# L0SG/grouped-ssd-pytorch

Hardware: AMD Instinct MI355X
Metric: 512x512 4-phase CT img/s (fwd+loss) (higher is better)
Workload: dtype f32; 1 GPU; gssdpp (BASELINE configs[2], GSSD++: self-attention + SA-base + 1 DCN layer x 4 deformable groups, dcn_cat_sab) fwd + MultiBoxLoss, train-mode BN, batch 32, [B,12,300,300] slices; batch_per_gpu=32, global_batch=32

## Files before the change

grouped-ssd-pytorch_amd/gssd/_lib.py:

```python
import ctypes as C
import os

import torch

_HERE = os.path.dirname(os.path.abspath(__file__))
LIB_PATH = os.environ.get('GSSD_LIB_PATH') or os.path.join(_HERE, 'lib', 'libgssd_hip.so')

c_fp = C.c_void_p
c_i = C.c_int
c_f = C.c_float
c_d = C.c_double
c_i64 = C.c_int64


class ConvDesc(C.Structure):
    _fields_ = [
        ('in_', c_fp), ('wgt', c_fp), ('bias', c_fp), ('out', c_fp), ('out_b', c_fp), ('alpha', c_fp),
        ('gate', c_fp), ('resid', c_fp), ('out2', c_fp), ('in_scale', c_fp), ('in_shift', c_fp), ('in_pad', c_fp),
        ('stats', c_fp), ('wgt_wino', c_fp), ('pool_sign', c_fp), ('wgt_x6', c_fp), ('wgt_patch', c_fp),
        ('B', c_i), ('H', c_i), ('W', c_i), ('in_stride', c_i), ('in_ch_off', c_i), ('Ho', c_i), ('Wo', c_i),
        ('Cout', c_i), ('groups', c_i), ('cin_g', c_i), ('KH', c_i), ('KW', c_i), ('stride', c_i), ('pad', c_i),
        ('dil', c_i), ('K', c_i), ('wgt_row_stride', c_i), ('out_stride', c_i), ('out_ch_off', c_i),
        ('out_mode', c_i), ('relu', c_i), ('m_per_image', c_i), ('split_n', c_i), ('split_k', c_i),
        ('out_b_stride', c_i), ('flags', c_i), ('stats_rep', c_i),
        ('in_batch_stride', c_i64), ('wgt_batch_stride', c_i64), ('out_batch_stride', c_i64),
        ('outb_batch_stride', c_i64), ('out_off', c_i64), ('outb_off', c_i64),
    ]


class DcnGeom(C.Structure):
    _fields_ = [(n, C.c_int32) for n in ('B', 'H', 'W', 'C', 'x_stride', 'Ho', 'Wo', 'kh', 'kw', 'sh', 'sw', 'ph', 'pw', 'dh', 'dw', 'dg',
                                         'off_stride', 'mask_stride', 'mask_logit')]


class PlanOp(C.Structure):
    _fields_ = [('kind', c_i), ('fn', c_i), ('stream', c_i), ('nargs', c_i), ('args', C.c_uint64 * 24)]


PLAN_LAUNCH, PLAN_WAIT = 0, 1


class SnItem(C.Structure):
    _fields_ = [('w', c_fp), ('u', c_fp), ('v', c_fp), ('inv_sigma', c_fp), ('rows', c_i), ('cols', c_i)]


OUT_NHWC, OUT_TRANSPOSED, OUT_HEADS, OUT_SPLIT_T = 0, 1, 2, 3
CONV_OUT_F32, CONV_OUTB_BF16_PERM32, CONV_HEADS_SLICES, CONV_POOL2, CONV_RESID_F32, CONV_F16_OK = 1, 2, 4, 8, 16, 32
CONV_IN_NCHW3, CONV_OUT_GROUPCAT, CONV_OUT_X6PLANES, CONV_RESID_XF = 64, 128, 256, 512

SIGNATURES = {
    'gssd_abi_version': (c_i, []),
    'gssd_event_create': (c_i, [C.POINTER(C.c_void_p)]),
    'gssd_event_destroy': (c_i, [c_fp]),
    'gssd_event_record_node': (c_i, [c_fp, c_fp]),
    'gssd_event_elapsed_ms': (c_i, [c_fp, c_fp, C.POINTER(C.c_float)]),
    'gssd_conv_desc_size': (c_i, []),
    'gssd_last_error': (C.c_char_p, []),
    'gssd_build_arch': (C.c_char_p, []),
    'gssd_pack_input_nhwc': (c_i, [c_fp, c_fp, c_i, c_i, c_i, c_i, c_i, c_i, c_fp]),
    'gssd_unpack_nhwc_to_nchw': (c_i, [c_fp, c_fp, c_i, c_i, c_i, c_i, c_i, c_fp]),
    'gssd_pack_conv_weight': (c_i, [c_fp, c_fp, c_i, c_i, c_i, c_i, c_i, c_i, c_fp]),
    'gssd_conv2d_nhwc_f32': (c_i, [C.POINTER(ConvDesc), c_fp]),
    'gssd_conv2d_nhwc_bf16': (c_i, [C.POINTER(ConvDesc), c_fp]),
    'gssd_conv_x6_tile': (c_i, [c_i, c_i, c_i64]),
    'gssd_conv_x6_weight_elems': (c_i64, [c_i, c_i, c_i, c_i, c_i]),
    'gssd_conv_x6_pack_weight': (c_i, [c_fp, c_fp, c_i, c_i, c_i, c_i, c_i, c_i, c_fp]),
    'gssd_conv_x6_takes': (c_i, [C.POINTER(ConvDesc)]),
    'gssd_conv_wino_x6_takes': (c_i, [C.POINTER(ConvDesc)]),
    'gssd_conv_thin_x6_takes': (c_i, [C.POINTER(ConvDesc)]),
    'gssd_conv_thin_nchw3_takes': (c_i, [C.POINTER(ConvDesc)]),
    'gssd_plan_fn_count': (c_i, []),
    'gssd_plan_fn_name': (C.c_char_p, [c_i]),
    'gssd_plan_fn_index': (c_i, [C.c_char_p]),
    'gssd_plan_fn_nargs': (c_i, [c_i]),
    'gssd_plan_op_size': (c_i, []),
    'gssd_plan_run': (c_i, [C.POINTER(PlanOp), c_i, C.POINTER(c_fp), c_i, C.POINTER(c_i)]),
    'gssd_pack_conv_weight_bf16': (c_i, [c_fp, c_fp, c_i, c_i, c_i, c_i, c_i, c_i, c_fp]),
    'gssd_cast_f32_bf16': (c_i, [c_fp, c_fp, c_i64, c_fp]),
    'gssd_cast_rows_f32_bf16': (c_i, [c_fp, c_fp, c_i64, c_i, c_i, c_i, c_fp]),
    'gssd_transpose_cast_f32_bf16': (c_i, [c_fp, c_fp, c_i64, c_i, c_i64, c_i64, c_fp]),
    'gssd_cast_bf16_f32': (c_i, [c_fp, c_fp, c_i64, c_fp]),
    'gssd_pack_input_nhwc_bf16': (c_i, [c_fp, c_fp, c_i, c_i, c_i, c_i, c_i, c_fp]),
    'gssd_bn_relu_pool_bf16': (c_i, [c_fp, c_fp, c_i, c_i, c_i, c_i, c_i, c_i, c_i, c_i, c_i, c_fp, c_d, c_fp, c_fp,
                                     c_fp, c_fp, c_f, c_f, c_i, c_i, c_i, c_fp]),
    'gssd_bn_finalize_bf16': (c_i, [c_fp, c_d, c_fp, c_fp, c_fp, c_fp, c_f, c_f, c_i, c_i, c_fp, c_fp, c_fp, c_i, c_fp]),
    'gssd_l2norm_bf16': (c_i, [c_fp, c_fp, c_fp, c_i64, c_i, c_f, c_fp]),
    'gssd_dcn_packed_weight_elems_bf16': (C.c_longlong, [c_i, c_i]),
    'gssd_dcn_pack_weight_bf16': (c_i, [c_fp, c_fp, c_i, c_i, c_i, c_fp]),
    'gssd_dcn_forward_bf16': (c_i, [c_fp, c_fp, c_fp, c_fp, c_fp, c_i, c_i, c_i, c_i, c_i, c_i, c_i, c_fp]),
    'gssd_winograd_weight_elems': (C.c_longlong, [c_i, c_i, c_i]),
    'gssd_winograd_weight_f32': (c_i, [c_fp, c_fp, c_i, c_i, c_i, c_i, c_fp]),
    'gssd_conv2d_wgrad_f32': (c_i, [C.POINTER(ConvDesc), c_fp, c_fp, c_fp]),
    'gssd_conv2d_wgrad_bf16': (c_i, [C.POINTER(ConvDesc), c_fp, c_fp, c_fp]),
    'gssd_conv2d_wgrad_bf16_supported': (c_i, [C.POINTER(ConvDesc)]),
    'gssd_unpack_conv_weight_grad': (c_i, [c_fp, c_fp, c_i, c_i, c_i, c_i, c_i, c_i, c_i, c_fp]),
    'gssd_pack_conv_weight_dgrad': (c_i, [c_fp, c_fp, c_i, c_i, c_i, c_i, c_i, c_fp]),
    'gssd_bn_relu_pool_f32': (c_i, [c_fp, c_fp, c_i, c_i, c_i, c_i, c_i, c_i, c_i, c_i, c_i, c_fp, c_d, c_fp, c_fp,
                                    c_fp, c_fp, c_f, c_f, c_i, c_i, c_i, c_fp]),
    'gssd_bn_finalize_f32': (c_i, [c_fp, c_d, c_fp, c_fp, c_fp, c_fp, c_f, c_f, c_i, c_i, c_fp, c_fp, c_fp, c_i, c_fp]),
    'gssd_bn_bwd_reduce_f32': (c_i, [c_fp, c_fp, c_fp, c_fp, c_fp, c_fp, c_i, c_i, c_i, c_i, c_i, c_i, c_i, c_i, c_i, c_i, c_fp]),
    'gssd_bn_bwd_finalize_f32': (c_i, [c_fp, c_d, c_fp, c_fp, c_f, c_i, c_fp, c_fp, c_fp, c_fp, c_fp, c_i, c_fp]),
    'gssd_bn_bwd_apply_f32': (c_i, [c_fp, c_fp, c_fp, c_fp, c_fp, c_i64, c_i, c_fp, c_fp]),
    'gssd_bn_bwd_reduce_mixed': (c_i, [c_fp, c_i, c_fp, c_fp, c_fp, c_fp, c_fp, c_fp, c_i, c_i, c_i, c_i, c_i, c_i, c_i, c_i, c_i, c_i, c_fp]),
    'gssd_bn_bwd_apply_mixed': (c_i, [c_fp, c_i, c_fp, c_fp, c_fp, c_fp, c_fp, c_i, c_fp, c_fp, c_fp, c_i64, c_i, c_fp, c_i, c_fp]),
    'gssd_bn_bwd_apply_masked_f32': (c_i, [c_fp, c_fp, c_fp, c_fp, c_i, c_fp, c_fp, c_fp, c_fp, c_i64, c_i, c_fp, c_fp]),
    'gssd_colsum_f32': (c_i, [c_fp, c_i64, c_i, c_i, c_fp, c_fp]),
    'gssd_cast_f64_f32': (c_i, [c_fp, c_fp, c_i, c_i, c_fp]),
    'gssd_l2norm_bwd_f32': (c_i, [c_fp, c_fp, c_fp, c_fp, c_fp, c_fp, c_i64, c_i, c_f, c_fp]),
    'gssd_heads_gather_f32': (c_i, [c_fp, c_fp, c_fp, c_i, c_i, c_i, c_i, c_i, c_i, c_fp]),
    'gssd_upsample_insert_f32': (c_i, [c_fp, c_fp, c_i, c_i, c_i, c_i, c_i, c_i, c_i, c_fp]),
    'gssd_l2norm_f32': (c_i, [c_fp, c_fp, c_fp, c_i64, c_i, c_f, c_fp]),
    'gssd_self_attn_core_f32': (c_i, [c_fp, c_fp, c_fp, c_i, c_i, c_i, c_i, c_i, c_i, c_fp]),
    'gssd_self_attn_core_kv_f32': (c_i, [c_fp, c_fp, c_fp, c_fp, c_i, c_i, c_i, c_i, c_i, c_i, c_i, c_i, c_fp, c_fp]),
    'gssd_sa_pool_kv_f32': (c_i, [c_fp, c_fp, c_fp, c_fp, c_i, c_i, c_i, c_i, c_i, c_i, c_i, c_fp]),
    'gssd_sa_unpool_f32': (c_i, [c_fp, c_fp, c_i, c_i, c_i, c_i, c_i, c_fp]),
    'gssd_pack_conv_weights_batched': (c_i, [c_fp, c_i, c_fp]),
    'gssd_gemm_slot_takes': (c_i, [c_fp]),
    'gssd_conv_flat_bf16_takes': (c_i, [c_fp]),
    'gssd_conv_flat_bf16_tile': (c_i, [c_i]),
    'gssd_heads_reduce_f32': (c_i, [c_fp, c_fp, c_fp, c_i, c_i, c_i, c_fp]),
    'gssd_interp_add_f32': (c_i, [c_fp, c_fp, c_fp, c_fp, c_i, c_i, c_i, c_i, c_i, c_i, c_fp]),
    'gssd_pixellink_final_f32': (c_i, [c_fp, c_fp, c_fp, c_fp, c_i, c_fp, c_fp, c_fp, c_fp, c_fp, c_fp, c_i, c_i, c_fp]),
    'gssd_pixellink_loss_f32': (c_i, [c_fp, c_fp, c_fp, c_fp, c_fp, c_fp, c_fp, c_fp, c_i, c_i, c_i, c_i, c_fp]),
    'gssd_interp_add_bwd_f32': (c_i, [c_fp, c_fp, c_fp, c_fp, c_i, c_i, c_i, c_i, c_i, c_i, c_i, c_fp]),
    'gssd_pixellink_final_bwd_f32': (c_i, [c_fp] * 6 + [c_i, c_fp, c_fp, c_fp, c_fp, c_fp, c_fp, c_i, c_fp, c_fp, c_i, c_i, c_i, c_fp]),
    'gssd_pixellink_loss_bwd_f32': (c_i, [c_fp] * 10 + [c_i, c_i, c_i, c_fp]),
    'gssd_pixellink_decode_f32': (c_i, [c_fp, c_fp, c_fp, c_fp, c_fp, c_i, c_i, c_i, C.c_float, C.c_float, c_i, c_fp]),
    'gssd_self_attn_flash_bwd_bf16': (c_i, [c_fp, c_fp, c_fp, c_fp, c_fp, c_fp, c_fp, c_fp, c_i, c_i, c_i, c_i, c_fp]),
    'gssd_cast_split_f32_bf16': (c_i, [c_fp, c_fp, c_fp, c_i64, c_fp]),
    'gssd_self_attn_flash_bwd_supported': (c_i, [c_i, c_i]),
    'gssd_self_attn_core_x6_supported': (c_i, [c_i, c_i]),
    'gssd_self_attn_core_x6_ws_bytes': (C.c_longlong, [c_i, c_i, c_i, c_i]),
    'gssd_self_attn_core_x6_f32': (c_i, [c_fp, c_fp, c_fp, c_i, c_i, c_i, c_i, c_i, c_fp, c_fp, c_fp]),
    'gssd_self_attn_core_x6_planes_f32': (c_i, [c_fp, c_fp, c_i, c_i, c_i, c_i, c_fp, c_fp]),
    'gssd_self_attn_core_bf16v': (c_i, [c_fp, c_fp, c_fp, c_i, c_i, c_i, c_i, c_i, c_fp, c_fp]),
    'gssd_softmax_rows_f32': (c_i, [c_fp, c_i64, c_i, c_i, c_fp]),
    'gssd_slice_and_cat_f32': (c_i, [c_fp, c_fp, c_fp, c_i64, c_i, c_i, c_i, c_fp]),
    'gssd_spectral_norm_f32': (c_i, [c_fp, c_i, c_i, c_f, c_fp]),
    'gssd_dcn_im2col_f32': (c_i, [c_fp, c_fp, c_fp, c_i, c_i, c_i, c_i, c_i, c_i, c_fp]),
    'gssd_dcn_im2col_bf16': (c_i, [c_fp, c_fp, c_fp, c_i, c_i, c_i, c_i, c_i, c_i, c_fp]),
    'gssd_dcn_packed_weight_elems_x6': (C.c_longlong, [c_i, c_i]),
    'gssd_dcn_pack_weight_x6': (c_i, [c_fp, c_fp, c_i, c_i, c_i, c_fp]),
    'gssd_dcn_forward_x6': (c_i, [c_fp, c_fp, c_fp, c_fp, c_fp, c_i, c_i, c_i, c_i, c_i, c_i, c_i, c_fp]),
    'gssd_conv_patch_x6_weight_elems': (C.c_longlong, [c_i, c_i]),
    'gssd_conv_patch_x6_pack_weight': (c_i, [c_fp, c_fp, c_i, c_i, c_i, c_fp]),
    'gssd_conv_patch_x6_takes': (c_i, [C.POINTER(ConvDesc)]),
    'gssd_dcn_forward_x6_ex': (c_i, [c_fp, c_fp, c_fp, c_fp, c_fp, c_i, c_i, c_i, c_i, c_i, c_i, c_i, c_i, c_fp]),
    'gssd_dcn_packed_weight_elems': (C.c_longlong, [c_i, c_i]),
    'gssd_dcn_pack_weight_f32': (c_i, [c_fp, c_fp, c_i, c_i, c_i, c_fp]),
    'gssd_dcn_streamk': (c_i, [c_i]),
    'gssd_dcn_streamk_status': (c_i, [c_fp]),
    'gssd_dcn_streamk_reset': (c_i, [c_fp]),
    'gssd_dcn_streamk_release': (c_i, [c_fp]),
    'gssd_dcn_forward_f32': (c_i, [c_fp, c_fp, c_fp, c_fp, c_fp, c_i, c_i, c_i, c_i, c_i, c_i, c_i, c_fp]),
    'gssd_resample_ksize': (c_i, [c_i, c_i, c_i]),
    'gssd_resample_coeffs': (c_i, [c_i, c_i, c_i, c_fp, c_fp]),
    'gssd_resize_u8_horizontal': (c_i, [c_fp, c_fp, c_fp, c_fp, c_i, c_i, c_i, c_i, c_i, c_i, c_fp]),
    'gssd_resize_u8_vertical': (c_i, [c_fp, c_fp, c_fp, c_fp, c_i, c_i, c_i, c_i, c_i, c_i, c_i, c_fp, c_fp]),
    'gssd_input_finish_f32': (c_i, [c_fp, c_fp, c_f, c_f, c_f, c_fp, c_i, c_i, c_i, c_i, c_i, c_fp]),
    'gssd_aug_desc_size': (c_i, []),
    'gssd_augment_minmax': (c_i, [c_fp, c_i, c_i, c_i, c_fp, c_fp]),
    'gssd_augment_horizontal': (c_i, [c_fp, c_fp, c_fp, c_f, c_f, c_f, c_fp, c_i, c_i, c_i, c_i, c_i, c_fp]),
    'gssd_augment_vertical': (c_i, [c_fp, c_fp, c_fp, c_fp, c_i, c_i, c_i, c_fp]),
    'gssd_pixellink_targets': (c_i, [c_fp, c_fp, c_i, c_i, c_i, c_fp, c_fp, c_fp, c_fp, c_fp]),
    'gssd_pixellink_final5_f32': (c_i, [c_fp] * 5 + [c_i] + [c_fp] * 6 + [c_i, c_i, c_fp]),
    'gssd_pixellink_final5_bwd_f32': (c_i, [c_fp] * 7 + [c_i] + [c_fp] * 7 + [c_i, c_fp, c_fp, c_i, c_i, c_i, c_fp]),
    'gssd_self_attn_flash_bwd_f32_supported': (c_i, [c_i, c_i]),
    'gssd_self_attn_flash_bwd_f32': (c_i, [c_fp, c_i, c_fp, c_i, c_fp, c_i, c_fp, c_fp, c_fp, c_fp, c_i, c_fp, c_fp, c_i, c_i, c_i, c_i, c_i,
                                           c_i, c_fp]),
    'gssd_eval_match': (c_i, [c_fp, C.c_longlong, c_i, c_i, c_fp, c_fp, c_fp, c_i, c_d, c_fp, c_i, c_i, c_fp, c_fp, c_fp]),
    'gssd_eval_workspace_bytes': (C.c_longlong, [c_i]),
    'gssd_eval_ap': (c_i, [c_fp, c_fp, c_i, c_i, c_d, c_i, c_fp, C.c_longlong, c_fp, c_fp]),
    'gssd_bgemm_f32': (c_i, [c_fp, c_fp, c_fp, c_i, c_i, c_i, c_i, c_i, c_i, c_i, c_i, C.c_longlong, C.c_longlong, C.c_longlong, c_i, c_f,
                             c_i, c_fp]),
    'gssd_softmax_bwd_rows_f32': (c_i, [c_fp, c_fp, c_i64, c_i, c_i, c_fp]),
    'gssd_sn_weight_grad_f32': (c_i, [c_fp, c_i, c_fp, c_fp, c_fp, c_fp, c_fp, c_fp, c_fp, c_i, c_i, c_fp]),
    'gssd_scaled_transpose_f32': (c_i, [c_fp, c_fp, c_fp, c_i, c_i, c_fp]),
    'gssd_dot_f32': (c_i, [c_fp, c_fp, c_i64, c_fp, c_fp]),
    'gssd_rowdot_f32': (c_i, [c_fp, c_fp, c_fp, c_i64, c_i, c_fp]),
    'gssd_bgemm_ex_f32': (c_i, [c_fp, c_fp, c_fp, c_i, c_i, c_i, c_i, c_i, c_i, c_i, c_i, C.c_longlong, C.c_longlong, C.c_longlong, c_i, c_f,
                                c_i, c_fp, c_fp, c_fp]),
    'gssd_axpby_f32': (c_i, [c_fp, c_fp, c_fp, c_i64, c_f, c_f, c_fp]),
    'gssd_scale_cast_f64_f32': (c_i, [c_fp, c_fp, c_fp, c_i, c_fp]),
    'gssd_sa_sigma_grad_f32': (c_i, [c_fp, c_fp, c_fp, c_i, c_fp, c_fp]),
    'gssd_dcn_col2im_f32': (c_i, [c_fp, c_fp, c_fp, c_fp, c_fp, c_i, c_i, c_i, c_i, c_i, c_i, c_fp]),
    'gssd_dcn_geo_im2col_f32': (c_i, [c_fp, c_fp, c_fp, c_fp, C.POINTER(DcnGeom), c_i, c_i, c_fp]),
    'gssd_dcn_geo_col2im_f32': (c_i, [c_fp] * 7 + [C.POINTER(DcnGeom), c_i, c_i, c_fp]),
    'gssd_match_batch': (c_i, [c_fp, c_fp, c_fp, c_i, c_i, c_f, c_f, c_f, c_fp, c_fp, c_fp]),
    'gssd_reduce_max_f32': (c_i, [c_fp, c_i64, c_fp, c_i, c_fp]),
    'gssd_hnm_loss': (c_i, [c_fp, c_fp, c_fp, c_fp, c_fp, c_i, c_i, c_i, c_i, c_i, c_fp, c_fp, c_fp, c_fp]),
    'gssd_loss_finalize': (c_i, [c_fp, c_i, c_fp, c_fp, c_fp]),
    'gssd_loss_finalize_global': (c_i, [c_fp, c_i, c_fp, c_i, c_fp, c_fp, c_fp]),
    'gssd_loss_backward': (c_i, [c_fp, c_fp, c_fp, c_fp, c_fp, c_fp, c_fp, c_fp, c_i, c_i, c_i, c_fp, c_fp, c_fp]),
    'gssd_detect': (c_i, [c_fp, c_fp, c_fp, c_i, c_i, c_i, c_i, c_f, c_f, c_f, c_f, c_i, c_i, c_fp, c_fp, c_fp, c_fp]),
    'gssd_softmax_lastdim_f32': (c_i, [c_fp, c_fp, c_i64, c_i, c_fp]),
}


class GssdError(RuntimeError):
    pass


def _load():
    if not os.path.exists(LIB_PATH):
        raise GssdError(
            f'{LIB_PATH} is missing: the HIP kernels are not built.  Run `make -C '
            f'{os.path.join(_HERE, "csrc")}` (needs hipcc, --offload-arch=gfx950) or '
            f'`python -c "import __graft_entry__ as g; g.build()"`.  There is no CPU fallback.')
    lib = C.CDLL(LIB_PATH)
    for name, (res, args) in SIGNATURES.items():
        try:
            fn = getattr(lib, name)
        except AttributeError as e:
            raise GssdError(f'{LIB_PATH} does not export {name}; rebuild it') from e
        fn.restype = res
        fn.argtypes = args
    if lib.gssd_plan_op_size() != C.sizeof(PlanOp):
        raise GssdError(f'{LIB_PATH}: struct gssd_plan_op is {lib.gssd_plan_op_size()} bytes in the library, {C.sizeof(PlanOp)} in this '
                        f'binding; rebuild the library')
    if lib.gssd_conv_desc_size() != C.sizeof(ConvDesc):
        raise GssdError(f'{LIB_PATH}: struct gssd_conv_desc is {lib.gssd_conv_desc_size()} bytes in the library, '
                        f'{C.sizeof(ConvDesc)} in this binding; rebuild the library')
    return lib


lib = _load()


def check(rc):
    if rc != 0:
        raise GssdError(f'libgssd_hip: error {rc}: {lib.gssd_last_error().decode()}')
```

grouped-ssd-pytorch_amd/gssd/csrc/elementwise.hip:

```cpp
#include "common.h"
#include "kernel_util.h"

namespace {

constexpr int EW_THREADS = 256;
inline int ew_blocks(long long work_items, int per_block = EW_THREADS, int cap = 8192) {
    long long b = (work_items + per_block - 1) / per_block;
    if (b < 1) b = 1;
    if (b > cap) b = cap;
    return (int)b;
}

__global__ void pack_input_kernel(const float* __restrict__ x, float* __restrict__ y, int B, int C, int HW,
                                  int groups, int cpg_in, int cpg_out) {
    const long long total = (long long)B * HW * groups;
    for (long long i = blockIdx.x * (long long)blockDim.x + threadIdx.x; i < total;
         i += (long long)gridDim.x * blockDim.x) {
        const int g = (int)(i % groups);
        const long long bp = i / groups;
        const int pix = (int)(bp % HW);
        const int b = (int)(bp / HW);
        float* o = y + (bp * groups + g) * cpg_out;
        for (int c = 0; c < cpg_out; ++c)
            o[c] = (c < cpg_in) ? x[((long long)b * C + g * cpg_in + c) * HW + pix] : 0.f;
    }
}

__global__ void unpack_nhwc_kernel(const float* __restrict__ x, float* __restrict__ y, int B, int C, int HW,
                                   int x_stride) {
    const long long total = (long long)B * C * HW;
    for (long long i = blockIdx.x * (long long)blockDim.x + threadIdx.x; i < total;
         i += (long long)gridDim.x * blockDim.x) {
        const int pix = (int)(i % HW);
        const long long bc = i / HW;
        const int c = (int)(bc % C);
        const int b = (int)(bc / C);
        y[i] = x[((long long)b * HW + pix) * x_stride + c];
    }
}

__global__ void pack_weight_kernel(const float* __restrict__ w, float* __restrict__ wp, int Cout, int cin_g, int taps,
                                   int cin_g_pad, int Kpad) {
    const long long total = (long long)Cout * Kpad;
    for (long long i = blockIdx.x * (long long)blockDim.x + threadIdx.x; i < total;
         i += (long long)gridDim.x * blockDim.x) {
        const int k = (int)(i % Kpad);
        const int o = (int)(i / Kpad);
        const int tap = k / cin_g_pad, c = k - tap * cin_g_pad;
        float v = 0.f;
        if (tap < taps && c < cin_g) v = w[((long long)o * cin_g + c) * taps + tap];
        wp[i] = v;
    }
}

__global__ void pack_weight_batched_kernel(const gssd_pack_item* __restrict__ items) {
    const gssd_pack_item it = items[blockIdx.y];
    const long long total = (long long)it.Cout * it.Kpad;
    for (long long i = blockIdx.x * (long long)blockDim.x + threadIdx.x; i < total; i += (long long)gridDim.x * blockDim.x) {
        const int k = (int)(i % it.Kpad);
        const int o = (int)(i / it.Kpad);
        const int tap = k / it.cin_g_pad, c = k - tap * it.cin_g_pad;
        float v = 0.f;
        if (tap < it.taps && c < it.cin_g) v = it.w[((long long)o * it.cin_g + c) * it.taps + tap];
        it.wp[i] = v;
    }
}

__global__ __launch_bounds__(256) void bn_relu_pool_kernel(
    const float* __restrict__ raw, float* __restrict__ out, int B, int H, int W, int C, int Ho, int Wo, int pk, int ps,
    int pp, const double* __restrict__ stats, double count, const float* __restrict__ gamma,
    const float* __restrict__ beta, float* running_mean, float* running_var, float momentum, float eps, int training,
    int relu, int srep) {
    extern __shared__ __attribute__((aligned(16))) float sm[];
    float* s_scale = sm;
    float* s_shift = sm + C;
    for (int c = threadIdx.x; c < C; c += blockDim.x) {
        if (gamma == nullptr) {
            s_scale[c] = 1.f;
            s_shift[c] = 0.f;
            continue;
        }
        double mean, var;
        if (training) {
            mean = gssd_stats_sum(stats, c, 2 * C, srep) / count;
            var = gssd_stats_sum(stats, C + c, 2 * C, srep) / count - mean * mean;
            if (var < 0.0) var = 0.0;
            if (blockIdx.x == 0) {
                const double unb = count > 1.0 ? var * count / (count - 1.0) : var;
                running_mean[c] = (float)((1.0 - (double)momentum) * (double)running_mean[c] + (double)momentum * mean);
                running_var[c] = (float)((1.0 - (double)momentum) * (double)running_var[c] + (double)momentum * unb);
            }
        } else {
            mean = (double)running_mean[c];
            var = (double)running_var[c];
        }
        const double inv = 1.0 / sqrt(var + (double)eps);
        const double sc = (double)gamma[c] * inv;
        s_scale[c] = (float)sc;
        s_shift[c] = (float)((double)beta[c] - mean * sc);
    }
    __syncthreads();
    const int C4 = C >> 2;
    const long long total = (long long)B * Ho * Wo * C4;
    for (long long i = blockIdx.x * (long long)blockDim.x + threadIdx.x; i < total;
         i += (long long)gridDim.x * blockDim.x) {
        const int c4 = (int)(i % C4);
        long long t = i / C4;
        const int xo = (int)(t % Wo);
        t /= Wo;
        const int yo = (int)(t % Ho);
        const int b = (int)(t / Ho);
        const f32x4 sc = *reinterpret_cast<const f32x4*>(s_scale + 4 * c4);
        const f32x4 sh = *reinterpret_cast<const f32x4*>(s_shift + 4 * c4);
        f32x4 r;
        if (pk == 0) {
            const f32x4 v = *reinterpret_cast<const f32x4*>(raw + (((long long)b * H + yo) * W + xo) * C + 4 * c4);
            r = v * sc + sh;
        } else {
            r = {-INFINITY, -INFINITY, -INFINITY, -INFINITY};
            const int y0 = yo * ps - pp, x0 = xo * ps - pp;
            for (int dy = 0; dy < pk; ++dy) {
                const int yy = y0 + dy;
                if ((unsigned)yy >= (unsigned)H) continue;
                for (int dx = 0; dx < pk; ++dx) {
                    const int xx = x0 + dx;
                    if ((unsigned)xx >= (unsigned)W) continue;
                    const f32x4 v =
                        *reinterpret_cast<const f32x4*>(raw + (((long long)b * H + yy) * W + xx) * C + 4 * c4);
                    const f32x4 a = v * sc + sh;
#pragma unroll
                    for (int e = 0; e < 4; ++e) r[e] = fmaxf(r[e], a[e]);
                }
            }
        }
        if (relu) {
#pragma unroll
            for (int e = 0; e < 4; ++e) r[e] = fmaxf(r[e], 0.f);
        }
        *reinterpret_cast<f32x4*>(out + i * 4) = r;
    }
}

__global__ void bn_finalize_kernel(const double* __restrict__ stats, double count, const float* __restrict__ gamma,
                                   const float* __restrict__ beta, float* running_mean, float* running_var,
                                   float momentum, float eps, int training, int C, float* __restrict__ scale,
                                   float* __restrict__ shift, float* __restrict__ pad, int srep) {
    const int c = blockIdx.x * blockDim.x + threadIdx.x;
    if (c >= C) return;
    double mean, var;
    if (training) {
        mean = gssd_stats_sum(stats, c, 2 * C, srep) / count;
        var = gssd_stats_sum(stats, C + c, 2 * C, srep) / count - mean * mean;
        if (var < 0.0) var = 0.0;
        if (training == 1) {
            const double unb = count > 1.0 ? var * count / (count - 1.0) : var;
            running_mean[c] = (float)((1.0 - (double)momentum) * (double)running_mean[c] + (double)momentum * mean);
            running_var[c] = (float)((1.0 - (double)momentum) * (double)running_var[c] + (double)momentum * unb);
        }
    } else {
        mean = (double)running_mean[c];
        var = (double)running_var[c];
    }
    double sc = (double)gamma[c] * (1.0 / sqrt(var + (double)eps));
    const float sh = (float)((double)beta[c] - mean * sc);
    float scf = (float)sc;
    if (scf == 0.f) scf = 1e-30f;
    scale[c] = scf;
    shift[c] = sh;
    pad[c] = scf > 0.f ? -3.0e38f : 3.0e38f;
}

__global__ __launch_bounds__(256) void l2norm_kernel(const float* __restrict__ x, const float* __restrict__ w,
                                                     float* __restrict__ out, long long pixels, int C, float eps) {
    const int lane = threadIdx.x & 63;
    const long long wave0 = (blockIdx.x * (long long)blockDim.x + threadIdx.x) >> 6;
    const long long nwaves = ((long long)gridDim.x * blockDim.x) >> 6;
    const int C4 = C >> 2;
    for (long long p = wave0; p < pixels; p += nwaves) {
        const f32x4* xp = reinterpret_cast<const f32x4*>(x + p * C);
        float ss = 0.f;
        for (int c = lane; c < C4; c += 64) {
            const f32x4 v = xp[c];
            ss += v[0] * v[0] + v[1] * v[1] + v[2] * v[2] + v[3] * v[3];
        }
        ss = wave_sum(ss);
        const float inv = 1.f / (sqrtf(ss) + eps);
        f32x4* op = reinterpret_cast<f32x4*>(out + p * C);
        for (int c = lane; c < C4; c += 64) {
            const f32x4 v = xp[c];
            const f32x4 ww = reinterpret_cast<const f32x4*>(w)[c];
            op[c] = ww * (v * inv);
        }
    }
}

__global__ __launch_bounds__(256) void softmax_rows_kernel(float* __restrict__ x, long long rows, int n, int stride) {
    const int lane = threadIdx.x & 63;
    const long long wave0 = (blockIdx.x * (long long)blockDim.x + threadIdx.x) >> 6;
    const long long nwaves = ((long long)gridDim.x * blockDim.x) >> 6;
    for (long long rI = wave0; rI < rows; rI += nwaves) {
        float* row = x + rI * stride;
        float m = -INFINITY;
        for (int c = lane; c < n; c += 64) m = fmaxf(m, row[c]);
        m = wave_max(m);
        float s = 0.f;
        for (int c = lane; c < n; c += 64) {
            const float e = expf(row[c] - m);
            row[c] = e;
            s += e;
        }
        s = wave_sum(s);
        const float inv = 1.f / s;
        for (int c = lane; c < stride; c += 64) row[c] = (c < n) ? row[c] * inv : 0.f;
    }
}

__global__ void slice_and_cat_kernel(const float* __restrict__ a, const float* __restrict__ b, float* __restrict__ out,
                                     long long pixels, int Ca, int Cb, int groups) {
    const int Co = Ca + Cb, Co4 = Co >> 2;
    const int ga = Ca / groups, gb = Cb / groups;
    const long long total = pixels * Co4;
    for (long long i = blockIdx.x * (long long)blockDim.x + threadIdx.x; i < total;
         i += (long long)gridDim.x * blockDim.x) {
        const int c = (int)(i % Co4) * 4;
        const long long p = i / Co4;
        const int g = c / (ga + gb), cc = c - g * (ga + gb);
        f32x4 v;
        if (cc < ga) v = *reinterpret_cast<const f32x4*>(a + p * Ca + g * ga + cc);
        else v = *reinterpret_cast<const f32x4*>(b + p * Cb + g * gb + (cc - ga));
        *reinterpret_cast<f32x4*>(out + i * 4) = v;
    }
}

__device__ float block_sum(float v, float* red) {
    v = wave_sum(v);
    const int lane = threadIdx.x & 63, wave = threadIdx.x >> 6;
    __syncthreads();
    if (lane == 0) red[wave] = v;
    __syncthreads();
    float t = 0.f;
    for (int i = 0; i < (int)(blockDim.x >> 6); ++i) t += red[i];
    return t;
}

__global__ __launch_bounds__(1024) void spectral_norm_kernel(const gssd_sn_item* __restrict__ items, int do_iter,
                                                            float eps) {
    extern __shared__ __attribute__((aligned(16))) float sm[];
    const gssd_sn_item it = items[blockIdx.x];
    const int R = it.rows, Cc = it.cols;
    float* su = sm;
    float* sv = sm + R;
    float* red = sv + Cc;
    const int tid = threadIdx.x, lane = tid & 63, wave = tid >> 6, nw = blockDim.x >> 6;
    for (int i = tid; i < R; i += blockDim.x) su[i] = it.u[i];
    for (int i = tid; i < Cc; i += blockDim.x) sv[i] = it.v[i];
    __syncthreads();
    const bool vec = ((Cc | R) & 3) == 0 && (Cc >> 2) <= (int)blockDim.x && (((uintptr_t)it.w) & 15) == 0;
    if (do_iter) {
        float nrm = 0.f;
        if (vec) {
            float* part = red + 16;
            const int nq = Cc >> 2, S = (int)blockDim.x / nq;
            const int cq = tid % nq, rs = tid / nq;
            if (rs < S) {
                f32x4 a8[8];
#pragma unroll
                for (int q = 0; q < 8; ++q) a8[q] = f32x4{0.f, 0.f, 0.f, 0.f};
                const float* wc = it.w + 4 * cq;
                int rr = rs;
                for (; rr + 7 * S < R; rr += 8 * S) {
#pragma unroll
                    for (int q = 0; q < 8; ++q) a8[q] += *reinterpret_cast<const f32x4*>(wc + (size_t)(rr + q * S) * Cc) * su[rr + q * S];
                }
                for (; rr < R; rr += S) a8[0] += *reinterpret_cast<const f32x4*>(wc + (size_t)rr * Cc) * su[rr];
                *reinterpret_cast<f32x4*>(part + rs * Cc + 4 * cq) = ((a8[0] + a8[1]) + (a8[2] + a8[3])) + ((a8[4] + a8[5]) + (a8[6] + a8[7]));
            }
            __syncthreads();
            for (int c = tid; c < Cc; c += blockDim.x) {
                float acc = part[c];
                for (int sl = 1; sl < S; ++sl) acc += part[sl * Cc + c];
                sv[c] = acc;
                nrm += acc * acc;
            }
        } else {
            for (int c = tid; c < Cc; c += blockDim.x) {
                float a8[8] = {0.f, 0.f, 0.f, 0.f, 0.f, 0.f, 0.f, 0.f};
                int rr = 0;
                for (; rr + 8 <= R; rr += 8) {
#pragma unroll
                    for (int q = 0; q < 8; ++q) a8[q] += it.w[(size_t)(rr + q) * Cc + c] * su[rr + q];
                }
                for (; rr < R; ++rr) a8[0] += it.w[(size_t)rr * Cc + c] * su[rr];
                const float acc = ((a8[0] + a8[1]) + (a8[2] + a8[3])) + ((a8[4] + a8[5]) + (a8[6] + a8[7]));
                sv[c] = acc;
                nrm += acc * acc;
            }
        }
        nrm = block_sum(nrm, red);
        const float inv = 1.f / fmaxf(sqrtf(nrm), eps);
        for (int c = tid; c < Cc; c += blockDim.x) sv[c] *= inv;
        __syncthreads();
    }
    float sig = 0.f, nrm2 = 0.f;
    auto row_done = [&](int rr, float acc) {
        if (do_iter) {
            su[rr] = acc;
            nrm2 += acc * acc;
        } else {
            sig += su[rr] * acc;
        }
    };
    if (vec) {
        for (int r0 = wave * 4; r0 < R; r0 += nw * 4) {
            float acc[4] = {0.f, 0.f, 0.f, 0.f};
            for (int c = lane * 4; c < Cc; c += 256) {
                const f32x4 v4 = *reinterpret_cast<const f32x4*>(sv + c);
#pragma unroll
                for (int q = 0; q < 4; ++q) {
                    if (r0 + q < R) {
                        const f32x4 w4 = *reinterpret_cast<const f32x4*>(it.w + (size_t)(r0 + q) * Cc + c);
                        acc[q] += (w4[0] * v4[0] + w4[1] * v4[1]) + (w4[2] * v4[2] + w4[3] * v4[3]);
                    }
                }
            }
#pragma unroll
            for (int q = 0; q < 4; ++q) {
                const float t = wave_sum(acc[q]);
                if (lane == 0 && r0 + q < R) row_done(r0 + q, t);
            }
        }
    } else {
        for (int rr = wave; rr < R; rr += nw) {
            float acc = 0.f;
            for (int c = lane; c < Cc; c += 64) acc += it.w[(size_t)rr * Cc + c] * sv[c];
            acc = wave_sum(acc);
            if (lane == 0) row_done(rr, acc);
        }
    }
    if (do_iter) {
        nrm2 = block_sum(nrm2, red);
        const float nn = fmaxf(sqrtf(nrm2), eps);
        __syncthreads();
        for (int i = tid; i < R; i += blockDim.x) it.u[i] = su[i] / nn;
        for (int i = tid; i < Cc; i += blockDim.x) it.v[i] = sv[i];
        const float is = nn / nrm2;
        for (int i = tid; i < R; i += blockDim.x) it.inv_sigma[i] = is;
    } else {
        sig = block_sum(sig, red);
        const float is = 1.f / sig;
        for (int i = tid; i < R; i += blockDim.x) it.inv_sigma[i] = is;
    }
}

__global__ void softmax_lastdim_kernel(const float* __restrict__ x, float* __restrict__ y, long long rows, int C) {
    for (long long i = blockIdx.x * (long long)blockDim.x + threadIdx.x; i < rows;
         i += (long long)gridDim.x * blockDim.x) {
        const float* xr = x + i * C;
        float m = xr[0];
        for (int c = 1; c < C; ++c) m = fmaxf(m, xr[c]);
        float s = 0.f;
        for (int c = 0; c < C; ++c) s += (float)exp((double)(xr[c] - m));
        for (int c = 0; c < C; ++c) y[i * C + c] = (float)exp((double)(xr[c] - m)) / s;
    }
}

__global__ __launch_bounds__(256) void reduce_max_kernel(const float* __restrict__ x, long long n, float* out) {
    __shared__ float red[4];
    float m = -INFINITY;
    const long long n4 = n >> 2;
    for (long long i = blockIdx.x * (long long)blockDim.x + threadIdx.x; i < n4; i += (long long)gridDim.x * blockDim.x) {
        const f32x4 v = reinterpret_cast<const f32x4*>(x)[i];
        m = fmaxf(fmaxf(m, fmaxf(v[0], v[1])), fmaxf(v[2], v[3]));
    }
    if (blockIdx.x == 0)
        for (long long i = (n4 << 2) + threadIdx.x; i < n; i += blockDim.x) m = fmaxf(m, x[i]);
    m = wave_max(m);
    if ((threadIdx.x & 63) == 0) red[threadIdx.x >> 6] = m;
    __syncthreads();
    if (threadIdx.x == 0) out[blockIdx.x] = fmaxf(fmaxf(red[0], red[1]), fmaxf(red[2], red[3]));
}

__global__ __launch_bounds__(256) void heads_reduce_kernel(const float* __restrict__ ws, const signed char* __restrict__ splits,
                                                          float* __restrict__ out, long long total, int P, int C) {
    for (long long i = blockIdx.x * (long long)blockDim.x + threadIdx.x; i < total; i += (long long)gridDim.x * blockDim.x) {
        const int p = (int)((i / C) % P);
        const int n = splits[p];
        float a = ws[i];
        for (int k = 1; k < n; ++k) a += ws[(size_t)k * total + i];
        out[i] = a;
    }
}

}

extern "C" int gssd_pack_input_nhwc(const float* x, float* y, int B, int C, int H, int W, int groups, int cpg_out,
                                    gssd_stream_t stream) {
    GSSD_CHECK_ARG(x && y && B > 0 && C > 0 && H > 0 && W > 0 && groups > 0 && C % groups == 0);
    GSSD_CHECK_ARG(cpg_out >= C / groups);
    const long long total = (long long)B * H * W * groups;
    hipLaunchKernelGGL(pack_input_kernel, dim3(ew_blocks(total)), dim3(EW_THREADS), 0, as_stream(stream), x, y, B, C,
                       H * W, groups, C / groups, cpg_out);
    GSSD_CHECK_LAUNCH();
    return GSSD_OK;
}

extern "C" int gssd_unpack_nhwc_to_nchw(const float* x, float* y, int B, int C, int H, int W, int x_stride,
                                        gssd_stream_t stream) {
    GSSD_CHECK_ARG(x && y && B > 0 && C > 0 && H > 0 && W > 0 && x_stride >= C);
    hipLaunchKernelGGL(unpack_nhwc_kernel, dim3(ew_blocks((long long)B * C * H * W)), dim3(EW_THREADS), 0,
                       as_stream(stream), x, y, B, C, H * W, x_stride);
    GSSD_CHECK_LAUNCH();
    return GSSD_OK;
}

extern "C" int gssd_pack_conv_weight(const float* w, float* wp, int Cout, int cin_g, int KH, int KW, int cin_g_pad,
                                     int Kpad, gssd_stream_t stream) {
    GSSD_CHECK_ARG(w && wp && Cout > 0 && cin_g > 0 && KH > 0 && KW > 0);
    GSSD_CHECK_ARG(cin_g_pad >= cin_g && cin_g_pad % 4 == 0 && Kpad >= KH * KW * cin_g_pad && Kpad % 4 == 0);
    hipLaunchKernelGGL(pack_weight_kernel, dim3(ew_blocks((long long)Cout * Kpad)), dim3(EW_THREADS), 0,
                       as_stream(stream), w, wp, Cout, cin_g, KH * KW, cin_g_pad, Kpad);
    GSSD_CHECK_LAUNCH();
    return GSSD_OK;
}

extern "C" int gssd_pack_conv_weights_batched(const gssd_pack_item* items_dev, int n_items, gssd_stream_t stream) {
    GSSD_CHECK_ARG(items_dev && n_items > 0 && n_items < 65536);
    hipLaunchKernelGGL(pack_weight_batched_kernel, dim3(48, n_items), dim3(EW_THREADS), 0, as_stream(stream), items_dev);
    GSSD_CHECK_LAUNCH();
    return GSSD_OK;
}

extern "C" int gssd_bn_relu_pool_f32(const float* raw, float* out, int B, int H, int W, int C, int Ho, int Wo,
                                     int pool_k, int pool_s, int pool_p, const double* stats, double count,
                                     const float* gamma, const float* beta, float* running_mean, float* running_var,
                                     float momentum, float eps, int training, int relu, int stats_rep, gssd_stream_t stream) {
    GSSD_CHECK_ARG(raw && out && stats_rep >= 0);
    GSSD_CHECK_ARG(gamma == nullptr || (beta && running_mean && running_var));
    GSSD_CHECK_ARG(B > 0 && H > 0 && W > 0 && C > 0 && C % 4 == 0 && Ho > 0 && Wo > 0);
    GSSD_CHECK_ARG(!training || gamma == nullptr || (stats != nullptr && count > 0));
    if (pool_k == 0) GSSD_CHECK_ARG(Ho == H && Wo == W);
    else GSSD_CHECK_ARG(pool_s > 0 && pool_p >= 0 && (Ho - 1) * pool_s - pool_p < H && (Wo - 1) * pool_s - pool_p < W);
    const long long total = (long long)B * Ho * Wo * (C / 4);
    const int blocks = ew_blocks(total, EW_THREADS * 4, 2048);
    hipLaunchKernelGGL(bn_relu_pool_kernel, dim3(blocks), dim3(EW_THREADS), 2 * C * sizeof(float), as_stream(stream),
                       raw, out, B, H, W, C, Ho, Wo, pool_k, pool_s, pool_p, stats, count, gamma, beta, running_mean,
                       running_var, momentum, eps, training, relu, stats_rep);
    GSSD_CHECK_LAUNCH();
    return GSSD_OK;
}

extern "C" int gssd_bn_finalize_f32(const double* stats, double count, const float* gamma, const float* beta,
                                    float* running_mean, float* running_var, float momentum, float eps, int training,
                                    int C, float* scale, float* shift, float* pad, int stats_rep, gssd_stream_t stream) {
    GSSD_CHECK_ARG(gamma && beta && running_mean && running_var && scale && shift && pad && C > 0 && stats_rep >= 0);
    GSSD_CHECK_ARG(!training || (stats != nullptr && count > 0));
    hipLaunchKernelGGL(bn_finalize_kernel, dim3((C + 255) / 256), dim3(256), 0, as_stream(stream), stats, count, gamma,
                       beta, running_mean, running_var, momentum, eps, training, C, scale, shift, pad, stats_rep);
    GSSD_CHECK_LAUNCH();
    return GSSD_OK;
}

extern "C" int gssd_l2norm_f32(const float* x, const float* weight, float* out, int64_t pixels, int C, float eps,
                               gssd_stream_t stream) {
    GSSD_CHECK_ARG(x && weight && out && pixels > 0 && C > 0 && C % 4 == 0);
    hipLaunchKernelGGL(l2norm_kernel, dim3(ew_blocks(pixels, 4, 4096)), dim3(256), 0, as_stream(stream), x, weight, out,
                       (long long)pixels, C, eps);
    GSSD_CHECK_LAUNCH();
    return GSSD_OK;
}

extern "C" int gssd_softmax_rows_f32(float* x, int64_t rows, int n, int row_stride, gssd_stream_t stream) {
    GSSD_CHECK_ARG(x && rows > 0 && n > 0 && row_stride >= n);
    hipLaunchKernelGGL(softmax_rows_kernel, dim3(ew_blocks(rows, 4, 16384)), dim3(256), 0, as_stream(stream), x,
                       (long long)rows, n, row_stride);
    GSSD_CHECK_LAUNCH();
    return GSSD_OK;
}

extern "C" int gssd_slice_and_cat_f32(const float* a, const float* b, float* out, int64_t pixels, int Ca, int Cb,
                                      int groups, gssd_stream_t stream) {
    GSSD_CHECK_ARG(a && b && out && pixels > 0 && groups > 0 && Ca % (4 * groups) == 0 && Cb % (4 * groups) == 0);
    hipLaunchKernelGGL(slice_and_cat_kernel, dim3(ew_blocks(pixels * ((Ca + Cb) / 4))), dim3(EW_THREADS), 0,
                       as_stream(stream), a, b, out, (long long)pixels, Ca, Cb, groups);
    GSSD_CHECK_LAUNCH();
    return GSSD_OK;
}

extern "C" int gssd_spectral_norm_f32(const gssd_sn_item* items_dev, int n, int do_power_iteration, float eps,
                                      gssd_stream_t stream) {
    GSSD_CHECK_ARG(items_dev && n > 0);
    const size_t smem = (4096 + 16 + 4096) * sizeof(float);
    hipLaunchKernelGGL(spectral_norm_kernel, dim3(n), dim3(1024), smem, as_stream(stream), items_dev,
                       do_power_iteration, eps);
    GSSD_CHECK_LAUNCH();
    return GSSD_OK;
}

extern "C" int gssd_softmax_lastdim_f32(const float* x, float* y, int64_t rows, int C, gssd_stream_t stream) {
    GSSD_CHECK_ARG(x && y && rows > 0 && C > 0);
    hipLaunchKernelGGL(softmax_lastdim_kernel, dim3(ew_blocks(rows)), dim3(EW_THREADS), 0, as_stream(stream), x, y,
                       (long long)rows, C);
    GSSD_CHECK_LAUNCH();
    return GSSD_OK;
}

extern "C" int gssd_reduce_max_f32(const float* x, int64_t n, float* out, int out_n, gssd_stream_t stream) {
    GSSD_CHECK_ARG(x && out && n > 0 && out_n > 0 && out_n <= 1024 && ((uintptr_t)x % 16) == 0);
    hipLaunchKernelGGL(reduce_max_kernel, dim3(out_n), dim3(256), 0, as_stream(stream), x, (long long)n, out);
    GSSD_CHECK_LAUNCH();
    return GSSD_OK;
}

extern "C" int gssd_heads_reduce_f32(const float* ws, const signed char* splits, float* out, int B, int P, int C, gssd_stream_t stream) {
    GSSD_CHECK_ARG(ws && splits && out && B > 0 && P > 0 && C > 0);
    const long long total = (long long)B * P * C;
    int blocks = (int)((total + 255) / 256);
    if (blocks > 4096) blocks = 4096;
    hipLaunchKernelGGL(heads_reduce_kernel, dim3(blocks), dim3(256), 0, as_stream(stream), ws, splits, out, total, P, C);
    GSSD_CHECK_LAUNCH();
    return GSSD_OK;
}
```

grouped-ssd-pytorch_amd/gssd/csrc/loss.hip:

```cpp
#include "common.h"

namespace {

constexpr int MAX_GT = 64;
constexpr int LT = 1024;

__device__ __forceinline__ float iou_pf(float ax1, float ay1, float ax2, float ay2, float area_a, float bx1, float by1,
                                        float bx2, float by2) {
    const float w = fmaxf(fminf(ax2, bx2) - fmaxf(ax1, bx1), 0.f);
    const float h = fmaxf(fminf(ay2, by2) - fmaxf(ay1, by1), 0.f);
    const float inter = w * h;
    const float area_b = (bx2 - bx1) * (by2 - by1);
    const float uni = (area_a + area_b) - inter;
    return __fdiv_rn(inter, uni);
}

__global__ __launch_bounds__(LT) void match_kernel(const float* __restrict__ targets, const int* __restrict__ gt_off,
                                                   const float* __restrict__ priors, int P, float thr,
                                                   float var0, float var1, float* __restrict__ loc_t,
                                                   int64_t* __restrict__ conf_t) {
    extern __shared__ __attribute__((aligned(16))) unsigned char smraw[];
    __shared__ float gt[MAX_GT][5];
    __shared__ float gt_area[MAX_GT];
    __shared__ int best_prior[MAX_GT];
    __shared__ float red_v[LT / 64];
    __shared__ int red_i[LT / 64];
    short* forced = reinterpret_cast<short*>(smraw);

    const int b = blockIdx.x, tid = threadIdx.x;
    const int g0 = gt_off[b];
    int n = gt_off[b + 1] - g0;
    if (n > MAX_GT) n = MAX_GT;
    if (tid < 5) gt[0][tid] = 0.f;
    __syncthreads();
    for (int i = tid; i < n * 5; i += LT) gt[i / 5][i % 5] = targets[(size_t)g0 * 5 + i];
    for (int p = tid; p < P; p += LT) forced[p] = -1;
    __syncthreads();
    if (tid < n) gt_area[tid] = (gt[tid][2] - gt[tid][0]) * (gt[tid][3] - gt[tid][1]);
    __syncthreads();

    for (int j = 0; j < n; ++j) {
        float bv = -INFINITY;
        int bi = 0x7fffffff;
        bool any_nan = false;
        for (int p = tid; p < P; p += LT) {
            const float4 pr = reinterpret_cast<const float4*>(priors)[p];
            const float hx = pr.z / 2.f, hy = pr.w / 2.f;
            const float v = iou_pf(gt[j][0], gt[j][1], gt[j][2], gt[j][3], gt_area[j], pr.x - hx, pr.y - hy, pr.x + hx,
                                   pr.y + hy);
            if (v > bv) {
                bv = v;
                bi = p;
            }
        }
        (void)any_nan;
        for (int o = 32; o > 0; o >>= 1) {
            const float ov = __shfl_xor(bv, o, 64);
            const int oi = __shfl_xor(bi, o, 64);
            if (ov > bv || (ov == bv && oi < bi)) {
                bv = ov;
                bi = oi;
            }
        }
        if ((tid & 63) == 0) {
            red_v[tid >> 6] = bv;
            red_i[tid >> 6] = bi;
        }
        __syncthreads();
        if (tid == 0) {
            for (int w = 1; w < LT / 64; ++w)
                if (red_v[w] > bv || (red_v[w] == bv && red_i[w] < bi)) {
                    bv = red_v[w];
                    bi = red_i[w];
                }
            best_prior[j] = (bi == 0x7fffffff) ? 0 : bi;
        }
        __syncthreads();
    }
    if (tid == 0)
        for (int j = 0; j < n; ++j) forced[best_prior[j]] = (short)j;
    __syncthreads();

    for (int p = tid; p < P; p += LT) {
        const float4 pr = reinterpret_cast<const float4*>(priors)[p];
        const float hx = pr.z / 2.f, hy = pr.w / 2.f;
        const float px1 = pr.x - hx, py1 = pr.y - hy, px2 = pr.x + hx, py2 = pr.y + hy;
        float bv = -INFINITY;
        int bj = 0;
        for (int j = 0; j < n; ++j) {
            const float v = iou_pf(gt[j][0], gt[j][1], gt[j][2], gt[j][3], gt_area[j], px1, py1, px2, py2);
            if (v > bv) {
                bv = v;
                bj = j;
            }
        }
        const int f = forced[p];
        if (f >= 0) {
            bv = 2.f;
            bj = f;
        }
        int64_t conf = (int64_t)(gt[bj][4] + 1.f);
        if (bv < thr) conf = 0;
        conf_t[(size_t)b * P + p] = conf;
        const float gx1 = gt[bj][0], gy1 = gt[bj][1], gx2 = gt[bj][2], gy2 = gt[bj][3];
        float4 o;
        o.x = __fdiv_rn(((gx1 + gx2) / 2.f) - pr.x, var0 * pr.z);
        o.y = __fdiv_rn(((gy1 + gy2) / 2.f) - pr.y, var0 * pr.w);
        o.z = __fdiv_rn((float)log((double)__fdiv_rn(gx2 - gx1, pr.z)), var1);
        o.w = __fdiv_rn((float)log((double)__fdiv_rn(gy2 - gy1, pr.w)), var1);
        reinterpret_cast<float4*>(loc_t)[(size_t)b * P + p] = o;
    }
}

__device__ unsigned radix_select_desc(const float* vals, int n, int k, unsigned* hist , int* bcast ,
                                      int* n_greater) {
    unsigned prefix = 0, mask = 0;
    int greater = 0;
    for (int shift = 24; shift >= 0; shift -= 8) {
        for (int i = threadIdx.x; i < 256; i += blockDim.x) hist[i] = 0;
        __syncthreads();
        for (int i = threadIdx.x; i < n; i += blockDim.x) {
            const unsigned u = __float_as_uint(vals[i]);
            if ((u & mask) == prefix) atomicAdd(&hist[(u >> shift) & 255u], 1u);
        }
        __syncthreads();
        if (threadIdx.x == 0) {
            int acc = greater, bin = 255;
            for (; bin > 0; --bin) {
                if (acc + (int)hist[bin] >= k) break;
                acc += (int)hist[bin];
            }
            bcast[0] = bin;
            bcast[1] = acc;
        }
        __syncthreads();
        prefix |= ((unsigned)bcast[0]) << shift;
        mask |= 255u << shift;
        greater = bcast[1];
        __syncthreads();
    }
    *n_greater = greater;
    return prefix;
}

__global__ __launch_bounds__(LT) void hnm_loss_kernel(const float* __restrict__ loc, const float* __restrict__ conf,
                                                      const float* __restrict__ loc_t,
                                                      const int64_t* __restrict__ conf_t,
                                                      const float* __restrict__ xmax_p, int xmax_n, int P, int C, int negpos_ratio,
                                                      uint8_t* __restrict__ sel, double* __restrict__ partial,
                                                      float* __restrict__ lca_out) {
    extern __shared__ __attribute__((aligned(16))) unsigned char smraw[];
    float* lca = reinterpret_cast<float*>(smraw);
    __shared__ unsigned hist[256];
    __shared__ int bcast[2];
    __shared__ int s_cnt[LT / 64];
    __shared__ double s_red[LT / 64][2];
    __shared__ int s_tie_base;

    const int b = blockIdx.x, tid = threadIdx.x, lane = tid & 63, wave = tid >> 6;
    float xmax = xmax_p[0];
    for (int i = 1; i < xmax_n; ++i) xmax = fmaxf(xmax, xmax_p[i]);
    const float* cb = conf + (size_t)b * P * C;
    const int64_t* tb = conf_t + (size_t)b * P;

    int npos = 0;
    for (int p = tid; p < P; p += LT) {
        const int t = (int)tb[p];
        float s = 0.f;
        for (int c = 0; c < C; ++c) s += (float)exp((double)(cb[(size_t)p * C + c] - xmax));
        float v = ((float)log((double)s) + xmax) - cb[(size_t)p * C + t];
        if (t > 0) {
            v = 0.f;
            ++npos;
        }
        if (!(v > 0.f)) v = 0.f;
        lca[p] = v;
    }
    npos = wave_sum(npos);
    if (lane == 0) s_cnt[wave] = npos;
    __syncthreads();
    npos = 0;
    for (int w = 0; w < LT / 64; ++w) npos += s_cnt[w];
    int num_neg = negpos_ratio * npos;
    if (num_neg > P - 1) num_neg = P - 1;
    if (lca_out)
        for (int p = tid; p < P; p += LT) lca_out[(size_t)b * P + p] = lca[p];

    unsigned kth_bits = 0xffffffffu;
    int n_greater = 0;
    if (num_neg > 0) kth_bits = radix_select_desc(lca, P, num_neg, hist, bcast, &n_greater);
    const int ties_needed = num_neg - n_greater;

    double sum_l = 0.0, sum_c = 0.0;
    if (tid == 0) s_tie_base = 0;
    __syncthreads();
    for (int p0 = 0; p0 < P; p0 += LT) {
        const int p = p0 + tid;
        bool is_tie = false, take = false, pos = false;
        if (p < P) {
            const unsigned u = __float_as_uint(lca[p]);
            pos = tb[p] > 0;
            if (num_neg > 0) {
                if (u > kth_bits) take = true;
                else if (u == kth_bits) is_tie = true;
            }
        }
        const unsigned long long bal = __ballot(is_tie);
        const int before = __popcll(bal & ((1ull << lane) - 1ull));
        if (lane == 0) s_cnt[wave] = __popcll(bal);
        __syncthreads();
        int base = s_tie_base;
        for (int w = 0; w < wave; ++w) base += s_cnt[w];
        if (is_tie && base + before < ties_needed) take = true;
        __syncthreads();
        if (tid == 0) {
            int t = 0;
            for (int w = 0; w < LT / 64; ++w) t += s_cnt[w];
            s_tie_base += t;
        }
        if (p < P) {
            const uint8_t code = pos ? 1 : (take ? 2 : 0);
            const bool neg_flag = take;
            sel[(size_t)b * P + p] = pos ? (uint8_t)(neg_flag ? 3 : 1) : code;
            if (pos) {
                const float4 a = reinterpret_cast<const float4*>(loc)[(size_t)b * P + p];
                const float4 t4 = reinterpret_cast<const float4*>(loc_t)[(size_t)b * P + p];
                const float d[4] = {a.x - t4.x, a.y - t4.y, a.z - t4.z, a.w - t4.w};
#pragma unroll
                for (int e = 0; e < 4; ++e) {
                    const float ad = fabsf(d[e]);
                    sum_l += (double)(ad < 1.f ? 0.5f * d[e] * d[e] : ad - 0.5f);
                }
            }
            if (pos || take) {
                const int t = (int)tb[p];
                float m = cb[(size_t)p * C];
                for (int c = 1; c < C; ++c) m = fmaxf(m, cb[(size_t)p * C + c]);
                double s = 0.0;
                for (int c = 0; c < C; ++c) s += exp((double)(cb[(size_t)p * C + c] - m));
                sum_c += (log(s) + (double)m) - (double)cb[(size_t)p * C + t];
            }
        }
        __syncthreads();
    }
    sum_l = wave_sum(sum_l);
    sum_c = wave_sum(sum_c);
    if (lane == 0) {
        s_red[wave][0] = sum_l;
        s_red[wave][1] = sum_c;
    }
    __syncthreads();
    if (tid == 0) {
        double l = 0.0, c = 0.0;
        for (int w = 0; w < LT / 64; ++w) {
            l += s_red[w][0];
            c += s_red[w][1];
        }
        partial[(size_t)b * 4 + 0] = l;
        partial[(size_t)b * 4 + 1] = c;
        partial[(size_t)b * 4 + 2] = (double)npos;
        partial[(size_t)b * 4 + 3] = (double)num_neg;
    }
}

__global__ void loss_finalize_kernel(const double* __restrict__ partial, int B, float* __restrict__ losses,
                                     double* __restrict__ n_total) {
    if (threadIdx.x == 0 && blockIdx.x == 0) {
        double l = 0.0, c = 0.0, n = 0.0;
        for (int b = 0; b < B; ++b) {
            l += partial[b * 4 + 0];
            c += partial[b * 4 + 1];
            n += partial[b * 4 + 2];
        }
        losses[0] = (float)(l / n);
        losses[1] = (float)(c / n);
        if (n_total) *n_total = n;
    }
}

__global__ void loss_finalize_global_kernel(const double* __restrict__ partial, int B, const double* __restrict__ n_global, int world,
                                            float* __restrict__ losses, double* __restrict__ n_total) {
    if (threadIdx.x == 0 && blockIdx.x == 0) {
        double l = 0.0, c = 0.0;
        for (int b = 0; b < B; ++b) {
            l += partial[b * 4 + 0];
            c += partial[b * 4 + 1];
        }
        const double n = *n_global / (double)world;
        losses[0] = (float)(l / n);
        losses[1] = (float)(c / n);
        *n_total = n;
    }
}

__global__ void loss_backward_kernel(const float* __restrict__ loc, const float* __restrict__ conf,
                                     const float* __restrict__ loc_t, const int64_t* __restrict__ conf_t,
                                     const uint8_t* __restrict__ sel, const double* __restrict__ n_total,
                                     const float* __restrict__ gl_p, const float* __restrict__ gc_p, long long BP, int C,
                                     float* __restrict__ dloc, float* __restrict__ dconf) {
    const float invN = (float)(1.0 / *n_total);
    const float gl = (gl_p ? *gl_p : 1.f) * invN, gc = (gc_p ? *gc_p : 1.f) * invN;
    for (long long i = blockIdx.x * (long long)blockDim.x + threadIdx.x; i < BP;
         i += (long long)gridDim.x * blockDim.x) {
        const uint8_t s = sel[i];
        float4 g = {0.f, 0.f, 0.f, 0.f};
        if (s & 1) {
            const float4 a = reinterpret_cast<const float4*>(loc)[i];
            const float4 t = reinterpret_cast<const float4*>(loc_t)[i];
            const float d[4] = {a.x - t.x, a.y - t.y, a.z - t.z, a.w - t.w};
            float o[4];
#pragma unroll
            for (int e = 0; e < 4; ++e) o[e] = (fabsf(d[e]) < 1.f ? d[e] : (d[e] > 0.f ? 1.f : -1.f)) * gl;
            g = {o[0], o[1], o[2], o[3]};
        }
        reinterpret_cast<float4*>(dloc)[i] = g;
        if (s) {
            const int t = (int)conf_t[i];
            float m = conf[i * C];
            for (int c = 1; c < C; ++c) m = fmaxf(m, conf[i * C + c]);
            float z = 0.f;
            for (int c = 0; c < C; ++c) z += __expf(conf[i * C + c] - m);
            for (int c = 0; c < C; ++c) dconf[i * C + c] = (__expf(conf[i * C + c] - m) / z - (c == t ? 1.f : 0.f)) * gc;
        } else {
            for (int c = 0; c < C; ++c) dconf[i * C + c] = 0.f;
        }
    }
}

}

extern "C" int gssd_match_batch(const float* targets, const int* gt_off, const float* priors, int B, int P,
                                float threshold, float var0, float var1, float* loc_t, int64_t* conf_t,
                                gssd_stream_t stream) {
    GSSD_CHECK_ARG(targets && gt_off && priors && loc_t && conf_t);
    GSSD_CHECK_ARG(B > 0 && P > 0 && P < 32768);
    GSSD_CHECK_ARG(((uintptr_t)priors % 16) == 0 && ((uintptr_t)loc_t % 16) == 0);
    hipLaunchKernelGGL(match_kernel, dim3(B), dim3(LT), (size_t)P * sizeof(short), as_stream(stream), targets, gt_off,
                       priors, P, threshold, var0, var1, loc_t, conf_t);
    GSSD_CHECK_LAUNCH();
    return GSSD_OK;
}

extern "C" int gssd_hnm_loss(const float* loc, const float* conf, const float* loc_t, const int64_t* conf_t,
                             const float* xmax, int xmax_n, int B, int P, int C, int negpos_ratio, uint8_t* sel,
                             double* partial, float* loss_c_all, gssd_stream_t stream) {
    GSSD_CHECK_ARG(loc && conf && loc_t && conf_t && xmax && xmax_n > 0 && sel && partial);
    GSSD_CHECK_ARG(B > 0 && P > 0 && P <= 36000 && C >= 2 && negpos_ratio >= 0);
    GSSD_CHECK_ARG(((uintptr_t)loc % 16) == 0 && ((uintptr_t)loc_t % 16) == 0);
    static unsigned attr_mask = 0;
    const size_t smem = (size_t)P * sizeof(float);
    if (smem > 48 * 1024)
        if (const int rc = gssd_max_dynamic_lds(&attr_mask, hnm_loss_kernel, 150 * 1024)) return rc;
    hipLaunchKernelGGL(hnm_loss_kernel, dim3(B), dim3(LT), smem, as_stream(stream), loc, conf, loc_t, conf_t, xmax, xmax_n, P,
                       C, negpos_ratio, sel, partial, loss_c_all);
    GSSD_CHECK_LAUNCH();
    return GSSD_OK;
}

extern "C" int gssd_loss_finalize(const double* partial, int B, float* losses, double* n_total, gssd_stream_t stream) {
    GSSD_CHECK_ARG(partial && losses && B > 0);
    hipLaunchKernelGGL(loss_finalize_kernel, dim3(1), dim3(64), 0, as_stream(stream), partial, B, losses, n_total);
    GSSD_CHECK_LAUNCH();
    return GSSD_OK;
}

extern "C" int gssd_loss_finalize_global(const double* partial, int B, const double* n_global, int world, float* losses, double* n_total,
                                         gssd_stream_t stream) {
    GSSD_CHECK_ARG(partial && losses && n_global && n_total && B > 0 && world > 0);
    hipLaunchKernelGGL(loss_finalize_global_kernel, dim3(1), dim3(64), 0, as_stream(stream), partial, B, n_global, world, losses, n_total);
    GSSD_CHECK_LAUNCH();
    return GSSD_OK;
}

extern "C" int gssd_loss_backward(const float* loc, const float* conf, const float* loc_t, const int64_t* conf_t,
                                  const uint8_t* sel, const double* n_total, const float* grad_l, const float* grad_c,
                                  int B, int P, int C, float* dloc, float* dconf, gssd_stream_t stream) {
    GSSD_CHECK_ARG(loc && conf && loc_t && conf_t && sel && n_total && dloc && dconf && B > 0 && P > 0 && C >= 2);
    const long long BP = (long long)B * P;
    int blocks = (int)((BP + 255) / 256);
    if (blocks > 4096) blocks = 4096;
    hipLaunchKernelGGL(loss_backward_kernel, dim3(blocks), dim3(256), 0, as_stream(stream), loc, conf, loc_t, conf_t, sel,
                       n_total, grad_l, grad_c, BP, C, dloc, dconf);
    GSSD_CHECK_LAUNCH();
    return GSSD_OK;
}
```

grouped-ssd-pytorch_amd/gssd/csrc/plan_run.hip:

```cpp
#include <hip/hip_runtime.h>
#include <cstdint>
#include <cstring>
#include <mutex>
#include <tuple>
#include <type_traits>
#include <utility>
#include "common.h"

namespace {

template <class T>
inline T plan_arg(uint64_t w) {
    if constexpr (std::is_pointer_v<T>) {
        return reinterpret_cast<T>(static_cast<uintptr_t>(w));
    } else if constexpr (std::is_same_v<T, float>) {
        const uint32_t b = static_cast<uint32_t>(w);
        float f;
        memcpy(&f, &b, 4);
        return f;
    } else if constexpr (std::is_same_v<T, double>) {
        double d;
        memcpy(&d, &w, 8);
        return d;
    } else {
        static_assert(std::is_integral_v<T>, "plan argument types: pointers, integers, float, double");
        return static_cast<T>(static_cast<int64_t>(w));
    }
}

template <class... P, size_t... I>
inline int plan_call(int (*f)(P...), const uint64_t* a, gssd_stream_t s, std::index_sequence<I...>) {
    using T = std::tuple<P...>;
    static_assert(sizeof...(P) - 1 <= GSSD_PLAN_MAX_ARGS, "GSSD_PLAN_MAX_ARGS");
    static_assert(std::is_same_v<std::tuple_element_t<sizeof...(P) - 1, T>, gssd_stream_t>, "the last parameter is the stream");
    return f(plan_arg<std::tuple_element_t<I, T>>(a[I])..., s);
}

template <class... P>
constexpr int plan_nargs(int (*)(P...)) { return (int)sizeof...(P) - 1; }

struct PlanFn {
    const char* name;
    int nargs;
    int (*thunk)(const uint64_t*, gssd_stream_t);
};

template <auto F>
int plan_thunk(const uint64_t* a, gssd_stream_t s) {
    return plan_call(F, a, s, std::make_index_sequence<plan_nargs(F)>{});
}

#define GSSD_PLAN_FN(f) PlanFn{#f, plan_nargs(&f), &plan_thunk<&f>}
const PlanFn g_plan_fns[] = {
    GSSD_PLAN_FN(gssd_event_record_node),
    GSSD_PLAN_FN(gssd_pack_input_nhwc),
    GSSD_PLAN_FN(gssd_unpack_nhwc_to_nchw),
    GSSD_PLAN_FN(gssd_pack_conv_weight),
    GSSD_PLAN_FN(gssd_pack_conv_weights_batched),
    GSSD_PLAN_FN(gssd_conv2d_nhwc_f32),
    GSSD_PLAN_FN(gssd_conv_x6_pack_weight),
    GSSD_PLAN_FN(gssd_conv_patch_x6_pack_weight),
    GSSD_PLAN_FN(gssd_conv2d_nhwc_bf16),
    GSSD_PLAN_FN(gssd_pack_conv_weight_bf16),
    GSSD_PLAN_FN(gssd_cast_f32_bf16),
    GSSD_PLAN_FN(gssd_cast_bf16_f32),
    GSSD_PLAN_FN(gssd_pack_input_nhwc_bf16),
    GSSD_PLAN_FN(gssd_bn_relu_pool_bf16),
    GSSD_PLAN_FN(gssd_bn_finalize_bf16),
    GSSD_PLAN_FN(gssd_l2norm_bf16),
    GSSD_PLAN_FN(gssd_winograd_weight_f32),
    GSSD_PLAN_FN(gssd_conv2d_wgrad_f32),
    GSSD_PLAN_FN(gssd_conv2d_wgrad_bf16),
    GSSD_PLAN_FN(gssd_unpack_conv_weight_grad),
    GSSD_PLAN_FN(gssd_pack_conv_weight_dgrad),
    GSSD_PLAN_FN(gssd_bn_relu_pool_f32),
    GSSD_PLAN_FN(gssd_bn_finalize_f32),
    GSSD_PLAN_FN(gssd_bn_bwd_reduce_f32),
    GSSD_PLAN_FN(gssd_bn_bwd_finalize_f32),
    GSSD_PLAN_FN(gssd_bn_bwd_apply_f32),
    GSSD_PLAN_FN(gssd_bn_bwd_reduce_mixed),
    GSSD_PLAN_FN(gssd_bn_bwd_apply_mixed),
    GSSD_PLAN_FN(gssd_bn_bwd_apply_masked_f32),
    GSSD_PLAN_FN(gssd_colsum_f32),
    GSSD_PLAN_FN(gssd_cast_f64_f32),
    GSSD_PLAN_FN(gssd_l2norm_bwd_f32),
    GSSD_PLAN_FN(gssd_heads_gather_f32),
    GSSD_PLAN_FN(gssd_upsample_insert_f32),
    GSSD_PLAN_FN(gssd_l2norm_f32),
    GSSD_PLAN_FN(gssd_self_attn_core_f32),
    GSSD_PLAN_FN(gssd_self_attn_core_kv_f32),
    GSSD_PLAN_FN(gssd_sa_pool_kv_f32),
    GSSD_PLAN_FN(gssd_sa_unpool_f32),
    GSSD_PLAN_FN(gssd_self_attn_core_bf16v),
    GSSD_PLAN_FN(gssd_self_attn_core_x6_f32),
    GSSD_PLAN_FN(gssd_self_attn_core_x6_planes_f32),
    GSSD_PLAN_FN(gssd_self_attn_flash_bwd_bf16),
    GSSD_PLAN_FN(gssd_softmax_rows_f32),
    GSSD_PLAN_FN(gssd_slice_and_cat_f32),
    GSSD_PLAN_FN(gssd_spectral_norm_f32),
    GSSD_PLAN_FN(gssd_dcn_im2col_f32),
    GSSD_PLAN_FN(gssd_dcn_im2col_bf16),
    GSSD_PLAN_FN(gssd_dcn_geo_im2col_f32),
    GSSD_PLAN_FN(gssd_dcn_geo_col2im_f32),
    GSSD_PLAN_FN(gssd_dcn_pack_weight_f32),
    GSSD_PLAN_FN(gssd_dcn_forward_f32),
    GSSD_PLAN_FN(gssd_dcn_streamk_reset),
    GSSD_PLAN_FN(gssd_dcn_pack_weight_x6),
    GSSD_PLAN_FN(gssd_dcn_forward_x6),
    GSSD_PLAN_FN(gssd_dcn_forward_x6_ex),
    GSSD_PLAN_FN(gssd_dcn_pack_weight_bf16),
    GSSD_PLAN_FN(gssd_dcn_forward_bf16),
    GSSD_PLAN_FN(gssd_dcn_col2im_f32),
    GSSD_PLAN_FN(gssd_resize_u8_horizontal),
    GSSD_PLAN_FN(gssd_resize_u8_vertical),
    GSSD_PLAN_FN(gssd_input_finish_f32),
    GSSD_PLAN_FN(gssd_augment_minmax),
    GSSD_PLAN_FN(gssd_augment_horizontal),
    GSSD_PLAN_FN(gssd_augment_vertical),
    GSSD_PLAN_FN(gssd_pixellink_targets),
    GSSD_PLAN_FN(gssd_bgemm_f32),
    GSSD_PLAN_FN(gssd_bgemm_ex_f32),
    GSSD_PLAN_FN(gssd_rowdot_f32),
    GSSD_PLAN_FN(gssd_softmax_bwd_rows_f32),
    GSSD_PLAN_FN(gssd_sn_weight_grad_f32),
    GSSD_PLAN_FN(gssd_scaled_transpose_f32),
    GSSD_PLAN_FN(gssd_cast_split_f32_bf16),
    GSSD_PLAN_FN(gssd_cast_rows_f32_bf16),
    GSSD_PLAN_FN(gssd_transpose_cast_f32_bf16),
    GSSD_PLAN_FN(gssd_dot_f32),
    GSSD_PLAN_FN(gssd_axpby_f32),
    GSSD_PLAN_FN(gssd_scale_cast_f64_f32),
    GSSD_PLAN_FN(gssd_sa_sigma_grad_f32),
    GSSD_PLAN_FN(gssd_match_batch),
    GSSD_PLAN_FN(gssd_reduce_max_f32),
    GSSD_PLAN_FN(gssd_hnm_loss),
    GSSD_PLAN_FN(gssd_loss_finalize),
    GSSD_PLAN_FN(gssd_loss_finalize_global),
    GSSD_PLAN_FN(gssd_loss_backward),
    GSSD_PLAN_FN(gssd_detect),
    GSSD_PLAN_FN(gssd_softmax_lastdim_f32),
    GSSD_PLAN_FN(gssd_eval_match),
    GSSD_PLAN_FN(gssd_eval_ap),
    GSSD_PLAN_FN(gssd_heads_reduce_f32),
    GSSD_PLAN_FN(gssd_interp_add_f32),
    GSSD_PLAN_FN(gssd_pixellink_final_f32),
    GSSD_PLAN_FN(gssd_pixellink_loss_f32),
    GSSD_PLAN_FN(gssd_interp_add_bwd_f32),
    GSSD_PLAN_FN(gssd_pixellink_final_bwd_f32),
    GSSD_PLAN_FN(gssd_pixellink_loss_bwd_f32),
    GSSD_PLAN_FN(gssd_pixellink_decode_f32),
    GSSD_PLAN_FN(gssd_pixellink_final5_f32),
    GSSD_PLAN_FN(gssd_pixellink_final5_bwd_f32),
    GSSD_PLAN_FN(gssd_self_attn_flash_bwd_f32),
};
#undef GSSD_PLAN_FN
constexpr int N_PLAN_FNS = (int)(sizeof(g_plan_fns) / sizeof(g_plan_fns[0]));

constexpr int N_EVENTS = 64;
struct EventRing {
    hipEvent_t ev[N_EVENTS];
    int next = 0;
    bool ready = false;
    std::mutex mu;
};
EventRing g_rings[32];

int record_and_wait(hipStream_t src, hipStream_t dst) {
    int cur = 0, dev = -1;
    (void)hipGetDevice(&cur);
    hipDevice_t sdev;
    if (src && hipStreamGetDevice(src, &sdev) == hipSuccess) dev = (int)sdev;
    if (dev < 0) dev = cur;
    if (dev < 0 || dev >= 32) return 1;
    EventRing& r = g_rings[dev];
    std::lock_guard<std::mutex> lock(r.mu);
    if (!r.ready) {
        if (dev != cur && hipSetDevice(dev) != hipSuccess) return 1;
        bool ok = true;
        for (int i = 0; i < N_EVENTS && ok; ++i) ok = hipEventCreateWithFlags(&r.ev[i], hipEventDisableTiming) == hipSuccess;
        if (dev != cur) (void)hipSetDevice(cur);
        if (!ok) return 1;
        r.ready = true;
    }
    hipEvent_t e = r.ev[r.next];
    r.next = (r.next + 1) % N_EVENTS;
    return (hipEventRecord(e, src) != hipSuccess || hipStreamWaitEvent(dst, e, 0) != hipSuccess) ? 1 : 0;
}

}

extern "C" int gssd_plan_fn_count(void) { return N_PLAN_FNS; }

extern "C" const char* gssd_plan_fn_name(int index) { return index >= 0 && index < N_PLAN_FNS ? g_plan_fns[index].name : nullptr; }

extern "C" int gssd_plan_fn_index(const char* name) {
    if (!name) return -1;
    for (int i = 0; i < N_PLAN_FNS; ++i)
        if (!strcmp(g_plan_fns[i].name, name)) return i;
    return -1;
}

extern "C" int gssd_plan_fn_nargs(int index) { return index >= 0 && index < N_PLAN_FNS ? g_plan_fns[index].nargs : -1; }

extern "C" int gssd_plan_op_size(void) { return (int)sizeof(gssd_plan_op); }

extern "C" int gssd_plan_run(const gssd_plan_op* ops, int n_ops, const gssd_stream_t* streams, int n_streams, int* failed_at) {
    GSSD_CHECK_ARG(ops && n_ops >= 0 && streams && n_streams > 0);
    if (failed_at) *failed_at = -1;
    for (int i = 0; i < n_ops; ++i) {
        const gssd_plan_op& op = ops[i];
        int rc = GSSD_OK;
        if (op.stream < 0 || op.stream >= n_streams) {
            gssd_set_error("gssd_plan_run: stream index out of range");
            rc = GSSD_EINVAL;
        } else if (op.kind == GSSD_PLAN_LAUNCH) {
            if (op.fn < 0 || op.fn >= N_PLAN_FNS) {
                gssd_set_error("gssd_plan_run: function index out of range");
                rc = GSSD_EINVAL;
            } else if (op.nargs != g_plan_fns[op.fn].nargs) {
                gssd_set_error("gssd_plan_run: argument count does not match the function's parameters");
                rc = GSSD_EINVAL;
            } else {
                rc = g_plan_fns[op.fn].thunk(op.args, streams[op.stream]);
            }
        } else if (op.kind == GSSD_PLAN_WAIT) {
            if (op.fn < 0 || op.fn >= n_streams) {
                gssd_set_error("gssd_plan_run: awaited stream index out of range");
                rc = GSSD_EINVAL;
            } else if (op.fn != op.stream) {
                if (record_and_wait(as_stream(streams[op.fn]), as_stream(streams[op.stream]))) {
                    gssd_set_error("gssd_plan_run: event record / stream wait failed");
                    rc = GSSD_ELAUNCH;
                }
            }
        } else {
            gssd_set_error("gssd_plan_run: unknown op kind");
            rc = GSSD_EINVAL;
        }
        if (rc != GSSD_OK) {
            if (failed_at) *failed_at = i;
            return rc;
        }
    }
    return GSSD_OK;
}
```

grouped-ssd-pytorch_amd/gssd/ops.py:

```python
import ctypes as C

import os
import torch

from . import _lib
from ._lib import ConvDesc, SnItem, check, lib

BK = 32


def _stream():
    return torch.cuda.current_stream().cuda_stream


def _p(t):
    return 0 if t is None else t.data_ptr()


def _need_cuda(*ts):
    for t in ts:
        if t is not None and not t.is_cuda:
            raise _lib.GssdError('the GSSD HIP path needs tensors on the MI355X (got a CPU tensor); '
                                 'there is no CPU fallback')


def round_up(x, m):
    return (x + m - 1) // m * m


def pack_input(x_nchw, groups, cpg_out):
    _need_cuda(x_nchw)
    x = x_nchw.contiguous().float()
    B, Cc, H, W = x.shape
    y = torch.empty(B, H, W, groups * cpg_out, device=x.device, dtype=torch.float32)
    check(lib.gssd_pack_input_nhwc(_p(x), _p(y), B, Cc, H, W, groups, cpg_out, _stream()))
    return y


def unpack_nhwc(x_nhwc, C_=None):
    _need_cuda(x_nhwc)
    B, H, W, S = x_nhwc.shape
    C_ = C_ or S
    y = torch.empty(B, C_, H, W, device=x_nhwc.device, dtype=torch.float32)
    check(lib.gssd_unpack_nhwc_to_nchw(_p(x_nhwc), _p(y), B, C_, H, W, S, _stream()))
    return y


def packed_k(cin_g, kh, kw):
    cin_pad = round_up(cin_g, 4)
    return cin_pad, kh * kw * cin_pad


class PackRecorder:

    class Unstable(Exception):
        """a source that is not the parameter's own fp32 storage (its pointer would not survive to the next refresh)"""

    def __init__(self):
        self.items, self.keep = [], []

    def add(self, src, dst, Cout, cin_g, taps, cin_pad, K):
        self.items.append((src.data_ptr(), dst.data_ptr(), Cout, cin_g, taps, cin_pad, K))
        self.keep += [src, dst]


recorder = None


def _stable_f32(t):
    d = t.detach()
    if not isinstance(t, torch.nn.Parameter) or d.dtype != torch.float32 or not d.is_contiguous():
        raise PackRecorder.Unstable()
    return d


def pack_weight(w_oihw, out=None, row_offset=0):
    _need_cuda(w_oihw)
    w = _stable_f32(w_oihw) if recorder is not None else w_oihw.detach().contiguous().float()
    Cout, cin_g, KH, KW = w.shape
    cin_pad, K = packed_k(cin_g, KH, KW)
    if out is None:
        out = torch.empty(Cout, K, device=w.device, dtype=torch.float32)
    assert out.shape[1] == K
    dst = out[row_offset:row_offset + Cout]
    if recorder is not None:
        recorder.add(w, dst, Cout, cin_g, KH * KW, cin_pad, K)
        return out
    check(lib.gssd_pack_conv_weight(_p(w), _p(dst), Cout, cin_g, KH, KW, cin_pad, K, _stream()))
    return out


def copy_into(dst, src):
    if recorder is not None and dst.dtype == torch.float32 and dst.is_contiguous() and dst.numel() == src.numel():
        s = _stable_f32(src)
        n = s.numel()
        recorder.add(s, dst, 1, n, 1, n, n)
        return dst
    if recorder is not None:
        raise PackRecorder.Unstable()
    return dst.copy_(src.detach().reshape(dst.shape) if src.numel() == dst.numel() else src.detach())


def pack_table(rec, device):
    import numpy as np
    dt = np.dtype([('w', np.uint64), ('wp', np.uint64), ('Cout', np.int32), ('cin_g', np.int32), ('taps', np.int32),
                   ('cin_pad', np.int32), ('K', np.int32), ('reserved', np.int32)])
    arr = np.zeros(len(rec.items), dt)
    for i, it in enumerate(rec.items):
        arr[i] = it + (0,)
    return torch.from_numpy(arr.view(np.uint8).copy()).to(device)


def run_pack_table(table, n):
    check(lib.gssd_pack_conv_weights_batched(_p(table), n, _stream()))


def pack_weight_bf16(w_oihw, out=None, row_offset=0, cin_pad=None):
    _need_cuda(w_oihw)
    w = w_oihw.detach().contiguous().float()
    Cout, cin_g, KH, KW = w.shape
    cin_pad = cin_pad or round_up(cin_g, 8)
    K = KH * KW * cin_pad
    if out is None:
        out = torch.empty(Cout, K, device=w.device, dtype=torch.bfloat16)
    assert out.shape[1] == K and out.dtype == torch.bfloat16
    dst = out[row_offset:row_offset + Cout]
    check(lib.gssd_pack_conv_weight_bf16(_p(w), _p(dst), Cout, cin_g, KH, KW, cin_pad, K, _stream()))
    return out


def cast_bf16(x, out=None):
    _need_cuda(x)
    x = x.detach().contiguous().float()
    if out is None:
        out = torch.empty(x.shape, device=x.device, dtype=torch.bfloat16)
    check(lib.gssd_cast_f32_bf16(_p(x), _p(out), x.numel(), _stream()))
    return out


def make_conv_desc(inp, wgt, out, *, B, H, W, in_stride, cin_g, Cout, groups=1, k=1, stride=1, pad=0, dil=1,
                   bias=None, in_ch_off=0, out_stride=None, out_ch_off=0, out_mode=_lib.OUT_NHWC, relu=False,
                   stats=None, alpha=None, gate=None, resid=None, out2=None, out_b=None, split_n=0,
                   m_per_image=False, in_batch_stride=0, wgt_batch_stride=0, out_batch_stride=0,
                   outb_batch_stride=0, out_off=0, outb_off=0, wgt_row_stride=None, split_k=1, in_scale=None,
                   in_shift=None, in_pad=None, wgt_wino=None, out_b_stride=0, flags=0, pool_sign=None, stats_rep=0, wgt_x6=None, wgt_patch=None):
    Ho = (H + 2 * pad - dil * (k - 1) - 1) // stride + 1
    Wo = (W + 2 * pad - dil * (k - 1) - 1) // stride + 1
    K = k * k * cin_g
    d = ConvDesc()
    d.in_, d.wgt, d.bias, d.out, d.out_b = _p(inp), _p(wgt), _p(bias), _p(out), _p(out_b)
    d.alpha, d.gate, d.resid, d.out2, d.stats = _p(alpha), _p(gate), _p(resid), _p(out2), _p(stats)
    d.B, d.H, d.W, d.in_stride, d.in_ch_off, d.Ho, d.Wo = B, H, W, in_stride, in_ch_off, Ho, Wo
    d.Cout, d.groups, d.cin_g, d.KH, d.KW, d.stride, d.pad, d.dil = Cout, groups, cin_g, k, k, stride, pad, dil
    d.K = K
    d.wgt_row_stride = wgt_row_stride if wgt_row_stride is not None else K
    d.out_stride = out_stride if out_stride is not None else Cout
    d.out_ch_off, d.out_mode, d.relu, d.m_per_image, d.split_n = out_ch_off, out_mode, int(relu), int(m_per_image), split_n
    d.split_k = split_k
    d.in_scale, d.in_shift, d.in_pad = _p(in_scale), _p(in_shift), _p(in_pad)
    d.wgt_wino = _p(wgt_wino)
    d.wgt_x6 = _p(wgt_x6)
    d.wgt_patch = _p(wgt_patch)
    d.stats_rep = int(stats_rep)
    d.pool_sign = _p(pool_sign)
    d.out_b_stride = out_b_stride
    d.flags = flags
    d.in_batch_stride, d.wgt_batch_stride = in_batch_stride, wgt_batch_stride
    d.out_batch_stride, d.outb_batch_stride, d.out_off, d.outb_off = out_batch_stride, outb_batch_stride, out_off, outb_off
    return d, Ho, Wo


def auto_split_k(M, Cout, groups, K, target_blocks=1024, max_split=48):
    cout_g = Cout // groups
    bn = 128 if cout_g > 64 else 64 if cout_g > 32 else 32 if cout_g > 16 else 16
    blocks = -(-M // 128) * groups * (-(-cout_g // bn))
    chunks = -(-K // BK)
    return int(max(1, min(max_split, chunks // 4, target_blocks // blocks)))


def run_conv(desc):
    check(lib.gssd_conv2d_nhwc_f32(C.byref(desc), _stream()))


def winograd_eligible(k, stride, pad, dil, cin_g, cout_g, groups=4):
    if not (k == 3 and stride == 1 and pad == 1 and dil == 1 and cin_g % 16 == 0):
        return False
    return cout_g % 32 == 0 or (groups == 1 and cout_g >= 24) or (groups == 4 and cin_g == 16 and cout_g == 16)


def x6_tile(cout_g, groups, M):
    return int(lib.gssd_conv_x6_tile(cout_g, groups, M))


X6_F16 = os.environ.get('GSSD_X6_F16', '1') != '0'


def x6_wanted(k, cin_g, cout_g, groups, M, winograd=False, forward=False):
    ok = cin_g % 32 == 0 and cout_g >= 128 and cout_g % 8 == 0 and k * k * cin_g >= 256 and M >= 4096
    if winograd:
        return ok and forward and X6_F16 and M < 16384
    return ok


def x6_weight(w_packed, groups, cin_g, taps, bn, out=None):
    Cout = w_packed.shape[0]
    if out is None:
        n = int(lib.gssd_conv_x6_weight_elems(Cout, groups, cin_g, taps, bn))
        if n <= 0:
            raise _lib.GssdError(f'not a conv_x6 shape: Cout {Cout}, groups {groups}, cin_g {cin_g}, tile {bn}')
        out = torch.empty(n, device=w_packed.device, dtype=torch.int16)
    check(lib.gssd_conv_x6_pack_weight(_p(w_packed), _p(out), Cout, groups, cin_g, taps, w_packed.stride(0), bn, _stream()))
    return out


def patch_x6_weight(w_packed, cin, out=None):
    Cout = w_packed.shape[0]
    if out is None:
        n = int(lib.gssd_conv_patch_x6_weight_elems(Cout, cin))
        if n <= 0:
            raise _lib.GssdError(f'not a conv_patch_x6 shape: Cout {Cout}, cin {cin}')
        out = torch.empty(n, device=w_packed.device, dtype=torch.int16)
    check(lib.gssd_conv_patch_x6_pack_weight(_p(w_packed), _p(out), Cout, cin, w_packed.stride(0), _stream()))
    return out


def winograd_weight(w_packed, groups, cin_g, out=None):
    Cout = w_packed.shape[0]
    if out is None:
        n = int(lib.gssd_winograd_weight_elems(Cout, groups, cin_g))
        if n <= 0:
            raise _lib.GssdError(f'not a Winograd shape: Cout {Cout}, groups {groups}, cin_g {cin_g}')
        out = torch.empty(n, device=w_packed.device, dtype=torch.float32)
    check(lib.gssd_winograd_weight_f32(_p(w_packed), _p(out), Cout, groups, cin_g, w_packed.stride(0), _stream()))
    return out


def conv2d_nhwc(x, w_oihw, bias=None, stride=1, pad=0, dil=1, groups=1, relu=False, stats=None, winograd=False, x6=False, patch=False, _keep=None, **kw):
    _need_cuda(x, w_oihw)
    B, H, W, Cin = x.shape
    Cout, cin_g, k, _ = w_oihw.shape
    assert cin_g % 4 == 0 and Cin == cin_g * groups
    wp = pack_weight(w_oihw)
    Ho = (H + 2 * pad - dil * (k - 1) - 1) // stride + 1
    Wo = (W + 2 * pad - dil * (k - 1) - 1) // stride + 1
    out = torch.empty(B, Ho, Wo, Cout, device=x.device, dtype=torch.float32)
    U = winograd_weight(wp, groups, cin_g) if winograd else None
    X6 = x6_weight(wp, groups, cin_g, k * k, x6_tile(Cout // groups, groups, B * Ho * Wo)) if x6 else None
    if patch:
        kw['wgt_patch'] = patch_x6_weight(wp, cin_g)
        kw['flags'] = kw.get('flags', 0) | _lib.CONV_F16_OK | _lib.CONV_OUT_F32
    d, _, _ = make_conv_desc(x, wp, out, B=B, H=H, W=W, in_stride=Cin, cin_g=cin_g, Cout=Cout, groups=groups, k=k,
                             stride=stride, pad=pad, dil=dil, bias=bias, relu=relu, stats=stats, wgt_wino=U, wgt_x6=X6, **kw)
    if patch and lib.gssd_conv_patch_x6_takes(C.byref(d)) != 1:
        raise _lib.GssdError('conv2d_nhwc(patch=True): csrc/conv_patch_x6.hip does not take this descriptor')
    if x6 and lib.gssd_conv_x6_takes(C.byref(d)) != 1:
        raise _lib.GssdError('conv2d_nhwc(x6=True): csrc/conv_x6.hip does not take this descriptor')
    if _keep is not None:
        _keep.extend([d, wp, U, X6, kw.get('wgt_patch'), out])
        return d
    run_conv(d)
    return out


def conv_wgrad(desc, dy, Cout, cin_g_real, k, cin_g_pad=None, out=None, accumulate=False):
    cin_g_pad = cin_g_pad or desc.cin_g
    K = k * k * cin_g_pad
    dwp = torch.zeros(Cout, K, device=dy.device, dtype=torch.float32)
    check(lib.gssd_conv2d_wgrad_f32(C.byref(desc), _p(dy), _p(dwp), _stream()))
    if out is None:
        out = torch.empty(Cout, cin_g_real, k, k, device=dy.device, dtype=torch.float32)
    check(lib.gssd_unpack_conv_weight_grad(_p(dwp), _p(out), Cout, cin_g_real, k, k, cin_g_pad, K, int(accumulate), _stream()))
    return out


def pack_weight_dgrad(w_oihw, groups, out=None):
    w = w_oihw.detach().contiguous().float()
    Cout, cin_g, KH, KW = w.shape
    Kd = KH * KW * (Cout // groups)
    if out is None:
        out = torch.empty(groups * cin_g, Kd, device=w.device, dtype=torch.float32)
    check(lib.gssd_pack_conv_weight_dgrad(_p(w), _p(out), Cout, groups, cin_g, KH, KW, _stream()))
    return out


def bn_relu_pool(raw, out, stats, count, gamma, beta, rmean, rvar, training, relu=True, pool=None, momentum=0.1,
                 eps=1e-5, stats_rep=0):
    B, H, W, Cc = raw.shape
    _, Ho, Wo, _ = out.shape
    pk, ps, pp = pool if pool else (0, 1, 0)
    check(lib.gssd_bn_relu_pool_f32(_p(raw), _p(out), B, H, W, Cc, Ho, Wo, pk, ps, pp, _p(stats), float(count),
                                    _p(gamma), _p(beta), _p(rmean), _p(rvar), momentum, eps, int(training), int(relu),
                                    int(stats_rep), _stream()))
    return out


def bn_finalize(stats, count, gamma, beta, rmean, rvar, training, scale, shift, pad, momentum=0.1, eps=1e-5, stats_rep=0):
    check(lib.gssd_bn_finalize_f32(_p(stats), float(count), _p(gamma), _p(beta), _p(rmean), _p(rvar), momentum, eps,
                                   int(training), gamma.numel(), _p(scale), _p(shift), _p(pad), int(stats_rep), _stream()))


def pool_out_size(n, k, s, p, ceil):
    if ceil:
        o = -(-(n + 2 * p - k) // s) + 1
        if (o - 1) * s >= n + p:
            o -= 1
        return o
    return (n + 2 * p - k) // s + 1


def l2norm(x, weight, eps=1e-10, out=None):
    _need_cuda(x, weight)
    Cc = x.shape[-1]
    out = torch.empty_like(x) if out is None else out
    check(lib.gssd_l2norm_f32(_p(x), _p(weight), _p(out), x.numel() // Cc, Cc, eps, _stream()))
    return out


def softmax_rows_(x, n):
    rows = x.numel() // x.shape[-1]
    check(lib.gssd_softmax_rows_f32(_p(x), rows, n, x.shape[-1], _stream()))
    return x


def slice_and_cat(a, b, groups, out=None):
    _need_cuda(a, b)
    Ca, Cb = a.shape[-1], b.shape[-1]
    out = torch.empty(*a.shape[:-1], Ca + Cb, device=a.device, dtype=torch.float32) if out is None else out
    check(lib.gssd_slice_and_cat_f32(_p(a), _p(b), _p(out), a.numel() // Ca, Ca, Cb, groups, _stream()))
    return out


def sn_items_tensor(items, device):
    arr = (SnItem * len(items))()
    for i, (w, u, v, s) in enumerate(items):
        rows = w.shape[0]
        cols = w.numel() // rows
        if rows + cols > 4096:
            raise _lib.GssdError(f'spectral norm: rows + cols = {rows + cols} exceeds the kernel\'s 4096-float LDS vectors')
        arr[i].w, arr[i].u, arr[i].v, arr[i].inv_sigma, arr[i].rows, arr[i].cols = _p(w), _p(u), _p(v), _p(s), rows, cols
    raw = bytes(arr)
    return torch.frombuffer(bytearray(raw), dtype=torch.uint8).to(device)


def spectral_norm(items_dev, n, do_power_iteration, eps=1e-12):
    check(lib.gssd_spectral_norm_f32(_p(items_dev), n, int(do_power_iteration), eps, _stream()))


def dcn_im2col(x, om, cols, dg):
    B, H, W, Cc = x.shape
    check(lib.gssd_dcn_im2col_f32(_p(x), _p(om), _p(cols), B, H, W, Cc, dg, om.shape[-1], _stream()))
    return cols


def dcn_pack_weight(w_oihw, dg, out=None):
    _need_cuda(w_oihw)
    w = w_oihw.detach().contiguous().float()
    Cout, Cc = w.shape[0], w.shape[1]
    if out is None:
        n = int(lib.gssd_dcn_packed_weight_elems(Cout, Cc))
        if n <= 0:
            raise _lib.GssdError(f'deformable conv: unsupported shape C {Cc}, Cout {Cout}')
        out = torch.empty(n, device=w.device, dtype=torch.float32)
    check(lib.gssd_dcn_pack_weight_f32(_p(w), _p(out), Cout, Cc, dg, _stream()))
    return out


def dcn_forward(x, om, w_oihw, bias, dg, w_packed=None):
    _need_cuda(x, om, w_oihw)
    B, H, W, Cc = x.shape
    Cout = w_oihw.shape[0]
    wp = w_packed if w_packed is not None else dcn_pack_weight(w_oihw, dg)
    out = torch.empty(B, H, W, Cout, device=x.device, dtype=torch.float32)
    check(lib.gssd_dcn_forward_f32(_p(x), _p(om), _p(wp), _p(bias), _p(out), B, H, W, Cc, dg, om.shape[-1], Cout, _stream()))
    return out


def dcn_forward_x6(x, om, w_oihw, bias, dg, f16ok=False):
    _need_cuda(x, om, w_oihw)
    B, H, W, Cc = x.shape
    w = w_oihw.detach().contiguous().float()
    Cout = w.shape[0]
    n = int(lib.gssd_dcn_packed_weight_elems_x6(Cout, Cc))
    if n <= 0:
        raise _lib.GssdError(f'deformable conv (x6): unsupported shape C {Cc}, Cout {Cout}')
    wp = torch.empty(n, device=w.device, dtype=torch.bfloat16)
    check(lib.gssd_dcn_pack_weight_x6(_p(w), _p(wp), Cout, Cc, dg, _stream()))
    out = torch.empty(B, H, W, Cout, device=x.device, dtype=torch.float32)
    check(lib.gssd_dcn_forward_x6_ex(_p(x), _p(om), _p(wp), _p(bias), _p(out), B, H, W, Cc, dg, om.shape[-1], Cout,
                                     _lib.CONV_F16_OK if f16ok else 0, _stream()))
    return out


def dcn_col2im(x, om, dcols, dx, dom, dg):
    B, H, W, Cc = x.shape
    check(lib.gssd_dcn_col2im_f32(_p(x), _p(om), _p(dcols), _p(dx), _p(dom), B, H, W, Cc, dg, om.shape[-1], _stream()))
    return dx, dom


def softmax_lastdim(x):
    _need_cuda(x)
    x = x.contiguous().float()
    y = torch.empty_like(x)
    check(lib.gssd_softmax_lastdim_f32(_p(x), _p(y), x.numel() // x.shape[-1], x.shape[-1], _stream()))
    return y


def pack_targets(targets, device):
    ns = [int(t.shape[0]) for t in targets]
    if max(ns) > 64:
        raise _lib.GssdError('more than 64 ground-truth boxes in one image')
    off = [0]
    for n in ns:
        off.append(off[-1] + n)
    if all(t.is_cuda for t in targets):
        flat = torch.cat([t.detach().reshape(-1, 5) for t in targets], 0).to(device=device, dtype=torch.float32)
    else:
        flat = torch.cat([t.detach().to('cpu', torch.float32).reshape(-1, 5) for t in targets], 0).to(device)
    if flat.shape[0] == 0:
        flat = torch.zeros(1, 5, device=device)
    return flat.contiguous(), torch.tensor(off, dtype=torch.int32).to(device, non_blocking=True)


def match_batch(tg, gt_off, priors, threshold=0.5, variance=(0.1, 0.2)):
    _need_cuda(tg, gt_off, priors)
    B = gt_off.shape[0] - 1
    P = priors.shape[0]
    loc_t = torch.empty(B, P, 4, device=tg.device, dtype=torch.float32)
    conf_t = torch.empty(B, P, device=tg.device, dtype=torch.int64)
    check(lib.gssd_match_batch(_p(tg), _p(gt_off), _p(priors), B, P, threshold, variance[0], variance[1], _p(loc_t),
                               _p(conf_t), _stream()))
    return loc_t, conf_t


def multibox_loss_forward(loc, conf, priors, tg, n_gt, threshold=0.5, negpos_ratio=3, variance=(0.1, 0.2),
                          want_scores=False, global_n=False):
    _need_cuda(loc, conf, priors)
    loc = loc.contiguous()
    conf = conf.contiguous()
    B, P, _ = loc.shape
    Cc = conf.shape[-1]
    priors = priors[:P].contiguous()
    loc_t, conf_t = match_batch(tg, n_gt, priors, threshold, variance)
    dev = loc.device
    NX = 128
    xmax = torch.empty(NX, device=dev, dtype=torch.float32)
    check(lib.gssd_reduce_max_f32(_p(conf), conf.numel(), _p(xmax), NX, _stream()))
    sel = torch.empty(B, P, device=dev, dtype=torch.uint8)
    partial = torch.empty(B, 4, device=dev, dtype=torch.float64)
    lca = torch.empty(B, P, device=dev, dtype=torch.float32) if want_scores else None
    check(lib.gssd_hnm_loss(_p(loc), _p(conf), _p(loc_t), _p(conf_t), _p(xmax), NX, B, P, Cc, int(negpos_ratio), _p(sel),
                            _p(partial), _p(lca), _stream()))
    losses = torch.empty(2, device=dev, dtype=torch.float32)
    n_total = torch.empty(1, device=dev, dtype=torch.float64)
    check(lib.gssd_loss_finalize(_p(partial), B, _p(losses), _p(n_total), _stream()))
    if global_n:
        import torch.distributed as dist
        if dist.is_initialized() and dist.get_world_size() > 1:
            n_glob = n_total.clone()
            dist.all_reduce(n_glob, op=dist.ReduceOp.SUM)
            check(lib.gssd_loss_finalize_global(_p(partial), B, _p(n_glob), dist.get_world_size(), _p(losses), _p(n_total), _stream()))
    return dict(losses=losses, loc_t=loc_t, conf_t=conf_t, sel=sel, n_total=n_total, loss_c_all=lca, partial=partial,
                loc=loc, conf=conf)


def multibox_loss_backward(ctx, grad_l, grad_c):
    loc, conf = ctx['loc'], ctx['conf']
    B, P, _ = loc.shape
    Cc = conf.shape[-1]
    dloc = torch.empty_like(loc)
    dconf = torch.empty_like(conf)
    gl = grad_l.reshape(1).float().contiguous() if grad_l is not None else None
    gc = grad_c.reshape(1).float().contiguous() if grad_c is not None else None
    check(lib.gssd_loss_backward(_p(loc), _p(conf), _p(ctx['loc_t']), _p(ctx['conf_t']), _p(ctx['sel']),
                                 _p(ctx['n_total']), _p(gl), _p(gc), B, P, Cc, _p(dloc), _p(dconf), _stream()))
    if grad_l is None:
        dloc.zero_()
    if grad_c is None:
        dconf.zero_()
    return dloc, dconf


def detect(loc, conf, priors, num_classes, top_k=200, conf_thresh=0.01, nms_thresh=0.45, variance=(0.1, 0.2),
           conf_is_logits=False, want_keep=False, loc_is_boxes=False):
    _need_cuda(loc, conf, priors)
    if nms_thresh <= 0:
        raise ValueError('nms_threshold must be non negative.')
    loc = loc.contiguous().float()
    conf = conf.contiguous().float()
    priors = priors.contiguous().float()
    B, P, _ = loc.shape
    out = torch.empty(B, num_classes, top_k, 5, device=loc.device, dtype=torch.float32)
    keep = torch.empty(B, num_classes, top_k, device=loc.device, dtype=torch.int32) if want_keep else None
    cnt = torch.empty(B, num_classes, device=loc.device, dtype=torch.int32) if want_keep else None
    check(lib.gssd_detect(_p(loc), _p(conf), _p(priors), B, P, num_classes, top_k, conf_thresh, nms_thresh,
                          variance[0], variance[1], int(conf_is_logits), int(loc_is_boxes), _p(out), _p(keep), _p(cnt),
                          _stream()))
    return (out, keep, cnt) if want_keep else out


def detect_boxes(boxes, scores, overlap, top_k):
    _need_cuda(boxes, scores)
    n = boxes.shape[0]
    conf = torch.stack([torch.zeros_like(scores), scores], 1).unsqueeze(0).contiguous()
    out, keep, cnt = detect(boxes.unsqueeze(0), conf, boxes, 2, top_k=top_k, conf_thresh=0.0, nms_thresh=overlap,
                            want_keep=True, loc_is_boxes=True)
    return out[0, 1], keep[0, 1], cnt[0, 1]


def bn_backward(dout, raw, fwd_stats, count, gamma, scale, shift, pool=None, relu=True, eps=1e-5, want_colsum=False, stats_rep=0):
    B, H, W, Cc = raw.shape
    _, Ho, Wo, _ = dout.shape
    pk, ps, pp = pool if pool else (0, 1, 0)
    dev = raw.device
    dz = torch.zeros_like(raw) if (pool and ps < pk) else torch.empty_like(raw)
    sums = torch.zeros(2 * Cc, device=dev, dtype=torch.float64)
    check(lib.gssd_bn_bwd_reduce_f32(_p(dout), _p(raw), _p(scale), _p(shift), _p(dz), _p(sums), B, H, W, Cc, Ho, Wo, pk, ps, pp,
                                     int(relu), _stream()))
    ca, cb, cc, dg, db = (torch.empty(Cc, device=dev) for _ in range(5))
    check(lib.gssd_bn_bwd_finalize_f32(_p(fwd_stats), float(count), _p(sums), _p(gamma), eps, Cc, _p(ca), _p(cb), _p(cc), _p(dg),
                                       _p(db), int(stats_rep), _stream()))
    cs = torch.zeros(Cc, device=dev, dtype=torch.float64) if want_colsum else None
    check(lib.gssd_bn_bwd_apply_f32(_p(dz), _p(raw), _p(ca), _p(cb), _p(cc), B * H * W, Cc, _p(cs), _stream()))
    return dz, dg, db, cs


def l2norm_backward(x, weight, dy, dx_add=None, eps=1e-10):
    Cc = x.shape[-1]
    dx = torch.empty_like(x)
    dw = torch.zeros(Cc, device=x.device, dtype=torch.float64)
    check(lib.gssd_l2norm_bwd_f32(_p(x), _p(weight), _p(dy), _p(dx), _p(dx_add), _p(dw), x.numel() // Cc, Cc, eps, _stream()))
    return dx, dw
```

grouped-ssd-pytorch_amd/gssd/plan_common.py:

```python
import ctypes as C
import os
import torch
from . import _lib, ops
from ._lib import lib

VGG_CFG = [64, 64, 'M', 128, 128, 'M', 256, 256, 256, 'C', 512, 512, 512, 'M', 512, 512, 512]
EXTRAS_CFG = [256, 'S', 512, 128, 'S', 256, 128, 256, 128, 256]
MBOX = [4, 6, 6, 6, 4, 4]
SRC_HW = [38, 19, 10, 5, 3, 1]
HEAD_OFF = [sum(h * h * a for h, a in zip(SRC_HW[:i], MBOX[:i])) for i in range(6)]
FUSE_NAMES = ['11', '21', '31', '41', '51', '61']


USE_HEADS_WINO = os.environ.get('GSSD_HEADS_WINO', '1') != '0'
USE_PATCH_X6 = os.environ.get('GSSD_PATCH_X6', '1') != '0'
USE_CONV_X6 = os.environ.get('GSSD_CONV_X6', '1') != '0'
USE_WINOGRAD = os.environ.get('GSSD_NO_WINOGRAD', '0') != '1'
DCN_X6 = os.environ.get('GSSD_DCN_X6', '1') != '0'
USE_GRAPH = os.environ.get('GSSD_NO_GRAPH', '0') != '1'
USE_FLASH_X6 = os.environ.get('GSSD_FLASH_X6', '1') != '0'
USE_BRANCH_STREAMS = os.environ.get('GSSD_NO_BRANCH_STREAMS', '0') != '1'
FUSE_PACK = os.environ.get('GSSD_FUSE_PACK', '1') != '0'
FUSE_CAT = os.environ.get('GSSD_FUSE_CAT', '1') != '0'
FUSE_SPLIT = os.environ.get('GSSD_FUSE_SPLIT', '1') != '0'
FUSE_SA_BN = os.environ.get('GSSD_FUSE_SA_BN', '1') != '0'
FUSE_HEAD_BN = os.environ.get('GSSD_FUSE_HEAD_BN', '1') != '0'
SN_STREAM = 9
ALL_STREAMS = -1

class Tag(tuple):
    layer = None


class _Step:
    __slots__ = ('fn', 'args', 'keep', 'tag', 'sid', 'wait')

    def __init__(self, fn, args, keep=None, tag=None, sid=0, wait=None):
        self.fn, self.args, self.keep, self.tag, self.sid, self.wait = fn, args, keep, tag, sid, wait


def conv_tag(d, real_cin_g=None, bf16=False):
    cout_g = d.Cout // d.groups
    inst = '128x128' if cout_g > 64 else '128x64' if cout_g > 32 else '128x32' if cout_g > 16 else '128x16'
    if cout_g > 64:
        mt = -(-(d.Ho * d.Wo * (1 if d.m_per_image else d.B)) // 128)
        z = d.B if d.m_per_image else d.split_k
        b128 = mt * d.groups * (-(-cout_g // 128)) * z
        b64 = mt * d.groups * (-(-cout_g // 64)) * z
        e128 = b128 / (-(-b128 // 512) * 512)
        e64 = 0.94 * b64 / (-(-b64 // 768) * 768)
        if e64 > e128 or d.K <= 256:
            inst = '128x64'
    Ms, Mtot = d.Ho * d.Wo * (1 if d.m_per_image else d.B), d.Ho * d.Wo * d.B
    if (cout_g > 32 and d.split_k == 1 and Mtot <= 4096 and os.environ.get('GSSD_NO_SMALL_TILES') is None
            and not (d.out_mode == _lib.OUT_SPLIT_T and d.split_n % 64 != 0)):
        inst = '32x64' if (Mtot <= 512 or (d.m_per_image and Ms <= 128)) else '64x64'
    if (bf16 and os.environ.get('GSSD_BF16_BIG_TILES', '0') == '1' and not d.m_per_image and d.split_k == 1 and d.B * d.Ho * d.Wo >= 8192
            and cout_g % 128 == 0 and d.K % 64 == 0 and d.K >= 256
            and (d.out_mode == _lib.OUT_NHWC or (d.out_mode == _lib.OUT_SPLIT_T and d.split_n % 128 == 0))):
        inst = '256x128'
    name = ('conv_bf16<' if bf16 else 'conv_igemm<') + inst + '>'
    if not bf16 and d.wgt_patch and lib.gssd_conv_patch_x6_takes(C.byref(d)) == 1:
        M6 = d.B * d.Ho * d.Wo
        return ('conv_patch_x6<128>', 2.0 * M6 * d.Cout * 9 * d.cin_g, 4.0 * (d.B * d.H * d.W * d.cin_g + M6 * d.Cout + d.Cout * 9 * d.cin_g))
    if not bf16 and d.wgt_x6 and lib.gssd_conv_x6_takes(C.byref(d)) == 1:
        M6 = d.B * d.Ho * d.Wo
        flops = 2.0 * M6 * d.Cout * d.KH * d.KW * d.cin_g
        return (f'conv_x6<{ops.x6_tile(cout_g, d.groups, M6)}>', flops, 4.0 * (d.B * d.H * d.W * d.cin_g * d.groups + M6 * d.Cout + d.Cout * d.KH * d.KW * d.cin_g))
    if bf16:
        if (d.groups == 4 and d.KH == 3 and d.stride == 1 and d.pad == 1 and d.dil == 1 and d.H * d.W >= 75 * 75
                and (d.cin_g, cout_g) in ((8, 16), (16, 16), (16, 32), (32, 32)) and not d.m_per_image and d.split_k == 1
                and d.flags in (0, _lib.CONV_POOL2)):
            name = f'conv_thin_bf16<{d.cin_g},{cout_g}>' + ('/pool2' if d.flags & _lib.CONV_POOL2 else '')
    elif (d.groups == 4 and d.KH == 3 and d.stride == 1 and d.pad == 1 and d.dil == 1 and d.H * d.W >= 75 * 75
            and (d.cin_g, cout_g) in ((4, 16), (16, 16), (16, 32)) and not d.m_per_image and d.split_k == 1):
        name = f'conv_thin<{d.cin_g},{cout_g}>'
        if d.wgt_wino and (d.cin_g, cout_g) == (16, 32) and os.environ.get('GSSD_CONV21_WINO', '1') != '0':
            name = 'conv_wino<32>'
        if d.wgt_wino and (d.cin_g, cout_g) == (16, 16) and not d.resid:
            name = 'conv_thin_wino<16,16>'
    elif (d.wgt_wino and ops.winograd_eligible(d.KH, d.stride, d.pad, d.dil, d.cin_g, cout_g, d.groups) and not d.m_per_image
          and d.split_k <= 1 and not d.relu):
        name = f'conv_wino<{64 if (cout_g % 64 == 0 or (cout_g % 32 != 0 and cout_g > 32)) else 32}>'
    igemm_name = ('conv_bf16<' if bf16 else 'conv_igemm<') + inst + '>'
    if name.startswith('conv_wino<') and lib.gssd_conv_wino_x6_takes(C.byref(d)) == 1:
        name = f'conv_wino_x6<{64 if cout_g > 32 else 32}>'
    elif name.startswith('conv_wino<') and d.out_mode == _lib.OUT_HEADS:
        name = igemm_name
    if not bf16 and lib.gssd_conv_thin_x6_takes(C.byref(d)) == 1:
        name = f'conv_thin_x6<{d.cin_g},{cout_g}>'
    if name.startswith(('conv_wino<', 'conv_wino_x6<', 'conv_thin_x6<')):
        name += ('' if d.in_scale else '/plain') + ('/pool2' if d.flags & _lib.CONV_POOL2 else '')
    if bf16 and name.startswith('conv_bf16'):
        bm = lib.gssd_conv_flat_bf16_takes(C.byref(d))
        if bm:
            name = f'conv_flat_bf16<{d.cin_g},{min(cout_g, 128) if cout_g % 128 == 0 else 64},{bm}>'
    if not bf16 and name.startswith('conv_igemm') and lib.gssd_gemm_slot_takes(C.byref(d)) == 1:
        name = 'gemm_slot<128x128>'
    M = d.B * d.Ho * d.Wo
    cin_g = real_cin_g if real_cin_g is not None else d.cin_g
    flops = 2.0 * M * d.Cout * d.KH * d.KW * cin_g
    esz = 2.0 if bf16 else 4.0
    out_elems = M * d.Cout // 4 if (d.flags & _lib.CONV_POOL2) else M * d.Cout
    byts = esz * (d.B * d.H * d.W * cin_g * d.groups + out_elems + d.Cout * d.KH * d.KW * cin_g)
    return (name, flops, byts)
```

grouped-ssd-pytorch_amd/gssd/plan_graph.py:

```python
import ctypes as C
import os
import torch
from . import _lib, ops, plan_common
from ._lib import lib
from .plan_common import ALL_STREAMS, FUSE_NAMES, SN_STREAM, VGG_CFG


class PlanGraphMixin:
    def _place_branch0(self):
        if (os.environ.get('GSSD_BRANCH0_LATE', '1') == '0' or getattr(self, '_mark_conv7', None) is None
                or not self.eng.net.use_self_attention):
            return
        idx = [i for i, st in enumerate(self.steps) if st.sid == 1]
        if not idx or idx[-1] - idx[0] + 1 != len(idx) or idx[-1] >= self._mark_conv7:
            return
        a, b, c = idx[0], idx[-1] + 1, self._mark_conv7
        block = self.steps[a:b]
        self.steps[a:c] = self.steps[b:c] + block

    def _place_sn_step(self):
        sn = next((i for i, st in enumerate(self.steps) if st.sid == SN_STREAM), None)
        if sn is None or sn > self._pack_step:
            return
        st = self.steps.pop(sn)
        self._pack_step -= 1
        self.steps.insert(self._pack_step + 2, st)

    def _fuse_input_pack(self):
        i = self._pack_step
        if (not plan_common.FUSE_PACK or not getattr(self, 'nograd', False) or self.bf16 or i + 1 >= len(self.steps)
                or self.steps[i].fn is not lib.gssd_pack_input_nhwc):
            return
        st, x16_ptr = self.steps[i + 1], self.steps[i].args[1]
        d = st.keep
        if (st.fn is not lib.gssd_conv2d_nhwc_f32 or not isinstance(d, _lib.ConvDesc) or d.in_ != x16_ptr or st.wait is not None
                or lib.gssd_conv_thin_nchw3_takes(C.byref(d)) != 1):
            return
        d.flags |= _lib.CONV_IN_NCHW3
        del self.steps[i]
        self._reduce_steps = tuple(k - 1 for k in self._reduce_steps)
        self._pack_step, self._in_desc = None, d

    def _set_input(self, ptr):
        d = self.__dict__.get('_in_desc')
        if d is not None:
            d.in_ = ptr
        else:
            self.steps[self._pack_step].args[0] = ptr

    def _build_bn_graph(self, x16):
        net = self.eng.net
        g = net.groups_vgg
        cur, H, Cc = x16, 300, self.cpad * g
        vi = 0
        cfg = list(VGG_CFG)
        i = 0
        x43 = None
        xf = None
        while i < len(cfg):
            v = cfg[i]
            assert v not in ('M', 'C')
            conv, bn = net.vgg[vi], net.vgg[vi + 1]
            pool = None
            nxt = cfg[i + 1] if i + 1 < len(cfg) else None
            is_conv4_3 = (vi == 30)
            last = (i == len(cfg) - 1)
            if nxt in ('M', 'C') and not is_conv4_3:
                pool = (2, 2, 0, nxt == 'C')
            if last:
                pool = (3, 1, 1, False)
            defer = (pool is None and not is_conv4_3) or (is_conv4_3 and self._sa_base_reads_raw(H, conv.out_channels))
            cur, H, Cc, xf = self._conv_bn(f'vgg.{vi}', conv, bn, cur, H, Cc, g, relu=True, pool=pool, in_xf=xf,
                                           defer_bn=defer)
            vi += 3
            if nxt in ('M', 'C'):
                vi += 1
                i += 1
            i += 1
            if is_conv4_3:
                x43 = cur
                cur, H, Cc, src0 = self._after_conv4_3(cur, H, Cc, xf)
                xf = None
        vi += 1
        xf = None
        for li in range(2):
            conv, bn = net.vgg[vi], net.vgg[vi + 1]
            cur, H, Cc, xf = self._conv_bn(f'vgg.{vi}', conv, bn, cur, H, Cc, g, relu=True, in_xf=xf, defer_bn=(li == 0))
            vi += 3
        sources = [src0]
        self._mark_conv7 = len(self.steps)
        sab_i, sa_i = 1, 1
        if net.use_self_attention_base:
            cur, _ = self._self_attn('self_attn_base_list', sab_i, cur, H, Cc, need_out2=False, want_map=self.want_maps)
            sab_i += 1
        sources.append(self._branch(cur, H, Cc, sa_i, '21'))
        sa_i += 1
        ge = net.groups_extra
        n_ex = len(net.extras)
        fi = 2
        xf = None
        for k in range(0, n_ex, 2):
            conv, bn = net.extras[k], net.extras[k + 1]
            cur, H, Cc, xf = self._conv_bn(f'extras.{k}', conv, bn, cur, H, Cc, ge, relu=True, in_xf=xf,
                                           defer_bn=((k + 1) % 4 != 3))
            if (k + 1) % 4 == 3:
                if net.use_self_attention_base:
                    cur, _ = self._self_attn('self_attn_base_list', sab_i, cur, H, Cc, need_out2=False, want_map=self.want_maps)
                    sab_i += 1
                sources.append(self._branch(cur, H, Cc, sa_i, FUSE_NAMES[fi]))
                sa_i += 1
                fi += 1
        self.sources = sources

    def _build_plain_graph(self, x16):
        net = self.eng.net
        g, ge = net.groups_vgg, net.groups_extra
        cur, H, Cc = x16, 300, self.cpad * g
        mods = list(net.vgg)
        i = 0
        src0 = None
        while i < len(mods):
            m = mods[i]
            if isinstance(m, torch.nn.Conv2d):
                cur, H, Cc = self._conv_act(f'vgg.{i}', m, cur, H, Cc, g)
                i += 2
                if i - 2 == 21:
                    cur, H, Cc, src0 = self._after_conv4_3(cur, H, Cc)
                    i += 1
            else:
                cur, H = self._pool_only(cur, H, Cc, m.kernel_size, m.stride, m.padding, m.ceil_mode)
                i += 1
        sources = [src0]
        sab_i, sa_i = 1, 1
        if net.use_self_attention_base:
            cur, _ = self._self_attn('self_attn_base_list', sab_i, cur, H, Cc, need_out2=False, want_map=self.want_maps)
            sab_i += 1
        sources.append(self._branch(cur, H, Cc, sa_i, '21'))
        sa_i += 1
        fi = 2
        for k, m in enumerate(net.extras):
            cur, H, Cc = self._conv_act(f'extras.{k}', m, cur, H, Cc, ge)
            if k % 2 == 1:
                if net.use_self_attention_base:
                    cur, _ = self._self_attn('self_attn_base_list', sab_i, cur, H, Cc, need_out2=False, want_map=self.want_maps)
                    sab_i += 1
                sources.append(self._branch(cur, H, Cc, sa_i, FUSE_NAMES[fi]))
                sa_i += 1
                fi += 1
        self.sources = sources

    def _finish_heads(self):
        B, dev = self.B, self.dev
        smax = max(d.split_k for d in self.head_descs)
        splits = torch.ones(self.P, dtype=torch.int8)
        off = 0
        for d in self.head_descs:
            A = d.split_n // 4
            n = d.Ho * d.Wo * A
            splits[off:off + n] = d.split_k
            off += n
        assert off == self.P
        self._head_splits = splits.to(dev)
        self._ws_loc = torch.empty(smax, B, self.P, 4, device=dev, dtype=torch.float32)
        self._ws_conf = torch.empty(smax, B, self.P, self.nc, device=dev, dtype=torch.float32)
        for d in self.head_descs:
            d.out, d.out_b = self._ws_loc.data_ptr(), self._ws_conf.data_ptr()
            d.flags |= _lib.CONV_HEADS_SLICES
        prev, self._sid = getattr(self, '_sid', 0), 0
        self._pending_wait = ALL_STREAMS
        self._reduce_steps = (len(self.steps), len(self.steps) + 1)
        self._add(lib.gssd_heads_reduce_f32, [self._ws_loc.data_ptr(), self._head_splits.data_ptr(), 0, B, self.P, 4])
        self._add(lib.gssd_heads_reduce_f32, [self._ws_conf.data_ptr(), self._head_splits.data_ptr(), 0, B, self.P, self.nc])
        self._sid = prev

    def _set_outputs(self, loc, conf):
        self.steps[self._reduce_steps[0]].args[2] = loc.data_ptr()
        self.steps[self._reduce_steps[1]].args[2] = conf.data_ptr()

    def _sa_base_reads_raw(self, H, Cc):
        net = self.eng.net
        return bool(plan_common.FUSE_SA_BN and getattr(self, 'nograd', False) and not self.bf16 and not self.want_maps
                    and net.use_self_attention_base and Cc <= 512 and (Cc // 4) % 64 == 0 and all(self._sa_on_x6(H, Cc)))

    def _after_conv4_3(self, x, H, Cc, xf=None):
        net, B = self.eng.net, self.B
        attn_g, cat_g = None, 0
        if net.use_self_attention_base:
            cat_g = (net.groups_vgg if (plan_common.FUSE_CAT and getattr(self, 'nograd', False) and not self.bf16 and net.use_dcn
                                        and net.dcn_cat_sab) else 0)
            x, attn_g = self._self_attn('self_attn_base_list', 0, x, H, Cc, need_out2=bool(net.dcn_cat_sab), want_map=self.want_maps,
                                        cat_groups=cat_g, in_xf=xf)
        if net.use_dcn:
            xin, Cin = x, Cc
            if net.dcn_cat_sab and cat_g and attn_g is None:
                xin, Cin = x, 2 * Cc
            elif net.dcn_cat_sab:
                xc = self._abuf(B, H, H, 2 * Cc)
                esz = 2 if self.bf16 else 1
                self._add(lib.gssd_slice_and_cat_f32, (x.data_ptr(), attn_g.data_ptr(), xc.data_ptr(), B * H * H, Cc // esz, Cc // esz,
                                                       net.groups_vgg))
                self.rec.append(('slice_cat', dict(a=x, b=attn_g, out=xc, H=H, Ca=Cc, Cb=Cc, groups=net.groups_vgg,
                                                   detach_b=bool(net.detach_sab))))
                xin, Cin = xc, 2 * Cc
            for li in range(net.num_dcn_layers):
                xin, Cin = self._dcn(li, xin, H, Cin)
            x, Cc = xin, Cin
        self.x_after_block = x
        s = self._abuf(B, H, H, Cc)
        self._sid = 1
        self._add(lib.gssd_l2norm_bf16 if self.bf16 else lib.gssd_l2norm_f32,
                  (x.data_ptr(), net.L2Norm.weight.data_ptr(), s.data_ptr(), B * H * H, Cc, float(net.L2Norm.eps)))
        self.rec.append(('l2norm', dict(x_in=x, out=s, H=H, C=Cc, mod=net.L2Norm)))
        self._sid = 0
        src0 = self._branch(s, H, Cc, 0, '11')
        self._layer = 'vgg.33'
        pooled, Hp = self._pool_only(x, H, Cc, 2, 2, 0)
        self._layer = None
        return pooled, Hp, Cc, src0

    def _branch(self, s, H, Cc, sa_i, fuse):
        net = self.eng.net
        xf = None
        prev, self._sid = getattr(self, '_sid', 0), sa_i + 1
        if net.use_self_attention:
            s, _ = self._self_attn('self_attn_list', sa_i, s, H, Cc, need_out2=False, want_map=self.want_maps)
        if net.use_fuseconv and net.batch_norm:
            conv, bn = getattr(net, f'fuse_{fuse}'), getattr(net, f'bn_fuse_{fuse}')
            defer = bool(plan_common.FUSE_HEAD_BN and getattr(self, 'nograd', False) and not self.bf16 and not self.want_maps
                         and conv.out_channels <= 512)
            s, H, Cc, xf = self._conv_bn(f'fuse_{fuse}', conv, bn, s, H, Cc, 1, relu=True, defer_bn=defer)
        elif net.use_fuseconv:
            s, H, Cc = self._conv_act(f'fuse_{fuse}', getattr(net, f'fuse_{fuse}'), s, H, Cc, 1)
        self._head(sa_i, s, H, Cc, in_xf=xf)
        self._sid = prev
        self.__dict__.setdefault('sources_xf', {})[sa_i] = xf
        return (s, H, Cc)
```

grouped-ssd-pytorch_amd/layers/modules/multibox_loss.py:

```python
import torch
import torch.nn as nn

from gssd import ops
from data.config import v2 as cfg


class _MultiBoxLossFn(torch.autograd.Function):
    @staticmethod
    def forward(ctx, loc, conf, priors, tg, n_gt, threshold, negpos_ratio, variance, global_n=False):
        st = ops.multibox_loss_forward(loc.detach(), conf.detach(), priors, tg, n_gt, threshold, negpos_ratio,
                                       variance, global_n=global_n)
        ctx.st = st
        losses = st['losses']
        return losses[0], losses[1]

    @staticmethod
    def backward(ctx, g_l, g_c):
        dloc, dconf = ops.multibox_loss_backward(ctx.st, g_l, g_c)
        return dloc, dconf, None, None, None, None, None, None, None


class MultiBoxLoss(nn.Module):
    def __init__(self, num_classes, overlap_thresh, prior_for_matching, bkg_label, neg_mining, neg_pos, neg_overlap,
                 encode_target, use_gpu=True):
        super().__init__()
        self.use_gpu = use_gpu
        self.num_classes = num_classes
        self.threshold = overlap_thresh
        self.background_label = bkg_label
        self.encode_target = encode_target
        self.use_prior_for_matching = prior_for_matching
        self.do_neg_mining = neg_mining
        self.negpos_ratio = neg_pos
        self.neg_overlap = neg_overlap
        self.variance = cfg['variance']
        self.global_normalizer = False

    def forward(self, predictions, targets):
        loc_data, conf_data, priors = predictions
        P = loc_data.size(1)
        priors = priors[:P, :]
        if priors.device != loc_data.device:
            priors = priors.to(loc_data.device)
        tg, n_gt = ops.pack_targets(targets, loc_data.device)
        return _MultiBoxLossFn.apply(loc_data, conf_data, priors.detach().contiguous(), tg, n_gt, float(self.threshold),
                                     int(self.negpos_ratio), (float(self.variance[0]), float(self.variance[1])),
                                     bool(self.global_normalizer))
```

include/gssd_hip.h:

```cpp
#ifndef GSSD_HIP_H
#define GSSD_HIP_H

#include <stdint.h>

#ifdef __cplusplus
extern "C" {
#endif

#define GSSD_OK 0
#define GSSD_EINVAL (-1)
#define GSSD_ELAUNCH (-2)

typedef void* gssd_stream_t;

int gssd_abi_version(void);
int gssd_conv_desc_size(void);
const char* gssd_last_error(void);
const char* gssd_build_arch(void);

typedef void* gssd_event_t;
int gssd_event_create(gssd_event_t* ev);
int gssd_event_destroy(gssd_event_t ev);
int gssd_event_record_node(gssd_event_t ev, gssd_stream_t stream);
int gssd_event_elapsed_ms(gssd_event_t start, gssd_event_t stop, float* ms);


int gssd_pack_input_nhwc(const float* x_nchw, float* y_nhwc, int B, int C, int H, int W, int groups,
                         int cpg_out, gssd_stream_t stream);

int gssd_unpack_nhwc_to_nchw(const float* x_nhwc, float* y_nchw, int B, int C, int H, int W, int x_stride,
                             gssd_stream_t stream);

int gssd_pack_conv_weight(const float* w_oihw, float* w_packed, int Cout, int cin_g, int KH, int KW,
                          int cin_g_pad, int Kpad, gssd_stream_t stream);

typedef struct gssd_pack_item {
    const float* w;
    float* wp;
    int32_t Cout, cin_g, taps, cin_g_pad, Kpad, reserved;
} gssd_pack_item;
int gssd_pack_conv_weights_batched(const gssd_pack_item* items_dev, int n_items, gssd_stream_t stream);

#define GSSD_OUT_NHWC 0
#define GSSD_OUT_TRANSPOSED 1
#define GSSD_OUT_HEADS 2
#define GSSD_OUT_SPLIT_T 3

typedef struct gssd_conv_desc {
    const float* in;
    const float* wgt;
    const float* bias;
    float* out;
    float* out_b;
    const float* alpha;
    const float* gate;
    const float* resid;
    float* out2;
    const float* in_scale;
    const float* in_shift;
    const float* in_pad;
    double* stats;
    const float* wgt_wino;
    const float* pool_sign;
    const void* wgt_x6;
    const void* wgt_patch;
    int B, H, W;
    int in_stride;
    int in_ch_off;
    int Ho, Wo;
    int Cout, groups;
    int cin_g;
    int KH, KW, stride, pad, dil;
    int K;
    int wgt_row_stride;
    int out_stride;
    int out_ch_off;
    int out_mode;
    int relu;
    int m_per_image;
    int split_n;
    int split_k;
    int out_b_stride;
    int flags;
    int stats_rep;
    int64_t in_batch_stride, wgt_batch_stride, out_batch_stride, outb_batch_stride;
    int64_t out_off, outb_off;
} gssd_conv_desc;

int gssd_conv2d_nhwc_f32(const gssd_conv_desc* d, gssd_stream_t stream);

int gssd_conv_x6_tile(int cout_g, int groups, long long M);
long long gssd_conv_x6_weight_elems(int Cout, int groups, int cin_g, int taps, int BN);
int gssd_conv_x6_pack_weight(const float* w_packed, void* w_x6, int Cout, int groups, int cin_g, int taps, int row_stride, int BN,
                             gssd_stream_t stream);
int gssd_conv_x6_takes(const gssd_conv_desc* d);

#define GSSD_CONV_OUT_F32 1
#define GSSD_CONV_OUTB_BF16_PERM32 2
#define GSSD_CONV_HEADS_SLICES 4
#define GSSD_CONV_POOL2 8
#define GSSD_CONV_RESID_F32 16
#define GSSD_CONV_F16_OK 32
#define GSSD_CONV_IN_NCHW3 64
#define GSSD_CONV_OUT_GROUPCAT 128
#define GSSD_CONV_OUT_X6PLANES 256
#define GSSD_CONV_RESID_XF 512
int gssd_conv2d_nhwc_bf16(const gssd_conv_desc* d, gssd_stream_t stream);
int gssd_pack_conv_weight_bf16(const float* w_oihw, void* w_packed, int Cout, int cin_g, int KH, int KW, int cin_g_pad, int Kpad,
                               gssd_stream_t stream);
int gssd_cast_f32_bf16(const float* x, void* y, int64_t n, gssd_stream_t stream);
int gssd_cast_bf16_f32(const void* x, float* y, int64_t n, gssd_stream_t stream);
int gssd_pack_input_nhwc_bf16(const float* x_nchw, void* y_nhwc, int B, int C, int H, int W, int groups, gssd_stream_t stream);
int gssd_bn_relu_pool_bf16(const void* raw, void* out, int B, int H, int W, int C, int Ho, int Wo, int pool_k, int pool_s, int pool_p,
                           const double* stats, double count, const float* gamma, const float* beta, float* running_mean,
                           float* running_var, float momentum, float eps, int training, int relu, int stats_rep,
                           gssd_stream_t stream);
int gssd_bn_finalize_bf16(const double* stats, double count, const float* gamma, const float* beta, float* running_mean,
                          float* running_var, float momentum, float eps, int training, int C, float* scale, float* shift,
                          void* pad_bf16, int stats_rep, gssd_stream_t stream);
int gssd_l2norm_bf16(const void* x, const float* weight, void* out, int64_t pixels, int C, float eps, gssd_stream_t stream);

long long gssd_winograd_weight_elems(int Cout, int groups, int cin_g);
int gssd_winograd_weight_f32(const float* w_packed, float* U, int Cout, int groups, int cin_g, int row_stride,
                             gssd_stream_t stream);

int gssd_conv2d_wgrad_f32(const gssd_conv_desc* d, const float* dy, float* dw_packed, gssd_stream_t stream);
int gssd_conv2d_wgrad_bf16(const gssd_conv_desc* d, const void* dy, float* dw_packed, gssd_stream_t stream);
int gssd_conv2d_wgrad_bf16_supported(const gssd_conv_desc* d);
int gssd_unpack_conv_weight_grad(const float* w_packed, float* w_oihw, int Cout, int cin_g, int KH, int KW,
                                 int cin_g_pad, int Kpad, int accumulate, gssd_stream_t stream);
int gssd_pack_conv_weight_dgrad(const float* w_oihw, float* w_packed, int Cout, int groups, int cin_g, int KH, int KW,
                                gssd_stream_t stream);

int gssd_bn_relu_pool_f32(const float* raw, float* out, int B, int H, int W, int C, int Ho, int Wo, int pool_k,
                          int pool_s, int pool_p, const double* stats, double count, const float* gamma,
                          const float* beta, float* running_mean, float* running_var, float momentum, float eps,
                          int training, int relu, int stats_rep, gssd_stream_t stream);

int gssd_bn_finalize_f32(const double* stats, double count, const float* gamma, const float* beta,
                         float* running_mean, float* running_var, float momentum, float eps, int training, int C,
                         float* scale, float* shift, float* pad, int stats_rep, gssd_stream_t stream);

int gssd_bn_bwd_reduce_f32(const float* dout, const float* raw, const float* scale, const float* shift, float* dz,
                           double* sums, int B, int H, int W, int C, int Ho, int Wo, int pool_k, int pool_s, int pool_p,
                           int relu, gssd_stream_t stream);
int gssd_bn_bwd_finalize_f32(const double* fwd_stats, double count, const double* bwd_sums, const float* gamma, float eps,
                             int C, float* coef_a, float* coef_b, float* coef_c, float* dgamma, float* dbeta,
                             int stats_rep, gssd_stream_t stream);
int gssd_bn_bwd_apply_f32(float* dz, const float* raw, const float* coef_a, const float* coef_b, const float* coef_c,
                          int64_t pixels, int C, double* colsum, gssd_stream_t stream);
int gssd_bn_bwd_reduce_mixed(const void* dout, int dout_bf16, const void* raw_bf16, const float* scale, const float* shift, float* dz,
                             void* dz_bf16, double* sums, int B, int H, int W, int C, int Ho, int Wo, int pool_k, int pool_s, int pool_p,
                             int relu, gssd_stream_t stream);
int gssd_bn_bwd_apply_mixed(const void* dout, int dout_bf16, float* dz, void* dz_bf16, const void* raw_bf16, const float* scale,
                            const float* shift, int relu, const float* coef_a, const float* coef_b, const float* coef_c, int64_t pixels,
                            int C, double* colsum, int store_f32, gssd_stream_t stream);
int gssd_bn_bwd_apply_masked_f32(const float* dout, const float* raw, const float* scale, const float* shift, int relu,
                                 const float* coef_a, const float* coef_b, const float* coef_c, float* draw, int64_t pixels, int C,
                                 double* colsum, gssd_stream_t stream);
int gssd_colsum_f32(const float* x, int64_t rows, int C, int row_stride, double* out, gssd_stream_t stream);
int gssd_cast_f64_f32(const double* x, float* y, int n, int accumulate, gssd_stream_t stream);
int gssd_l2norm_bwd_f32(const float* x, const float* weight, const float* dy, float* dx, const float* dx_add,
                        double* dweight, int64_t pixels, int C, float eps, gssd_stream_t stream);
int gssd_heads_gather_f32(const float* dloc, const float* dconf, float* out, int B, int HW, int A, int nc, int P,
                          int prior_off, gssd_stream_t stream);
int gssd_upsample_insert_f32(const float* dy, float* u, int B, int Ho, int Wo, int H, int W, int C, int s,
                             gssd_stream_t stream);

int gssd_l2norm_f32(const float* x, const float* weight, float* out, int64_t pixels, int C, float eps,
                    gssd_stream_t stream);

int gssd_self_attn_core_f32(const float* tp, const float* gT, void* out, int B, int N, int Np, int D, int C2, int out_bf16,
                            gssd_stream_t stream);

int gssd_self_attn_core_kv_f32(const float* tp, const float* kp, const float* gT, void* out, int B, int N, int Nk, int Nkp, int D,
                               int C2, int kstride, int out_bf16, float* lse, gssd_stream_t stream);

int gssd_sa_pool_kv_f32(const float* tp, const float* gT, float* kp, float* gTp, int B, int H, int P, int C8, int C2, int Np, int Nkp,
                        gssd_stream_t stream);

int gssd_sa_unpool_f32(const float* dkg, float* dst, int B, int H, int P, int CW, int ld, gssd_stream_t stream);

int gssd_gemm_slot_takes(const gssd_conv_desc* d);

int gssd_conv_flat_bf16_takes(const gssd_conv_desc* d);
int gssd_conv_flat_bf16_tile(int pixels_per_workgroup);

int gssd_self_attn_core_bf16v(const float* tp, const void* gT_bf16, void* out_bf16, int B, int N, int Np32, int D, int C2,
                              float* lse, gssd_stream_t stream);

int gssd_self_attn_flash_bwd_bf16(const float* tp, const void* tp_bf16, const void* tp_bf16_lo, const void* g_bf16, const void* dag_bf16,
                                  const float* lse, const float* dvec, float* dtpg, int B, int N, int D, int C2, gssd_stream_t stream);
int gssd_self_attn_flash_bwd_supported(int D, int C2);

int gssd_softmax_rows_f32(float* x, int64_t rows, int n, int row_stride, gssd_stream_t stream);

int gssd_slice_and_cat_f32(const float* a, const float* b, float* out, int64_t pixels, int Ca, int Cb,
                           int groups, gssd_stream_t stream);

typedef struct gssd_sn_item {
    const float* w;
    float* u;
    float* v;
    float* inv_sigma;
    int rows, cols;
} gssd_sn_item;
int gssd_spectral_norm_f32(const gssd_sn_item* items_dev, int n, int do_power_iteration, float eps,
                           gssd_stream_t stream);

int gssd_dcn_im2col_f32(const float* x, const float* om, float* cols, int B, int H, int W, int C, int dg,
                        int om_stride, gssd_stream_t stream);
int gssd_dcn_im2col_bf16(const void* x_bf16, const float* om, void* cols_bf16, int B, int H, int W, int C, int dg, int om_stride,
                         gssd_stream_t stream);

long long gssd_dcn_packed_weight_elems(int Cout, int C);
int gssd_dcn_pack_weight_f32(const float* w_oihw, float* w_packed, int Cout, int C, int dg, gssd_stream_t stream);
int gssd_dcn_forward_f32(const float* x, const float* om, const float* w_packed, const float* bias, float* out, int B, int H,
                         int W, int C, int dg, int om_stride, int Cout, gssd_stream_t stream);
int gssd_dcn_streamk(int mode);
#define GSSD_DCN_SK_UNSUPPORTED 1
#define GSSD_DCN_SK_MAPPING 2
#define GSSD_DCN_SK_TIMEOUT 4
int gssd_dcn_streamk_status(unsigned* xcc_map);
int gssd_dcn_streamk_reset(gssd_stream_t stream);
int gssd_dcn_streamk_release(const void* out);

long long gssd_dcn_packed_weight_elems_x6(int Cout, int C);
int gssd_dcn_pack_weight_x6(const float* w_oihw, void* w_packed, int Cout, int C, int dg, gssd_stream_t stream);
int gssd_dcn_forward_x6(const float* x, const float* om, const void* w_packed, const float* bias, float* out, int B, int H, int W, int C,
                        int dg, int om_stride, int Cout, gssd_stream_t stream);
long long gssd_conv_patch_x6_weight_elems(int Cout, int C);
int gssd_conv_patch_x6_pack_weight(const float* w_packed, void* out, int Cout, int C, int row_stride, gssd_stream_t stream);
int gssd_conv_patch_x6_takes(const gssd_conv_desc* d);
int gssd_dcn_forward_x6_ex(const float* x, const float* om, const void* w_packed, const float* bias, float* out, int B, int H, int W, int C,
                           int dg, int om_stride, int Cout, int flags, gssd_stream_t stream);
long long gssd_dcn_packed_weight_elems_bf16(int Cout, int C);
int gssd_dcn_pack_weight_bf16(const float* w_oihw, void* w_packed, int Cout, int C, int dg, gssd_stream_t stream);
int gssd_dcn_forward_bf16(const void* x, const float* om, const void* w_packed, const float* bias, void* out, int B, int H, int W,
                          int C, int dg, int om_stride, int Cout, gssd_stream_t stream);

int gssd_dcn_col2im_f32(const float* x, const float* om, const float* dcols, float* dx, float* dom, int B, int H, int W,
                        int C, int dg, int om_stride, gssd_stream_t stream);

typedef struct gssd_dcn_geom {
    int32_t B, H, W, C, x_stride;
    int32_t Ho, Wo;
    int32_t kh, kw, sh, sw, ph, pw, dh, dw;
    int32_t dg;
    int32_t off_stride, mask_stride;
    int32_t mask_logit;
} gssd_dcn_geom;
int gssd_dcn_geo_im2col_f32(const float* x, const float* offset, const float* mask, float* cols, const gssd_dcn_geom* geom, int b0,
                            int b1, gssd_stream_t stream);
int gssd_dcn_geo_col2im_f32(const float* x, const float* offset, const float* mask, const float* dcols, float* dx, float* doffset,
                            float* dmask, const gssd_dcn_geom* geom, int b0, int b1, gssd_stream_t stream);

#define GSSD_FILTER_BILINEAR 2
#define GSSD_FILTER_BICUBIC 3

int gssd_resample_ksize(int in_size, int out_size, int filter);
int gssd_resample_coeffs(int in_size, int out_size, int filter, int32_t* bounds, int32_t* kk);

int gssd_resize_u8_horizontal(const uint8_t* in, uint8_t* out, const int32_t* bounds, const int32_t* kk, int ksize,
                              int n_img, int H, int W_in, int W_out, int C, gssd_stream_t stream);
int gssd_resize_u8_vertical(const uint8_t* in, uint8_t* out, const int32_t* bounds, const int32_t* kk, int ksize, int n_img,
                            int H_in, int H_out, int W, int C, int imgs_per_study, int32_t* minmax, gssd_stream_t stream);

int gssd_input_finish_f32(const uint8_t* img, const int32_t* minmax, float mean0, float mean1, float mean2, float* out_nchw,
                          int B, int phases, int S, int C, int normalize, gssd_stream_t stream);

typedef struct gssd_aug_desc {
    int64_t src;
    int64_t work;
    int32_t H, W;
    int32_t s_phase, s_chan, s_y, s_x;
    int32_t top, left;
    int32_t cy, cx, ch, cw;
    int32_t mirror;
    int32_t fill;
    float delta, alpha;
    int32_t hb, hk, hks;
    int32_t vb, vk, vks;
    int32_t row0, nrows;
} gssd_aug_desc;
int gssd_aug_desc_size(void);

int gssd_augment_minmax(const gssd_aug_desc* desc, int B, int max_rows, int p_only, int32_t* minmax, gssd_stream_t stream);
int gssd_augment_horizontal(const gssd_aug_desc* desc, const int32_t* minmax, const int32_t* table, float mean0, float mean1,
                            float mean2, uint8_t* work, int B, int max_rows, int max_cw, int size, int p_only, gssd_stream_t stream);
int gssd_augment_vertical(const gssd_aug_desc* desc, const int32_t* table, const uint8_t* work, float* out_nchw, int B, int size,
                          int p_only, gssd_stream_t stream);

int gssd_pixellink_targets(const float* boxes, const int32_t* offsets, int B, int size, int factor, int64_t* pixel_mask,
                           int64_t* neg_pixel_mask, float* pixel_pos_weight, int64_t* link_mask, gssd_stream_t stream);

int gssd_bgemm_f32(const float* A, const float* B, float* C, int M, int N, int K, int lda, int ldb, int ldc, int transA, int transB,
                   long long strideA, long long strideB, long long strideC, int batch, float alpha, int accumulate,
                   gssd_stream_t stream);
int gssd_bgemm_ex_f32(const float* A, const float* B, float* C, int M, int N, int K, int lda, int ldb, int ldc, int transA, int transB,
                      long long strideA, long long strideB, long long strideC, int batch, float alpha, int mode, const float* rowvec,
                      const float* aux, gssd_stream_t stream);
int gssd_rowdot_f32(const float* a, const float* b, float* out, int64_t rows, int C, gssd_stream_t stream);
int gssd_softmax_bwd_rows_f32(const float* attn, float* dattn, int64_t rows, int n, int row_stride, gssd_stream_t stream);
int gssd_sn_weight_grad_f32(const float* dw_eff, int ld_dw, const float* w_orig, const float* u, const float* v, const float* inv_sigma,
                            const float* scale, double* dot_scratch , float* dw_orig, int rows, int cols,
                            gssd_stream_t stream);
int gssd_scaled_transpose_f32(const float* w, const float* alpha, float* out, int rows, int cols, gssd_stream_t stream);
int gssd_cast_split_f32_bf16(const float* x, void* hi, void* lo, int64_t n, gssd_stream_t stream);
int gssd_cast_rows_f32_bf16(const float* x, void* y, int64_t rows, int cols, int ld_x, int ld_y, gssd_stream_t stream);
int gssd_transpose_cast_f32_bf16(const float* x, void* y, int64_t rows, int cols, int64_t ld_x, int64_t ld_y, gssd_stream_t stream);
int gssd_dot_f32(const float* a, const float* b, int64_t n, double* out, gssd_stream_t stream);
int gssd_axpby_f32(const float* x, const float* y, float* out, int64_t n, float a, float b, gssd_stream_t stream);
int gssd_scale_cast_f64_f32(const double* x, const float* scale, float* y, int n, gssd_stream_t stream);
int gssd_sa_sigma_grad_f32(const double* dot, const double* colsum, const float* bias, int C, float* dsigma, gssd_stream_t stream);


int gssd_match_batch(const float* targets, const int* gt_off, const float* priors, int B, int P,
                     float threshold, float var0, float var1, float* loc_t, int64_t* conf_t, gssd_stream_t stream);

int gssd_reduce_max_f32(const float* x, int64_t n, float* out, int out_n, gssd_stream_t stream);

int gssd_hnm_loss(const float* loc, const float* conf, const float* loc_t, const int64_t* conf_t, const float* xmax,
                  int xmax_n, int B, int P, int C, int negpos_ratio, uint8_t* sel, double* partial, float* loss_c_all,
                  gssd_stream_t stream);
int gssd_loss_finalize(const double* partial, int B, float* losses, double* n_total, gssd_stream_t stream);
int gssd_loss_finalize_global(const double* partial, int B, const double* n_global, int world, float* losses, double* n_total,
                              gssd_stream_t stream);
int gssd_loss_backward(const float* loc, const float* conf, const float* loc_t, const int64_t* conf_t,
                       const uint8_t* sel, const double* n_total, const float* grad_l, const float* grad_c, int B,
                       int P, int C, float* dloc, float* dconf, gssd_stream_t stream);

int gssd_detect(const float* loc, const float* conf, const float* priors, int B, int P, int C, int top_k,
                float conf_thresh, float nms_thresh, float var0, float var1, int conf_is_logits, int loc_is_boxes,
                float* out, int* keep_idx, int* keep_cnt, gssd_stream_t stream);

int gssd_softmax_lastdim_f32(const float* x, float* y, int64_t rows, int C, gssd_stream_t stream);


int gssd_eval_match(const float* det, long long img_stride, int N, int top_k, const float* scales, const double* gt,
                    const int* gt_off, int max_gt, double thresh, const double* thr, int n_iou, int n_iobb, float* conf_out,
                    uint8_t* flag_out, gssd_stream_t stream);

long long gssd_eval_workspace_bytes(int M);
int gssd_eval_ap(const float* conf, const uint8_t* flags, int M, int n_metrics, double npos, int use_07_metric, void* workspace,
                 long long workspace_bytes, double* ap_out, gssd_stream_t stream);

int gssd_heads_reduce_f32(const float* ws, const signed char* splits, float* out, int B, int P, int C, gssd_stream_t stream);


int gssd_interp_add_f32(const float* src, const float* addend, float* out, float* out2, int B, int Hs, int Ws, int Hd, int Wd, int C,
                        gssd_stream_t stream);

int gssd_pixellink_final_f32(const float* f0, const float* f1, const float* f2, const float* f3, int nf, const float* w1,
                             const float* b1, const float* w2, const float* b2, float* out1, float* out2, int B, int HW,
                             gssd_stream_t stream);

int gssd_pixellink_loss_f32(const float* out1, const float* out2, const long long* pixel_target, const unsigned char* neg_pixel_mask,
                            const float* pixel_pos_weight, const long long* link_target, double* per_image, float* neg_weight_out,
                            int B, int H, int W, int neg_pos_ratio, gssd_stream_t stream);

int gssd_interp_add_bwd_f32(const float* d_out, const float* d_out2, float* d_src, float* d_addend, int B, int Hs, int Ws, int Hd, int Wd,
                            int C, int ld, gssd_stream_t stream);
int gssd_pixellink_final_bwd_f32(const float* d_out1, const float* d_out2, const float* f0, const float* f1, const float* f2,
                                 const float* f3, int nf, const float* w1, const float* w2, float* g0, float* g1, float* g2, float* g3,
                                 int accumulate_mask, double* dw1, double* dw2, int B, int HW, int ld, gssd_stream_t stream);
int gssd_pixellink_loss_bwd_f32(const float* out1, const float* out2, const long long* pixel_target, const float* neg_weight,
                                const float* pixel_pos_weight, const long long* link_target, const double* per_image,
                                const float* upstream4, float* d_out1, float* d_out2, int B, int H, int W, gssd_stream_t stream);

int gssd_pixellink_decode_f32(const float* out1, const float* out2, int* labels, float* comps, int* ncomp, int B, int H, int W,
                              float pixel_thr, float link_thr, int max_comp, gssd_stream_t stream);

int gssd_pixellink_final5_f32(const float* f0, const float* f1, const float* f2, const float* f3, const float* f4, int nf, const float* w1,
                              const float* b1, const float* w2, const float* b2, float* out1, float* out2, int B, int HW, gssd_stream_t stream);
int gssd_pixellink_final5_bwd_f32(const float* d_out1, const float* d_out2, const float* f0, const float* f1, const float* f2, const float* f3,
                                  const float* f4, int nf, const float* w1, const float* w2, float* g0, float* g1, float* g2, float* g3,
                                  float* g4, int accumulate_mask, double* dw1, double* dw2, int B, int HW, int ld, gssd_stream_t stream);

int gssd_self_attn_flash_bwd_f32_supported(int D, int C2);
int gssd_self_attn_flash_bwd_f32(const float* tp, int qstride, const float* keys, int krow, const float* gT, int Nkp, const float* dag,
                                 const float* lse, const float* dvec, float* dq, int ld_q, float* dk, float* dv, int ld_kv, int B, int N, int Nk,
                                 int D, int C2, gssd_stream_t stream);

int gssd_self_attn_core_x6_supported(int D, int C2);
long long gssd_self_attn_core_x6_ws_bytes(int B, int N, int D, int C2);
int gssd_self_attn_core_x6_f32(const float* tp, const float* gT, float* out, int B, int N, int Np, int D, int C2, void* ws, float* lse,
                               gssd_stream_t stream);
int gssd_self_attn_core_x6_planes_f32(const void* ws, float* out, int B, int N, int D, int C2, float* lse, gssd_stream_t stream);

#define GSSD_PLAN_LAUNCH 0
#define GSSD_PLAN_WAIT 1
#define GSSD_PLAN_MAX_ARGS 24
typedef struct gssd_plan_op {
    int kind;
    int fn;
    int stream;
    int nargs;
    uint64_t args[GSSD_PLAN_MAX_ARGS];
} gssd_plan_op;
int gssd_plan_fn_count(void);
const char* gssd_plan_fn_name(int index);
int gssd_plan_fn_index(const char* name);
int gssd_plan_fn_nargs(int index);
int gssd_plan_op_size(void);
int gssd_plan_run(const gssd_plan_op* ops, int n_ops, const gssd_stream_t* streams, int n_streams, int* failed_at);

int gssd_conv_wino_x6_takes(const gssd_conv_desc* d);
int gssd_conv_thin_x6_takes(const gssd_conv_desc* d);
int gssd_conv_thin_nchw3_takes(const gssd_conv_desc* d);

#ifdef __cplusplus
}
#endif
#endif
```

Baseline: 4710 img/s.

## Fuse multibox loss match/HNM/finalize kernels and merge heads reduce launches

Replaces the match_batch, reduce_max, hnm_loss and loss_finalize sequence with a fused two-stage path. Prior matching is sliced across blocks and also computes per-slice conf maxima, and a per-image hard-negative-mining kernel does a radix select and finalizes the loss through a ticket. It also merges the two heads-reduce launches (loc and conf) into one kernel with vectorized loads. The aim is fewer kernel launches and fewer passes over conf/loc_t in the loss tail, at the cost of more complex kernels and new workspace handling.

Measured after the change: 4789 img/s (median of 6 runs). +1.7%, better.

```diff
diff --git a/grouped-ssd-pytorch_amd/gssd/_lib.py b/grouped-ssd-pytorch_amd/gssd/_lib.py
--- a/grouped-ssd-pytorch_amd/gssd/_lib.py
+++ b/grouped-ssd-pytorch_amd/gssd/_lib.py
@@ -119,6 +119,7 @@
     'gssd_conv_flat_bf16_takes': (c_i, [c_fp]),
     'gssd_conv_flat_bf16_tile': (c_i, [c_i]),
     'gssd_heads_reduce_f32': (c_i, [c_fp, c_fp, c_fp, c_i, c_i, c_i, c_fp]),
+    'gssd_heads_reduce2_f32': (c_i, [c_fp, c_fp, c_fp, c_fp, c_fp, c_i, c_i, c_i, c_fp]),
     'gssd_interp_add_f32': (c_i, [c_fp, c_fp, c_fp, c_fp, c_i, c_i, c_i, c_i, c_i, c_i, c_fp]),
     'gssd_pixellink_final_f32': (c_i, [c_fp, c_fp, c_fp, c_fp, c_i, c_fp, c_fp, c_fp, c_fp, c_fp, c_fp, c_i, c_i, c_fp]),
     'gssd_pixellink_loss_f32': (c_i, [c_fp, c_fp, c_fp, c_fp, c_fp, c_fp, c_fp, c_fp, c_i, c_i, c_i, c_i, c_fp]),
@@ -190,6 +191,9 @@
     'gssd_reduce_max_f32': (c_i, [c_fp, c_i64, c_fp, c_i, c_fp]),
     'gssd_hnm_loss': (c_i, [c_fp, c_fp, c_fp, c_fp, c_fp, c_i, c_i, c_i, c_i, c_i, c_fp, c_fp, c_fp, c_fp]),
     'gssd_loss_finalize': (c_i, [c_fp, c_i, c_fp, c_fp, c_fp]),
+    'gssd_multibox_loss_workspace_bytes': (C.c_longlong, [c_i]),
+    'gssd_multibox_loss_forward_f32': (c_i, [c_fp, c_fp, c_fp, c_fp, c_fp, c_i, c_i, c_i, c_f, c_f, c_f, c_i, c_fp, c_fp, c_fp, c_fp,
+                                             c_fp, c_fp, c_fp, c_fp, C.c_longlong, c_fp]),
     'gssd_loss_finalize_global': (c_i, [c_fp, c_i, c_fp, c_i, c_fp, c_fp, c_fp]),
     'gssd_loss_backward': (c_i, [c_fp, c_fp, c_fp, c_fp, c_fp, c_fp, c_fp, c_fp, c_i, c_i, c_i, c_fp, c_fp, c_fp]),
     'gssd_detect': (c_i, [c_fp, c_fp, c_fp, c_i, c_i, c_i, c_i, c_f, c_f, c_f, c_f, c_i, c_i, c_fp, c_fp, c_fp, c_fp]),
diff --git a/grouped-ssd-pytorch_amd/gssd/csrc/elementwise.hip b/grouped-ssd-pytorch_amd/gssd/csrc/elementwise.hip
--- a/grouped-ssd-pytorch_amd/gssd/csrc/elementwise.hip
+++ b/grouped-ssd-pytorch_amd/gssd/csrc/elementwise.hip
@@ -391,6 +391,47 @@
     }
 }
 
+template <int CV>
+__device__ __forceinline__ void heads_reduce_rows(const float* __restrict__ ws, const signed char* __restrict__ splits,
+                                                  float* __restrict__ out, int rows, int P, int C, int block, int nblocks) {
+    const size_t total = (size_t)rows * C;
+    for (int r = block * 256 + threadIdx.x; r < rows; r += nblocks * 256) {
+        const int n = splits[r % P];
+        if constexpr (CV == 4) {
+            float4 a = reinterpret_cast<const float4*>(ws)[r];
+            for (int k = 1; k < n; ++k) {
+                const float4 t = reinterpret_cast<const float4*>(ws + (size_t)k * total)[r];
+                a.x += t.x; a.y += t.y; a.z += t.z; a.w += t.w;
+            }
+            reinterpret_cast<float4*>(out)[r] = a;
+        } else if constexpr (CV == 2) {
+            float2 a = reinterpret_cast<const float2*>(ws)[r];
+            for (int k = 1; k < n; ++k) {
+                const float2 t = reinterpret_cast<const float2*>(ws + (size_t)k * total)[r];
+                a.x += t.x; a.y += t.y;
+            }
+            reinterpret_cast<float2*>(out)[r] = a;
+        } else {
+            for (int c = 0; c < C; ++c) {
+                const size_t i = (size_t)r * C + c;
+                float a = ws[i];
+                for (int k = 1; k < n; ++k) a += ws[(size_t)k * total + i];
+                out[i] = a;
+            }
+        }
+    }
+}
+
+template <int CV>
+__global__ __launch_bounds__(256) void heads_reduce2_kernel(const float* __restrict__ ws_loc, const float* __restrict__ ws_conf,
+                                                           const signed char* __restrict__ splits, float* __restrict__ loc,
+                                                           float* __restrict__ conf, int rows, int P, int C, int blocks_loc) {
+    if ((int)blockIdx.x < blocks_loc)
+        heads_reduce_rows<4>(ws_loc, splits, loc, rows, P, 4, blockIdx.x, blocks_loc);
+    else
+        heads_reduce_rows<CV>(ws_conf, splits, conf, rows, P, C, blockIdx.x - blocks_loc, gridDim.x - blocks_loc);
+}
+
 }
 
 extern "C" int gssd_pack_input_nhwc(const float* x, float* y, int B, int C, int H, int W, int groups, int cpg_out,
@@ -520,3 +561,23 @@
     GSSD_CHECK_LAUNCH();
     return GSSD_OK;
 }
+
+extern "C" int gssd_heads_reduce2_f32(const float* ws_loc, const float* ws_conf, const signed char* splits, float* loc, float* conf, int B,
+                                      int P, int C, gssd_stream_t stream) {
+    GSSD_CHECK_ARG(ws_loc && ws_conf && splits && loc && conf && B > 0 && P > 0 && C > 0);
+    GSSD_CHECK_ARG((long long)B * P < (1ll << 30));
+    GSSD_CHECK_ARG(((uintptr_t)ws_loc % 16) == 0 && ((uintptr_t)loc % 16) == 0);
+    const int rows = B * P;
+    int blocks = (rows + 255) / 256;
+    if (blocks > 4096) blocks = 4096;
+    const uintptr_t ca = (uintptr_t)ws_conf | (uintptr_t)conf | (uintptr_t)((size_t)rows * C * sizeof(float));
+    const dim3 grid(2 * blocks), block(256);
+    if (C == 4 && ca % 16 == 0)
+        hipLaunchKernelGGL(heads_reduce2_kernel<4>, grid, block, 0, as_stream(stream), ws_loc, ws_conf, splits, loc, conf, rows, P, C, blocks);
+    else if (C == 2 && ca % 8 == 0)
+        hipLaunchKernelGGL(heads_reduce2_kernel<2>, grid, block, 0, as_stream(stream), ws_loc, ws_conf, splits, loc, conf, rows, P, C, blocks);
+    else
+        hipLaunchKernelGGL(heads_reduce2_kernel<0>, grid, block, 0, as_stream(stream), ws_loc, ws_conf, splits, loc, conf, rows, P, C, blocks);
+    GSSD_CHECK_LAUNCH();
+    return GSSD_OK;
+}
diff --git a/grouped-ssd-pytorch_amd/gssd/csrc/loss.hip b/grouped-ssd-pytorch_amd/gssd/csrc/loss.hip
--- a/grouped-ssd-pytorch_amd/gssd/csrc/loss.hip
+++ b/grouped-ssd-pytorch_amd/gssd/csrc/loss.hip
@@ -290,6 +290,382 @@
         losses[0] = (float)(l / n);
         losses[1] = (float)(c / n);
         *n_total = n;
+    }
+}
+
+constexpr int MS = GSSD_MULTIBOX_SLICES;
+constexpr int MT = 512;
+constexpr int MK = 6;
+constexpr int MAX_CH = 36;
+
+__device__ __forceinline__ unsigned long long wave_max_u64(unsigned long long k) {
+#pragma unroll
+    for (int o = 32; o > 0; o >>= 1) {
+        const unsigned long long t = __shfl_xor(k, o, 64);
+        k = t > k ? t : k;
+    }
+    return k;
+}
+
+__device__ __forceinline__ unsigned long long match_key(float v, int p) {
+    unsigned u = (v == 0.f) ? 0u : __float_as_uint(v);
+    u = (u & 0x80000000u) ? ~u : (u | 0x80000000u);
+    return ((unsigned long long)u << 32) | (unsigned)~p;
+}
+
+__global__ __launch_bounds__(MT) void match_slice_kernel(const float* __restrict__ targets, const int* __restrict__ gt_off,
+                                                         const float* __restrict__ priors, const float* __restrict__ conf, int P, int C,
+                                                         float thr, float var0, float var1, float* __restrict__ loc_t,
+                                                         int64_t* __restrict__ conf_t, float* __restrict__ pmax) {
+    extern __shared__ __attribute__((aligned(16))) unsigned char smraw[];
+    __shared__ float gt[MAX_GT][5];
+    __shared__ float gt_area[MAX_GT];
+    __shared__ unsigned long long best_key[MAX_GT];
+    __shared__ int best_prior[MAX_GT];
+    __shared__ float red_m[MT / 64];
+
+    const int s = blockIdx.x, b = blockIdx.y, tid = threadIdx.x, lane = tid & 63;
+    const int chunk = (P + MS - 1) / MS;
+    const int p0 = min(s * chunk, P), p1 = min(p0 + chunk, P);
+    float* s_bv = reinterpret_cast<float*>(smraw);
+    int* s_bj = reinterpret_cast<int*>(s_bv + chunk);
+
+    const int g0 = gt_off[b];
+    int n = gt_off[b + 1] - g0;
+    if (n > MAX_GT) n = MAX_GT;
+    if (tid < 5) gt[0][tid] = 0.f;
+    if (tid < MAX_GT) best_key[tid] = 0ull;
+    for (int q = p0 + tid; q < p1; q += MT) {
+        s_bv[q - p0] = -INFINITY;
+        s_bj[q - p0] = 0;
+    }
+    __syncthreads();
+    for (int i = tid; i < n * 5; i += MT) gt[i / 5][i % 5] = targets[(size_t)g0 * 5 + i];
+    __syncthreads();
+    if (tid < n) gt_area[tid] = (gt[tid][2] - gt[tid][0]) * (gt[tid][3] - gt[tid][1]);
+    __syncthreads();
+
+    for (int base = 0; base < P; base += MT * MK) {
+        float px1[MK], py1[MK], px2[MK], py2[MK];
+#pragma unroll
+        for (int k = 0; k < MK; ++k) {
+            const int p = base + k * MT + tid;
+            const float4 pr = p < P ? reinterpret_cast<const float4*>(priors)[p] : make_float4(0.f, 0.f, 0.f, 0.f);
+            const float hx = pr.z / 2.f, hy = pr.w / 2.f;
+            px1[k] = pr.x - hx;
+            py1[k] = pr.y - hy;
+            px2[k] = pr.x + hx;
+            py2[k] = pr.y + hy;
+        }
+        for (int j = 0; j < n; ++j) {
+            const float gx1 = gt[j][0], gy1 = gt[j][1], gx2 = gt[j][2], gy2 = gt[j][3], ga = gt_area[j];
+            float bv = -INFINITY;
+            int bi = 0x7fffffff;
+#pragma unroll
+            for (int k = 0; k < MK; ++k) {
+                const int p = base + k * MT + tid;
+                if (p < P) {
+                    const float v = iou_pf(gx1, gy1, gx2, gy2, ga, px1[k], py1[k], px2[k], py2[k]);
+                    if (v > bv) {
+                        bv = v;
+                        bi = p;
+                    }
+                    if (p >= p0 && p < p1 && v > s_bv[p - p0]) {
+                        s_bv[p - p0] = v;
+                        s_bj[p - p0] = j;
+                    }
+                }
+            }
+            unsigned long long key = (bi == 0x7fffffff) ? 0ull : match_key(bv, bi);
+            key = wave_max_u64(key);
+            if (lane == 0 && key) atomicMax(&best_key[j], key);
+        }
+    }
+    __syncthreads();
+    if (tid < n) best_prior[tid] = best_key[tid] ? (int)~(unsigned)best_key[tid] : 0;
+    __syncthreads();
+
+    for (int p = p0 + tid; p < p1; p += MT) {
+        const float4 pr = reinterpret_cast<const float4*>(priors)[p];
+        float bv = s_bv[p - p0];
+        int bj = s_bj[p - p0];
+        int f = -1;
+        for (int j = 0; j < n; ++j)
+            if (best_prior[j] == p) f = j;
+        if (f >= 0) {
+            bv = 2.f;
+            bj = f;
+        }
+        int64_t cf = (int64_t)(gt[bj][4] + 1.f);
+        if (bv < thr) cf = 0;
+        conf_t[(size_t)b * P + p] = cf;
+        const float gx1 = gt[bj][0], gy1 = gt[bj][1], gx2 = gt[bj][2], gy2 = gt[bj][3];
+        float4 o;
+        o.x = __fdiv_rn(((gx1 + gx2) / 2.f) - pr.x, var0 * pr.z);
+        o.y = __fdiv_rn(((gy1 + gy2) / 2.f) - pr.y, var0 * pr.w);
+        o.z = __fdiv_rn((float)log((double)__fdiv_rn(gx2 - gx1, pr.z)), var1);
+        o.w = __fdiv_rn((float)log((double)__fdiv_rn(gy2 - gy1, pr.w)), var1);
+        reinterpret_cast<float4*>(loc_t)[(size_t)b * P + p] = o;
+    }
+
+    const float* cs = conf + ((size_t)b * P + p0) * C;
+    const int len = (p1 - p0) * C;
+    int head = (int)(((16u - (unsigned)((uintptr_t)cs & 15u)) & 15u) >> 2);
+    if (head > len) head = len;
+    float m = -INFINITY;
+    if (tid < head) m = cs[tid];
+    const int n4 = (len - head) >> 2;
+    for (int i = tid; i < n4; i += MT) {
+        const float4 v = reinterpret_cast<const float4*>(cs + head)[i];
+        m = fmaxf(fmaxf(m, fmaxf(v.x, v.y)), fmaxf(v.z, v.w));
+    }
+    for (int i = head + (n4 << 2) + tid; i < len; i += MT) m = fmaxf(m, cs[i]);
+    m = wave_max(m);
+    if (lane == 0) red_m[tid >> 6] = m;
+    __syncthreads();
+    if (tid == 0) {
+        for (int w = 1; w < MT / 64; ++w) m = fmaxf(m, red_m[w]);
+        pmax[b * MS + s] = m;
+    }
+}
+
+__device__ unsigned radix_select_desc_scan(const float* vals, int n, int k, unsigned (*hist)[256], int* n_greater) {
+    const int tid = threadIdx.x, lane = tid & 63;
+    unsigned prefix = 0, mask = 0;
+    int greater = 0;
+    for (int pass = 0; pass < 4; ++pass) {
+        const int shift = 24 - 8 * pass;
+        unsigned* h = hist[pass];
+        for (int base = 0; base < n; base += LT) {
+            const int i = base + tid;
+            bool act = false;
+            unsigned d = 0;
+            if (i < n) {
+                const unsigned u = __float_as_uint(vals[i]);
+                act = (u & mask) == prefix;
+                d = (u >> shift) & 255u;
+            }
+            unsigned long long peers = __ballot(act);
+            if (peers == 0ull) continue;
+#pragma unroll
+            for (int bit = 0; bit < 8; ++bit) {
+                const bool on = (d >> bit) & 1u;
+                const unsigned long long bb = __ballot(act && on);
+                peers &= on ? bb : ~bb;
+            }
+            if (act && lane == __ffsll((long long)peers) - 1) atomicAdd(&h[d], (unsigned)__popcll(peers));
+        }
+        __syncthreads();
+        const uint4 c = reinterpret_cast<const uint4*>(h)[lane];
+        const int sum4 = (int)(c.x + c.y + c.z + c.w);
+        int incl = sum4;
+#pragma unroll
+        for (int o = 1; o < 64; o <<= 1) {
+            const int t = __shfl_down(incl, o, 64);
+            if (lane + o < 64) incl += t;
+        }
+        const int above = greater + incl - sum4;
+        const int cum3 = above + (int)c.w, cum2 = cum3 + (int)c.z, cum1 = cum2 + (int)c.y, cum0 = cum1 + (int)c.x;
+        const int reach = wave_sum((int)(cum3 >= k) + (int)(cum2 >= k) + (int)(cum1 >= k) + (int)(cum0 >= k));
+        const int bin = reach > 0 ? reach - 1 : 0;
+        const int r = bin & 3;
+        const int before = r == 3 ? above : (r == 2 ? cum3 : (r == 1 ? cum2 : cum1));
+        greater = __shfl(before, bin >> 2, 64);
+        prefix |= ((unsigned)bin) << shift;
+        mask |= 255u << shift;
+    }
+    *n_greater = greater;
+    return prefix;
+}
+
+__global__ __launch_bounds__(LT) void hnm_fused_kernel(const float* __restrict__ loc, const float* __restrict__ conf,
+                                                       const float* __restrict__ loc_t, const int64_t* __restrict__ conf_t,
+                                                       const float* __restrict__ pmax, int pmax_n, int P, int C, int negpos_ratio,
+                                                       uint8_t* __restrict__ sel, double* partial, float* __restrict__ lca_out,
+                                                       unsigned* ticket, int B, float* __restrict__ losses,
+                                                       double* __restrict__ n_total) {
+    extern __shared__ __attribute__((aligned(16))) unsigned char smraw[];
+    float* lca = reinterpret_cast<float*>(smraw);
+    __shared__ __attribute__((aligned(16))) unsigned hist[4][256];
+    __shared__ int s_cnt[LT / 64];
+    __shared__ float s_max[LT / 64];
+    __shared__ double s_red[LT / 64][2];
+    __shared__ int s_tie[MAX_CH * (LT / 64)];
+    __shared__ int s_last;
+
+    const int b = blockIdx.x, tid = threadIdx.x, lane = tid & 63, wave = tid >> 6;
+    float xmax = -INFINITY;
+    for (int i = tid; i < pmax_n; i += LT) xmax = fmaxf(xmax, pmax[i]);
+    xmax = wave_max(xmax);
+    if (lane == 0) s_max[wave] = xmax;
+    reinterpret_cast<unsigned*>(hist)[tid] = 0u;
+    __syncthreads();
+    xmax = s_max[0];
+    for (int w = 1; w < LT / 64; ++w) xmax = fmaxf(xmax, s_max[w]);
+    const float* cb = conf + (size_t)b * P * C;
+    const int64_t* tb = conf_t + (size_t)b * P;
+
+    int npos = 0;
+    int t_n = 0;
+    float c_n[4] = {0.f, 0.f, 0.f, 0.f};
+    auto fetch = [&](int q) {
+        if (q < P) {
+            t_n = (int)tb[q];
+#pragma unroll
+            for (int c = 0; c < 4; ++c)
+                if (c < C) c_n[c] = cb[(size_t)q * C + c];
+        }
+    };
+    fetch(tid);
+    for (int p = tid; p < P; p += LT) {
+        const int t = t_n;
+        const float cv[4] = {c_n[0], c_n[1], c_n[2], c_n[3]};
+        fetch(p + LT);
+        float s = 0.f;
+#pragma unroll
+        for (int c = 0; c < 4; ++c)
+            if (c < C) s += (float)exp((double)(cv[c] - xmax));
+        for (int c = 4; c < C; ++c) s += (float)exp((double)(cb[(size_t)p * C + c] - xmax));
+        const float xt = t == 0 ? cv[0] : (t == 1 ? cv[1] : (t == 2 ? cv[2] : (t == 3 ? cv[3] : cb[(size_t)p * C + t])));
+        float v = ((float)log((double)s) + xmax) - xt;
+        if (t > 0) {
+            v = 0.f;
+            ++npos;
+        }
+        if (!(v > 0.f)) v = 0.f;
+        lca[p] = v;
+    }
+    npos = wave_sum(npos);
+    if (lane == 0) s_cnt[wave] = npos;
+    __syncthreads();
+    npos = 0;
+    for (int w = 0; w < LT / 64; ++w) npos += s_cnt[w];
+    int num_neg = negpos_ratio * npos;
+    if (num_neg > P - 1) num_neg = P - 1;
+    if (lca_out)
+        for (int p = tid; p < P; p += LT) lca_out[(size_t)b * P + p] = lca[p];
+
+    unsigned kth_bits = 0xffffffffu;
+    int n_greater = 0;
+    const int nch = (P + LT - 1) / LT;
+    if (num_neg > 0) {
+        kth_bits = radix_select_desc_scan(lca, P, num_neg, hist, &n_greater);
+        for (int k = 0; k < nch; ++k) {
+            const int p = k * LT + tid;
+            const unsigned long long bal = __ballot(p < P && __float_as_uint(lca[p < P ? p : 0]) == kth_bits);
+            if (lane == 0) s_tie[k * (LT / 64) + wave] = __popcll(bal);
+        }
+        __syncthreads();
+        if (wave == 0) {
+            const int ntot = nch * (LT / 64), per = (ntot + 63) / 64;
+            int sum = 0;
+            for (int e = 0; e < per; ++e) {
+                const int idx = lane * per + e;
+                if (idx < ntot) sum += s_tie[idx];
+            }
+            int incl = sum;
+#pragma unroll
+            for (int o = 1; o < 64; o <<= 1) {
+                const int t = __shfl_up(incl, o, 64);
+                if (lane >= o) incl += t;
+            }
+            int run = incl - sum;
+            for (int e = 0; e < per; ++e) {
+                const int idx = lane * per + e;
+                if (idx < ntot) {
+                    const int v = s_tie[idx];
+                    s_tie[idx] = run;
+                    run += v;
+                }
+            }
+        }
+        __syncthreads();
+    }
+    const int ties_needed = num_neg - n_greater;
+
+    double sum_l = 0.0, sum_c = 0.0;
+    for (int k = 0; k < nch; ++k) {
+        const int p = k * LT + tid;
+        bool is_tie = false, take = false, pos = false;
+        if (p < P) {
+            const unsigned u = __float_as_uint(lca[p]);
+            pos = tb[p] > 0;
+            if (num_neg > 0) {
+                if (u > kth_bits) take = true;
+                else if (u == kth_bits) is_tie = true;
+            }
+        }
+        const unsigned long long bal = __ballot(is_tie);
+        if (is_tie && s_tie[k * (LT / 64) + wave] + __popcll(bal & ((1ull << lane) - 1ull)) < ties_needed) take = true;
+        if (p < P) {
+            const uint8_t code = pos ? 1 : (take ? 2 : 0);
+            const bool neg_flag = take;
+            sel[(size_t)b * P + p] = pos ? (uint8_t)(neg_flag ? 3 : 1) : code;
+            if (pos) {
+                const float4 a = reinterpret_cast<const float4*>(loc)[(size_t)b * P + p];
+                const float4 t4 = reinterpret_cast<const float4*>(loc_t)[(size_t)b * P + p];
+                const float d[4] = {a.x - t4.x, a.y - t4.y, a.z - t4.z, a.w - t4.w};
+#pragma unroll
+                for (int e = 0; e < 4; ++e) {
+                    const float ad = fabsf(d[e]);
+                    sum_l += (double)(ad < 1.f ? 0.5f * d[e] * d[e] : ad - 0.5f);
+                }
+            }
+            if (pos || take) {
+                const int t = (int)tb[p];
+                float m = cb[(size_t)p * C];
+                for (int c = 1; c < C; ++c) m = fmaxf(m, cb[(size_t)p * C + c]);
+                double s = 0.0;
+                for (int c = 0; c < C; ++c) s += exp((double)(cb[(size_t)p * C + c] - m));
+                sum_c += (log(s) + (double)m) - (double)cb[(size_t)p * C + t];
+            }
+        }
+    }
+    sum_l = wave_sum(sum_l);
+    sum_c = wave_sum(sum_c);
+    if (lane == 0) {
+        s_red[wave][0] = sum_l;
+        s_red[wave][1] = sum_c;
+    }
+    __syncthreads();
+    unsigned long long* part = reinterpret_cast<unsigned long long*>(partial);
+    if (tid == 0) {
+        double l = 0.0, c = 0.0;
+        for (int w = 0; w < LT / 64; ++w) {
+            l += s_red[w][0];
+            c += s_red[w][1];
+        }
+        __hip_atomic_store(part + (size_t)b * 4 + 0, (unsigned long long)__double_as_longlong(l), __ATOMIC_RELAXED, __HIP_MEMORY_SCOPE_AGENT);
+        __hip_atomic_store(part + (size_t)b * 4 + 1, (unsigned long long)__double_as_longlong(c), __ATOMIC_RELAXED, __HIP_MEMORY_SCOPE_AGENT);
+        __hip_atomic_store(part + (size_t)b * 4 + 2, (unsigned long long)__double_as_longlong((double)npos), __ATOMIC_RELAXED,
+                           __HIP_MEMORY_SCOPE_AGENT);
+        __hip_atomic_store(part + (size_t)b * 4 + 3, (unsigned long long)__double_as_longlong((double)num_neg), __ATOMIC_RELAXED,
+                           __HIP_MEMORY_SCOPE_AGENT);
+        asm volatile("s_waitcnt vmcnt(0)" ::: "memory");
+        const unsigned t = __hip_atomic_fetch_add(ticket, 1u, __ATOMIC_RELAXED, __HIP_MEMORY_SCOPE_AGENT);
+        s_last = (t == (unsigned)(B - 1)) ? 1 : 0;
+    }
+    __syncthreads();
+    if (s_last && wave == 0) {
+        double l = 0.0, c = 0.0, n = 0.0;
+        for (int base = 0; base < B; base += 64) {
+            const int bb = base + lane < B ? base + lane : B - 1;
+            const double vl = __longlong_as_double((long long)__hip_atomic_load(part + (size_t)bb * 4 + 0, __ATOMIC_RELAXED, __HIP_MEMORY_SCOPE_AGENT));
+            const double vc = __longlong_as_double((long long)__hip_atomic_load(part + (size_t)bb * 4 + 1, __ATOMIC_RELAXED, __HIP_MEMORY_SCOPE_AGENT));
+            const double vn = __longlong_as_double((long long)__hip_atomic_load(part + (size_t)bb * 4 + 2, __ATOMIC_RELAXED, __HIP_MEMORY_SCOPE_AGENT));
+            const int cnt = B - base < 64 ? B - base : 64;
+            for (int i = 0; i < cnt; ++i) {
+                l += __shfl(vl, i, 64);
+                c += __shfl(vc, i, 64);
+                n += __shfl(vn, i, 64);
+            }
+        }
+        if (lane == 0) {
+            losses[0] = (float)(l / n);
+            losses[1] = (float)(c / n);
+            if (n_total) *n_total = n;
+            __hip_atomic_store(ticket, 0u, __ATOMIC_RELAXED, __HIP_MEMORY_SCOPE_AGENT);
+        }
     }
 }
 
@@ -364,6 +740,34 @@
     return GSSD_OK;
 }
 
+extern "C" long long gssd_multibox_loss_workspace_bytes(int B) { return B > 0 ? 16 + (long long)B * MS * (long long)sizeof(float) : 0; }
+
+extern "C" int gssd_multibox_loss_forward_f32(const float* loc, const float* conf, const float* priors, const float* targets,
+                                              const int* gt_off, int B, int P, int C, float threshold, float var0, float var1,
+                                              int negpos_ratio, float* loc_t, int64_t* conf_t, uint8_t* sel, double* partial,
+                                              float* losses, double* n_total, float* loss_c_all, void* workspace,
+                                              long long workspace_bytes, gssd_stream_t stream) {
+    GSSD_CHECK_ARG(loc && conf && priors && targets && gt_off && loc_t && conf_t && sel && partial && losses && workspace);
+    GSSD_CHECK_ARG(B > 0 && B <= 65535 && P > 0 && P < 32768 && C >= 2 && negpos_ratio >= 0);
+    GSSD_CHECK_ARG(workspace_bytes >= gssd_multibox_loss_workspace_bytes(B));
+    GSSD_CHECK_ARG(((uintptr_t)priors % 16) == 0 && ((uintptr_t)loc % 16) == 0 && ((uintptr_t)loc_t % 16) == 0);
+    GSSD_CHECK_ARG(((uintptr_t)workspace % 16) == 0 && ((uintptr_t)partial % 8) == 0 && ((uintptr_t)conf % 4) == 0);
+    unsigned* ticket = static_cast<unsigned*>(workspace);
+    float* pmax = reinterpret_cast<float*>(static_cast<unsigned char*>(workspace) + 16);
+    const int chunk = (P + MS - 1) / MS;
+    hipLaunchKernelGGL(match_slice_kernel, dim3(MS, B), dim3(MT), (size_t)chunk * (sizeof(float) + sizeof(int)), as_stream(stream),
+                       targets, gt_off, priors, conf, P, C, threshold, var0, var1, loc_t, conf_t, pmax);
+    GSSD_CHECK_LAUNCH();
+    static unsigned attr_mask = 0;
+    const size_t smem = (size_t)P * sizeof(float);
+    if (smem > 48 * 1024)
+        if (const int rc = gssd_max_dynamic_lds(&attr_mask, hnm_fused_kernel, 150 * 1024)) return rc;
+    hipLaunchKernelGGL(hnm_fused_kernel, dim3(B), dim3(LT), smem, as_stream(stream), loc, conf, loc_t, conf_t, pmax, B * MS, P, C,
+                       negpos_ratio, sel, partial, loss_c_all, ticket, B, losses, n_total);
+    GSSD_CHECK_LAUNCH();
+    return GSSD_OK;
+}
+
 extern "C" int gssd_loss_finalize_global(const double* partial, int B, const double* n_global, int world, float* losses, double* n_total,
                                          gssd_stream_t stream) {
     GSSD_CHECK_ARG(partial && losses && n_global && n_total && B > 0 && world > 0);
diff --git a/grouped-ssd-pytorch_amd/gssd/csrc/plan_run.hip b/grouped-ssd-pytorch_amd/gssd/csrc/plan_run.hip
--- a/grouped-ssd-pytorch_amd/gssd/csrc/plan_run.hip
+++ b/grouped-ssd-pytorch_amd/gssd/csrc/plan_run.hip
@@ -135,6 +135,7 @@
     GSSD_PLAN_FN(gssd_reduce_max_f32),
     GSSD_PLAN_FN(gssd_hnm_loss),
     GSSD_PLAN_FN(gssd_loss_finalize),
+    GSSD_PLAN_FN(gssd_multibox_loss_forward_f32),
     GSSD_PLAN_FN(gssd_loss_finalize_global),
     GSSD_PLAN_FN(gssd_loss_backward),
     GSSD_PLAN_FN(gssd_detect),
@@ -142,6 +143,7 @@
     GSSD_PLAN_FN(gssd_eval_match),
     GSSD_PLAN_FN(gssd_eval_ap),
     GSSD_PLAN_FN(gssd_heads_reduce_f32),
+    GSSD_PLAN_FN(gssd_heads_reduce2_f32),
     GSSD_PLAN_FN(gssd_interp_add_f32),
     GSSD_PLAN_FN(gssd_pixellink_final_f32),
     GSSD_PLAN_FN(gssd_pixellink_loss_f32),
diff --git a/grouped-ssd-pytorch_amd/gssd/ops.py b/grouped-ssd-pytorch_amd/gssd/ops.py
--- a/grouped-ssd-pytorch_amd/gssd/ops.py
+++ b/grouped-ssd-pytorch_amd/gssd/ops.py
@@ -432,27 +432,51 @@
     return loc_t, conf_t
 
 
+FUSE_LOSS = os.environ.get('GSSD_FUSE_LOSS', '1') != '0'
+_loss_ws = {}
+
+
+def _loss_workspace(dev, B):
+    key = (dev.index if dev.index is not None else torch.cuda.current_device(), _stream())
+    need = int(lib.gssd_multibox_loss_workspace_bytes(B))
+    if torch.cuda.is_current_stream_capturing():
+        return torch.zeros(max(need, 4096), device=dev, dtype=torch.uint8)
+    ws = _loss_ws.get(key)
+    if ws is None or ws.numel() < need:
+        ws = _loss_ws[key] = torch.zeros(max(need, 4096), device=dev, dtype=torch.uint8)
+    return ws
+
+
 def multibox_loss_forward(loc, conf, priors, tg, n_gt, threshold=0.5, negpos_ratio=3, variance=(0.1, 0.2),
-                          want_scores=False, global_n=False):
+                          want_scores=False, global_n=False, fused=None):
     _need_cuda(loc, conf, priors)
     loc = loc.contiguous()
     conf = conf.contiguous()
     B, P, _ = loc.shape
     Cc = conf.shape[-1]
     priors = priors[:P].contiguous()
-    loc_t, conf_t = match_batch(tg, n_gt, priors, threshold, variance)
     dev = loc.device
-    NX = 128
-    xmax = torch.empty(NX, device=dev, dtype=torch.float32)
-    check(lib.gssd_reduce_max_f32(_p(conf), conf.numel(), _p(xmax), NX, _stream()))
     sel = torch.empty(B, P, device=dev, dtype=torch.uint8)
     partial = torch.empty(B, 4, device=dev, dtype=torch.float64)
     lca = torch.empty(B, P, device=dev, dtype=torch.float32) if want_scores else None
-    check(lib.gssd_hnm_loss(_p(loc), _p(conf), _p(loc_t), _p(conf_t), _p(xmax), NX, B, P, Cc, int(negpos_ratio), _p(sel),
-                            _p(partial), _p(lca), _stream()))
     losses = torch.empty(2, device=dev, dtype=torch.float32)
     n_total = torch.empty(1, device=dev, dtype=torch.float64)
-    check(lib.gssd_loss_finalize(_p(partial), B, _p(losses), _p(n_total), _stream()))
+    if FUSE_LOSS if fused is None else fused:
+        _need_cuda(tg, n_gt)
+        loc_t = torch.empty(B, P, 4, device=dev, dtype=torch.float32)
+        conf_t = torch.empty(B, P, device=dev, dtype=torch.int64)
+        ws = _loss_workspace(dev, B)
+        check(lib.gssd_multibox_loss_forward_f32(_p(loc), _p(conf), _p(priors), _p(tg), _p(n_gt), B, P, Cc, threshold, variance[0],
+                                                 variance[1], int(negpos_ratio), _p(loc_t), _p(conf_t), _p(sel), _p(partial),
+                                                 _p(losses), _p(n_total), _p(lca), _p(ws), ws.numel(), _stream()))
+    else:
+        loc_t, conf_t = match_batch(tg, n_gt, priors, threshold, variance)
+        NX = 128
+        xmax = torch.empty(NX, device=dev, dtype=torch.float32)
+        check(lib.gssd_reduce_max_f32(_p(conf), conf.numel(), _p(xmax), NX, _stream()))
+        check(lib.gssd_hnm_loss(_p(loc), _p(conf), _p(loc_t), _p(conf_t), _p(xmax), NX, B, P, Cc, int(negpos_ratio), _p(sel),
+                                _p(partial), _p(lca), _stream()))
+        check(lib.gssd_loss_finalize(_p(partial), B, _p(losses), _p(n_total), _stream()))
     if global_n:
         import torch.distributed as dist
         if dist.is_initialized() and dist.get_world_size() > 1:
diff --git a/grouped-ssd-pytorch_amd/gssd/plan_common.py b/grouped-ssd-pytorch_amd/gssd/plan_common.py
--- a/grouped-ssd-pytorch_amd/gssd/plan_common.py
+++ b/grouped-ssd-pytorch_amd/gssd/plan_common.py
@@ -25,6 +25,7 @@
 FUSE_SPLIT = os.environ.get('GSSD_FUSE_SPLIT', '1') != '0'
 FUSE_SA_BN = os.environ.get('GSSD_FUSE_SA_BN', '1') != '0'
 FUSE_HEAD_BN = os.environ.get('GSSD_FUSE_HEAD_BN', '1') != '0'
+FUSE_HEADS_REDUCE = os.environ.get('GSSD_FUSE_HEADS_REDUCE', '1') != '0'
 SN_STREAM = 9
 ALL_STREAMS = -1
 
diff --git a/grouped-ssd-pytorch_amd/gssd/plan_graph.py b/grouped-ssd-pytorch_amd/gssd/plan_graph.py
--- a/grouped-ssd-pytorch_amd/gssd/plan_graph.py
+++ b/grouped-ssd-pytorch_amd/gssd/plan_graph.py
@@ -168,12 +168,20 @@
             d.flags |= _lib.CONV_HEADS_SLICES
         prev, self._sid = getattr(self, '_sid', 0), 0
         self._pending_wait = ALL_STREAMS
-        self._reduce_steps = (len(self.steps), len(self.steps) + 1)
-        self._add(lib.gssd_heads_reduce_f32, [self._ws_loc.data_ptr(), self._head_splits.data_ptr(), 0, B, self.P, 4])
-        self._add(lib.gssd_heads_reduce_f32, [self._ws_conf.data_ptr(), self._head_splits.data_ptr(), 0, B, self.P, self.nc])
+        if plan_common.FUSE_HEADS_REDUCE:
+            self._reduce_steps = (len(self.steps),)
+            self._add(lib.gssd_heads_reduce2_f32, [self._ws_loc.data_ptr(), self._ws_conf.data_ptr(), self._head_splits.data_ptr(), 0, 0,
+                                                   B, self.P, self.nc])
+        else:
+            self._reduce_steps = (len(self.steps), len(self.steps) + 1)
+            self._add(lib.gssd_heads_reduce_f32, [self._ws_loc.data_ptr(), self._head_splits.data_ptr(), 0, B, self.P, 4])
+            self._add(lib.gssd_heads_reduce_f32, [self._ws_conf.data_ptr(), self._head_splits.data_ptr(), 0, B, self.P, self.nc])
         self._sid = prev
 
     def _set_outputs(self, loc, conf):
+        if len(self._reduce_steps) == 1:
+            self.steps[self._reduce_steps[0]].args[3:5] = [loc.data_ptr(), conf.data_ptr()]
+            return
         self.steps[self._reduce_steps[0]].args[2] = loc.data_ptr()
         self.steps[self._reduce_steps[1]].args[2] = conf.data_ptr()
 
diff --git a/grouped-ssd-pytorch_amd/layers/modules/multibox_loss.py b/grouped-ssd-pytorch_amd/layers/modules/multibox_loss.py
--- a/grouped-ssd-pytorch_amd/layers/modules/multibox_loss.py
+++ b/grouped-ssd-pytorch_amd/layers/modules/multibox_loss.py
@@ -7,9 +7,9 @@
 
 class _MultiBoxLossFn(torch.autograd.Function):
     @staticmethod
-    def forward(ctx, loc, conf, priors, tg, n_gt, threshold, negpos_ratio, variance, global_n=False):
+    def forward(ctx, loc, conf, priors, tg, n_gt, threshold, negpos_ratio, variance, global_n=False, fused=None):
         st = ops.multibox_loss_forward(loc.detach(), conf.detach(), priors, tg, n_gt, threshold, negpos_ratio,
-                                       variance, global_n=global_n)
+                                       variance, global_n=global_n, fused=fused)
         ctx.st = st
         losses = st['losses']
         return losses[0], losses[1]
@@ -17,7 +17,7 @@
     @staticmethod
     def backward(ctx, g_l, g_c):
         dloc, dconf = ops.multibox_loss_backward(ctx.st, g_l, g_c)
-        return dloc, dconf, None, None, None, None, None, None, None
+        return dloc, dconf, None, None, None, None, None, None, None, None
 
 
 class MultiBoxLoss(nn.Module):
@@ -35,8 +35,9 @@
         self.neg_overlap = neg_overlap
         self.variance = cfg['variance']
         self.global_normalizer = False
+        self.fused = None
 
-    def forward(self, predictions, targets):
+    def forward(self, predictions, targets, fused=None):
         loc_data, conf_data, priors = predictions
         P = loc_data.size(1)
         priors = priors[:P, :]
@@ -45,4 +46,4 @@
         tg, n_gt = ops.pack_targets(targets, loc_data.device)
         return _MultiBoxLossFn.apply(loc_data, conf_data, priors.detach().contiguous(), tg, n_gt, float(self.threshold),
                                      int(self.negpos_ratio), (float(self.variance[0]), float(self.variance[1])),
-                                     bool(self.global_normalizer))
+                                     bool(self.global_normalizer), self.fused if fused is None else fused)
diff --git a/include/gssd_hip.h b/include/gssd_hip.h
--- a/include/gssd_hip.h
+++ b/include/gssd_hip.h
@@ -326,6 +326,12 @@
 int gssd_loss_finalize(const double* partial, int B, float* losses, double* n_total, gssd_stream_t stream);
 int gssd_loss_finalize_global(const double* partial, int B, const double* n_global, int world, float* losses, double* n_total,
                               gssd_stream_t stream);
+#define GSSD_MULTIBOX_SLICES 8
+long long gssd_multibox_loss_workspace_bytes(int B);
+int gssd_multibox_loss_forward_f32(const float* loc, const float* conf, const float* priors, const float* targets, const int* gt_off,
+                                   int B, int P, int C, float threshold, float var0, float var1, int negpos_ratio, float* loc_t,
+                                   int64_t* conf_t, uint8_t* sel, double* partial, float* losses, double* n_total, float* loss_c_all,
+                                   void* workspace, long long workspace_bytes, gssd_stream_t stream);
 int gssd_loss_backward(const float* loc, const float* conf, const float* loc_t, const int64_t* conf_t,
                        const uint8_t* sel, const double* n_total, const float* grad_l, const float* grad_c, int B,
                        int P, int C, float* dloc, float* dconf, gssd_stream_t stream);
@@ -346,6 +352,8 @@
                  long long workspace_bytes, double* ap_out, gssd_stream_t stream);
 
 int gssd_heads_reduce_f32(const float* ws, const signed char* splits, float* out, int B, int P, int C, gssd_stream_t stream);
+int gssd_heads_reduce2_f32(const float* ws_loc, const float* ws_conf, const signed char* splits, float* loc, float* conf, int B, int P,
+                           int C, gssd_stream_t stream);
 
 
 int gssd_interp_add_f32(const float* src, const float* addend, float* out, float* out2, int B, int Hs, int Ws, int Hd, int Wd, int C,
```
